# klory/vqa-attention-networks

Hardware: AMD Instinct MI355X
Metric: QA-pairs/sec fwd+bwd, MFB-baseline batch 512 (higher is better)
Workload: dtype f32

## Files before the change

include/vqa_fusion.h:

```cpp
#ifndef VQA_FUSION_H
#define VQA_FUSION_H

#include <stddef.h>
#include <stdint.h>

#ifdef __cplusplus
extern "C" {
#endif

#define VQF_OK 0
#define VQF_E_BADARG (-1)
#define VQF_E_ALIGN (-2)
#define VQF_E_UNSUPPORTED (-3)
#define VQF_E_WORKSPACE (-4)
#define VQF_E_TIMEOUT (-5)

#define VQF_POOL_K 5

#define VQF_GEMM_RELU 1
#define VQF_GEMM_ACCUM 2
#define VQF_GEMM_OUT_BF16 4

int vqf_abi_version(void);
const char* vqf_build_info(void);

#define VQF_OPT_GEMM_F32_PERSIST 0
#define VQF_OPT_GEMM_BF16_PERSIST 1
#define VQF_OPT_GEMM_F32_LOOP 2
#define VQF_OPT_GEMM_BF16_LOOP 3
#define VQF_OPT_GEMM_F32_BIG 4
#define VQF_OPT_GEMM_BF16_BIG 5
#define VQF_OPT_GEMM_F32_WAVE 6
#define VQF_OPT_FUSE_COAL 7
#define VQF_OPT_FUSE_LS 8
#define VQF_OPT_FUSE_LS_BWD 9
#define VQF_OPT_GEMM_CU_LIMIT 10
#define VQF_OPT_GEMM_F32_EDGE 11
#define VQF_OPT_GEMM_F32_ROUNDS 12
#define VQF_OPT_GEMM_SPLITK_FUSED 13
#define VQF_OPT_GEMM_F32_STREAMK 14
#define VQF_OPT_GEMM_SPLITK_ORDER 15
#define VQF_OPT_GEMM_F32_SAMPLE 16
#define VQF_OPT_GEMM_F32_N80 17
#define VQF_OPT_COUNT 18
int vqf_set_option(int option, int value, int* previous);
int vqf_get_option(int option, int* value);
const char* vqf_option_env_name(int option);

#define VQF_STAT_GEMM_F32_TILE128 0
#define VQF_STAT_GEMM_F32_BIG 1
#define VQF_STAT_GEMM_F32_WAVE 2
#define VQF_STAT_GEMM_BF16_TILE128 3
#define VQF_STAT_GEMM_BF16_BIG 4
#define VQF_STAT_GEMM_F32_SAMPLE 5
#define VQF_STAT_GEMM_F32_N80 6
#define VQF_STAT_COUNT 7
int vqf_stat_get(int stat, long long* value);

size_t vqf_gemm_f32_ws_bytes(int ta, int tb, int M, int N, int K);
int vqf_gemm_f32(int ta, int tb, int M, int N, int K,
                 const float* A, int lda, const float* B, int ldb,
                 float* C, int ldc, const float* bias, int flags,
                 void* ws, size_t ws_bytes, void* stream);

int vqf_gemm_f32_rowscale(int ta, int tb, int M, int N, int K, const float* A, int lda, const float* B, int ldb,
                          float* C, int ldc, const float* bias, int flags, const float* rowscale, int rows_per_scale,
                          void* stream);

int vqf_gemm_f32_big_rows(int ta, int tb, int M, int N, int K);
int vqf_gemm_f32_sample_supported(int NS, int L, int N, int K);
int vqf_gemm_f32_sample(int tb, int NS, int L, int N, int K, const float* A, int lda, const float* B, int ldb, float* C, int ldc,
                        const float* bias, int flags, void* stream);

int vqf_gemm_f32_batched(int ta, int tb, int batch, int M, int N, int K,
                         const float* A, int lda, long long strideA,
                         const float* B, int ldb, long long strideB,
                         float* C, int ldc, long long strideC, int flags, void* stream);

size_t vqf_gemm_bf16_ws_bytes(int ta, int tb, int M, int N, int K);
int vqf_gemm_bf16(int ta, int tb, int M, int N, int K,
                  const void* A, int lda, const void* B, int ldb,
                  float* C, int ldc, const float* bias, int flags,
                  void* ws, size_t ws_bytes, void* stream);
int vqf_gemm_bf16_rowscale(int ta, int tb, int M, int N, int K, const void* A, int lda, const void* B, int ldb,
                           float* C, int ldc, const float* bias, int flags, const float* rowscale, int rows_per_scale,
                           void* stream);

int vqf_cast_f32_bf16(const float* x, int R, int C, int ldx, void* y, int ldy, void* stream);

size_t vqf_colsum_ws_bytes(int M, int N);
int vqf_colsum_f32(const float* dY, int M, int N, int ldy, float* db,
                   void* ws, size_t ws_bytes, void* stream);

int vqf_group_reduce_f32(const float* in, int G, int J, int W, float* out, void* stream);

int vqf_relu_bwd_f32(const float* dX, const float* Y, int M, int C, float* dXpre,
                     float* dbias, void* ws, size_t ws_bytes, void* stream);

int vqf_relu_bwd_rank1_f32(const float* dX, const float* Y, const float* wts, const float* dpooled, int L, float scale, int M,
                           int C, float* dXpre, float* dbias, void* ws, size_t ws_bytes, void* stream);
int vqf_multi_add_f32(const float* const* a, const float* const* b, float* const* out, const long long* n, int count, void* stream);
int vqf_multi_copy_f32(const float* const* src, float* const* dst, const long long* n, int count, void* stream);


int vqf_att_logits_fwd(const float* hid, const float* w2, const float* b2,
                       int M, int Hh, int G, float* logits, void* stream);

int vqf_att_logits_fwd_lin(const float* hid, const float* w2, const float* b2, const float* b1, int M, int Hh, int G,
                           float* logits, float* lin, void* stream);

size_t vqf_att_logits_bwd_ws_bytes(int M, int Hh);
int vqf_att_logits_bwd(const float* dlogits, const float* hid, const float* w2,
                       int M, int Hh, int G, int relu_mask, float* dhid_pre, float* dw2,
                       float* db2, float* dbias1, void* ws, size_t ws_bytes, void* stream);
int vqf_att_logits_bwd_rowscale(const float* dlogits, const float* hid, const float* w2, const float* rowscale,
                                int rows_per_scale, int M, int Hh, int G, int relu_mask, float* dhid_pre, float* dw2,
                                float* db2, float* dbias1, void* ws, size_t ws_bytes, void* stream);
int vqf_att_logits_bwd_rowscale_obf16(const float* dlogits, const float* hid, const float* w2, const float* rowscale,
                                      int rows_per_scale, int M, int Hh, int G, void* dhid_pre_bf16, float* dw2, float* db2,
                                      float* dbias1, void* ws, size_t ws_bytes, void* stream);

int vqf_glimpse_pool_fwd(const float* feat, const float* logits, int N, int S, int C, int G,
                         int unit_softmax, float* wts, float* pooled, void* stream);

int vqf_glimpse_pool_bwd(const float* dpooled, const float* dwts_extra, const float* feat,
                         const float* wts, int N, int S, int C, int G, int unit_softmax,
                         float* dlogits, float* dfeat, void* stream);

int vqf_glimpse_pool_fwd_bf16(const void* feat, const float* logits, int N, int S, int C, int G,
                              int unit_softmax, float* wts, float* pooled, void* stream);
int vqf_glimpse_pool_bwd_bf16(const float* dpooled, const float* dwts_extra, const void* feat,
                              const float* wts, int N, int S, int C, int G, int unit_softmax,
                              float* dlogits, void* stream);

int vqf_mfb_fuse_fwd(const float* P, const float* pbias, const float* q, const float* cascade,
                     const uint8_t* keep, uint64_t seed, float p_drop,
                     int N, int L, int O, float* R, float* rowssq, float* zdrop,
                     void* stream);

int vqf_l2_group_norm(const float* rowssq, int N, int L, float* norm, float* inv, void* stream);

int vqf_scale_rows(const float* R, const float* inv, int M, int L, int W, float* Y, void* stream);

int vqf_rowdot(const float* Y, const float* dY, int M, int W, float* rowdot, void* stream);

int vqf_l2_norm_bwd_coef(const float* rowdot, const float* norm, const float* inv,
                         int N, int L, float* coefA, float* coefB, void* stream);
int vqf_l2_norm_bwd_coef_lin(const float* dlogits, const float* lin, int G, const float* norm, const float* inv, int N,
                             int L, float* coefA, float* coefB, float* unit, void* stream);

size_t vqf_mfb_fuse_bwd_ws_bytes(int N, int L, int O);
int vqf_mfb_fuse_bwd(const float* dY, const float* dzdrop, const float* Y, const float* inv,
                     const float* coefA, const float* coefB,
                     const float* P, const float* pbias, const float* q, const float* cascade,
                     const uint8_t* keep, uint64_t seed, float p_drop,
                     int N, int L, int O,
                     float* dP, float* dq, float* dcascade, float* dbiasP,
                     void* ws, size_t ws_bytes, void* stream);
int vqf_mfb_fuse_bwd_bf16dp(const float* dY, const float* Y, const float* inv, const float* coefA,
                            const float* coefB, const float* P, const float* pbias, const float* q,
                            const uint8_t* keep, uint64_t seed, float p_drop, int N, int L, int O,
                            void* dP_bf16, float* dq, float* dbiasP, void* ws, size_t ws_bytes, void* stream);
int vqf_mfb_fuse_fwd_pbf16(const void* P_bf16, const float* pbias, const float* q, const uint8_t* keep, uint64_t seed,
                           float p_drop, int N, int L, int O, float* R, float* rowssq, void* stream);
int vqf_mfb_fuse_fwd_pbf16_rb(const void* P_bf16, const float* pbias, const float* q, const uint8_t* keep, uint64_t seed,
                              float p_drop, int N, int L, int O, float* R, void* R_bf16, int ldrb, float* rowssq, void* stream);
int vqf_mfb_fuse_bwd_pbf16(const float* dY, const float* Y, const float* inv, const float* coefA,
                           const float* coefB, const void* P_bf16, const float* pbias, const float* q,
                           const uint8_t* keep, uint64_t seed, float p_drop, int N, int L, int O, void* dP_bf16,
                           float* dq, float* dbiasP, void* ws, size_t ws_bytes, void* stream);

int vqf_mfb_fuse_grouped_supported(int N, int U, int L, int O);
int vqf_mfb_fuse_fwd_grouped(const float* P, const float* pbias, const float* q, const int* idx, const uint8_t* keep, uint64_t seed,
                             float p_drop, int N, int U, int L, int O, float* R, float* rowssq, void* stream);
size_t vqf_mfb_fuse_bwd_grouped_ws_bytes(int N, int U, int L, int O);
int vqf_mfb_fuse_bwd_grouped(const float* dY, const float* Y, const float* inv, const float* coefA, const float* coefB,
                             const float* P, const float* pbias, const float* q, const int* idx, const int* order,
                             const int* grp_off, const uint8_t* keep, uint64_t seed, float p_drop, int N, int U, int L, int O,
                             float* dP, float* dq, float* dbiasP, void* ws, size_t ws_bytes, void* stream);

int vqf_mfb_fuse_fwd_len(const float* P, const float* pbias, const float* q, const int* lens, const uint8_t* keep, uint64_t seed,
                         float p_drop, int N, int L, int O, float* R, float* rowssq, void* stream);
int vqf_mfb_fuse_bwd_len(const float* dY, const float* Y, const float* inv, const float* coefA, const float* coefB, const float* P,
                         const float* pbias, const float* q, const int* lens, const uint8_t* keep, uint64_t seed, float p_drop,
                         int N, int L, int O, float* dP, float* dq, float* dbiasP, void* ws, size_t ws_bytes, void* stream);
int vqf_mfb_fuse_fwd_grouped_len(const float* P, const float* pbias, const float* q, const int* idx, const int* lens_q,
                                 const int* lens_u, const uint8_t* keep, uint64_t seed, float p_drop, int N, int U, int L, int O,
                                 float* R, float* rowssq, void* stream);
int vqf_mfb_fuse_bwd_grouped_len(const float* dY, const float* Y, const float* inv, const float* coefA, const float* coefB,
                                 const float* P, const float* pbias, const float* q, const int* idx, const int* order,
                                 const int* grp_off, const int* lens_q, const int* lens_u, const uint8_t* keep, uint64_t seed,
                                 float p_drop, int N, int U, int L, int O, float* dP, float* dq, float* dbiasP, void* ws,
                                 size_t ws_bytes, void* stream);
int vqf_glimpse_pool_fwd_grouped_len(const float* feat, const float* logits, const int* idx, const int* lens, int N, int U, int S, int C,
                                     int G, float* wts, float* pooled, void* stream);
int vqf_glimpse_pool_bwd_grouped_len(const float* dpooled, const float* dwts_extra, const float* feat, const float* wts, const int* idx,
                                     const int* order, const int* grp_off, const int* lens, int N, int U, int S, int C, int G,
                                     float* dlogits, float* dfeat, void* stream);


int vqf_dropout_f32(const float* x, const uint8_t* keep, uint64_t seed, float p_drop,
                    long long n, float* y, void* stream);
int vqf_dropout_bt(const float* x, long long sb_in, long long st_in, const uint8_t* keep, uint64_t seed, float p_drop, int B,
                   int T, int H, float* y, long long sb_out, long long st_out, void* stream);
int vqf_gate_tanh_sigmoid_fwd(const float* a, const float* b, long long n, float* y, void* stream);
int vqf_gate_tanh_sigmoid_bwd(const float* dy, const float* a, const float* b, long long n, float* da, float* db, void* stream);
int vqf_tanh_dropout_fwd(const float* a, const float* b, const uint8_t* keep, uint64_t seed,
                         float p_drop, long long n, float* y, void* stream);
int vqf_tanh_dropout_bwd(const float* dy, const float* y, const uint8_t* keep, uint64_t seed,
                         float p_drop, long long n, float* dx, void* stream);
int vqf_tanh_dropout_fwd2d(const float* a, int lda, const float* b, int ldb, const uint8_t* keep, uint64_t seed, float p_drop,
                           int R, int W, float* y, int ldy, void* stream);
int vqf_tanh_dropout_bwd2d(const float* dy, int lddy, const float* y, int ldy, const uint8_t* keep, uint64_t seed, float p_drop,
                           int R, int W, float* dx, int lddx, void* stream);
int vqf_hie_stream_supported(int N, int L, int E, int T);
int vqf_hie_chunks(int N, int L);
// ... 172 lines not shown
```

vqa-attention-networks_amd/csrc/common.h:

```cpp
#pragma once
#include <hip/hip_runtime.h>
#include <stdint.h>
#include "../../include/vqa_fusion.h"

typedef float f32x4 __attribute__((ext_vector_type(4)));
typedef float f32x16 __attribute__((ext_vector_type(16)));
typedef unsigned int u32x4 __attribute__((ext_vector_type(4)));

enum VqfKernelId {
  KID_GEMM_A0B0 = 0,
  KID_GEMM_A0B1,
  KID_GEMM_A1B0,
  KID_GEMM_A1B1,
  KID_SPLITK_REDUCE,
  KID_COLSUM,
  KID_GROUP_REDUCE,
  KID_RELU_BWD,
  KID_ATT_LOGITS_FWD,
  KID_ATT_LOGITS_BWD,
  KID_GLIMPSE_FWD,
  KID_GLIMPSE_BWD,
  KID_MFB_FUSE_FWD,
  KID_L2_GROUP_NORM,
  KID_SCALE_ROWS,
  KID_ROWDOT,
  KID_L2_BWD_COEF,
  KID_MFB_FUSE_BWD,
  KID_DROPOUT,
  KID_TANH_DROP_FWD,
  KID_TANH_DROP_BWD,
  KID_SOFTMAX_FWD,
  KID_SOFTMAX_BWD,
  KID_GEMM_BF16,
  KID_CAST_BF16,
  KID_LSTM_FWD,
  KID_LSTM_BWD,
  KID_CE_LOSS,
  KID_KLDIV_LOSS,
  KID_ADAM,
  KID_FEAT_TRANSPOSE,
  KID_LSTM_CELL_FWD,
  KID_LSTM_CELL_BWD,
  KID_EMBED_FWD,
  KID_EMBED_BWD,
  KID_HBM_COPY,
  KID_HBM_READ,
  KID_MULTI_ADD,
  KID_MULTI_COPY,
  KID_HIE_FWD,
  KID_HIE_HEAD,
  KID_HIE_ADD,
  KID_HIE_LEFT,
  KID_HIE_SLABSUM,
  KID_HIE_AFF,
  KID_PHRASE_FWD,
  KID_PHRASE_BWD,
  KID_HIE_AFF_LEVELS,
  KID_GUIDED_FWD,
  KID_GUIDED_BWD,
  KID_CE_LOSS_PRED,
  KID_ANSWER_MATCH,
  KID_TOPK_ROWS,
  KID_GLIMPSE_DFEAT_GROUPED,
  KID_ROW_BLOCK_GATHER,
  KID_ROW_BLOCK_GROUP_SUM,
  KID_MFB_FUSE_BWD_IMAGE,
  KID_ZERO_COLS,
  KID_COUNT
};

extern int g_vqf_prof_on;
extern int g_vqf_opt[VQF_OPT_COUNT];
static inline int vqf_opt(int id, int dflt) { const int v = g_vqf_opt[id]; return v < 0 ? dflt : v; }
extern long long g_vqf_stat[VQF_STAT_COUNT];
static inline void vqf_stat_bump(int id) { __atomic_fetch_add(&g_vqf_stat[id], 1LL, __ATOMIC_RELAXED); }
bool vqf_prof_begin(int id, hipStream_t s);
void vqf_prof_end(int id, hipStream_t s);
void vqf_prof_dims(int d0, int d1, int d2);

#define VQF_LAUNCH(id, kern, grid, block, shmem, stream, ...)                      \
  do {                                                                             \
    (void)hipGetLastError();     \
    const bool vqf_bracket_ = g_vqf_prof_on && vqf_prof_begin((id), (stream));     \
    hipLaunchKernelGGL(kern, grid, block, shmem, stream, __VA_ARGS__);             \
    if (vqf_bracket_) vqf_prof_end((id), (stream));                                \
  } while (0)

#define VQF_REDUCE_SPLITS 32
int vqf_colreduce_2stage(const float* in, int J, int W, float* out, float* scratch, hipStream_t s);

int vqf_splitk_reduce(const float* slab, int splits, int M, int N, float* C, int ldc,
                      const float* bias, int flags, hipStream_t s);
void vqf_splitk_counters_clear(int* words, int tiles, hipStream_t s);
int* vqf_splitk_counters(int tiles);

int vqf_gemm_bf16_big_try(int ta, int tb, int M, int N, int K, const void* A, int lda, const void* B, int ldb, float* C,
                          int ldc, const float* bias, int flags, const float* rowscale, int rps, void* ws, size_t ws_bytes,
                          hipStream_t s, int* rc);
size_t vqf_gemm_bf16_big_ws_bytes(int ta, int tb, int M, int N, int K);
int vqf_gemm_f32_big_try(int ta, int tb, int M, int N, int K, const float* A, int lda, const float* B, int ldb, float* C,
                         int ldc, const float* bias, int flags, const float* rowscale, int rps, void* ws, size_t ws_bytes,
                         hipStream_t s, int* rc, int* rows_done);
int vqf_gemm_f32_big_rows_impl(int ta, int tb, int M, int N, int K, int flags, size_t ws_bytes);
size_t vqf_gemm_f32_big_ws_bytes(int ta, int tb, int M, int N, int K);
int vqf_gemm_f32_n80_try(int M, int N, int K, const float* A, int lda, const float* B, int ldb, float* C, int ldc,
                         const float* bias, int flags, hipStream_t s, int* rc);
int vqf_lstm_step16_try(const float* h_prev, const float* w_hh, float* gates, const float* c_prev, int B, int H, float* c_out,
                        float* h_out, hipStream_t s, int* rc);
int vqf_gemm_f32_wave_try(int ta, int tb, int M, int N, int K, const float* A, int lda, const float* B, int ldb, float* C,
                          int ldc, const float* bias, int flags, hipStream_t s, int* rc);

static inline int vqf_last_error() {
  hipError_t e = hipGetLastError();
  return e == hipSuccess ? VQF_OK : (int)e;
}

static inline bool aligned16(const void* p) { return (((uintptr_t)p) & 15) == 0; }

struct VqfDynLdsFlags { int bytes[64]; };
static inline int vqf_set_dyn_lds(const void* fn, int bytes, VqfDynLdsFlags& f) {
  int dev = 0;
  (void)hipGetDevice(&dev);
  const bool tracked = dev >= 0 && dev < 64;
  if (tracked && f.bytes[dev] >= bytes) return VQF_OK;
  hipError_t e = hipFuncSetAttribute(fn, hipFuncAttributeMaxDynamicSharedMemorySize, bytes);
  if (e != hipSuccess) return (int)e;
  if (tracked && f.bytes[dev] < bytes) f.bytes[dev] = bytes;
  return VQF_OK;
}

static inline int vqf_cu_count() {
  static int cached[64] = {};
  int dev = 0;
  (void)hipGetDevice(&dev);
  const bool tracked = dev >= 0 && dev < 64;
  if (tracked && cached[dev] > 0) return cached[dev];
  int n = 0;
  if (hipDeviceGetAttribute(&n, hipDeviceAttributeMultiprocessorCount, dev) != hipSuccess) n = 0;
  if (tracked) cached[dev] = n;
  return n;
}

__device__ __forceinline__ float vqf_tanh_fast(float x) {
  const float e = __expf(2.0f * x);
  const float r = __builtin_amdgcn_rcpf(e + 1.0f);
  return e > 16777216.0f ? 1.0f : (e - 1.0f) * r;
}

#ifndef VQF_STREAM_NT
#define VQF_STREAM_NT 1
#endif
template <typename T> __device__ __forceinline__ T vqf_ld_stream(const T* p) {
  return VQF_STREAM_NT ? __builtin_nontemporal_load(p) : *p;
}
template <typename T> __device__ __forceinline__ void vqf_st_stream(T* p, T v) {
  if (VQF_STREAM_NT) __builtin_nontemporal_store(v, p); else *p = v;
}

__device__ __forceinline__ bool aligned16_dev(const void* p) { return (((uintptr_t)p) & 15) == 0; }
__device__ __forceinline__ float wave_sum(float v) {
#pragma unroll
  for (int o = 32; o > 0; o >>= 1) v += __shfl_xor(v, o, 64);
  return v;
}
__device__ __forceinline__ float wave_max(float v) {
#pragma unroll
  for (int o = 32; o > 0; o >>= 1) v = fmaxf(v, __shfl_xor(v, o, 64));
  return v;
}

__device__ __forceinline__ unsigned long long vqf_argmax_key(float v, int idx) {
  const unsigned int b = __float_as_uint(v);
  const unsigned int k = (v != v) ? 0xFFFFFFFEu : (v == 0.f ? 0x80000000u : ((b & 0x80000000u) ? ~b : (b | 0x80000000u)));
  return ((unsigned long long)k << 32) | (unsigned int)~(unsigned int)idx;
}
__device__ __forceinline__ int vqf_argmax_index(unsigned long long key) { return (int)~(unsigned int)key; }
__device__ __forceinline__ unsigned long long wave_max_u64(unsigned long long v) {
#pragma unroll
  for (int o = 32; o > 0; o >>= 1) {
    const unsigned long long t = __shfl_xor(v, o, 64);
    v = t > v ? t : v;
  }
  return v;
}
__device__ __forceinline__ unsigned long long vqf_block256_max_u64(unsigned long long v, unsigned long long* sh) {
  v = wave_max_u64(v);
  __syncthreads();
  if ((threadIdx.x & 63) == 0) sh[threadIdx.x >> 6] = v;
  __syncthreads();
  const unsigned long long a = sh[0] > sh[1] ? sh[0] : sh[1], b = sh[2] > sh[3] ? sh[2] : sh[3];
  return a > b ? a : b;
}

struct VqfSplitkTile { int* cnt; const float* slab; float* C; const float* bias; int M, N, ldc, flags; long long pstride; int sld; };
template <int TILE_M, int TILE_N, int NT, bool WT = false>
__device__ __forceinline__ bool vqf_splitk_combine(const VqfSplitkTile& g, int tile, int splits, int m0, int n0, int tid,
                                                   float* scratch) {
  asm volatile("s_waitcnt vmcnt(0)" ::: "memory");
  __syncthreads();
  if (tid == 0) {
    if (!WT) {
      __builtin_amdgcn_fence(__ATOMIC_RELEASE, "agent");
      asm volatile("s_waitcnt vmcnt(0)" ::: "memory");
    }
    const int ticket = __hip_atomic_fetch_add(g.cnt + tile, 1, __ATOMIC_RELAXED, __HIP_MEMORY_SCOPE_AGENT);
    *reinterpret_cast<volatile int*>(scratch) = ticket;
  }
  __syncthreads();
  const int ticket = *reinterpret_cast<volatile int*>(scratch);
  __syncthreads();
  if (ticket != splits - 1) return false;
  if (tid == 0) {
    __builtin_amdgcn_fence(__ATOMIC_ACQUIRE, "agent");
    asm volatile("s_waitcnt vmcnt(0)" ::: "memory");
    __hip_atomic_store(g.cnt + tile, 0, __ATOMIC_RELAXED, __HIP_MEMORY_SCOPE_AGENT);
  }
  __syncthreads();
  constexpr int CT = TILE_N / 4, RSTEP = NT / CT;
  static_assert(NT % CT == 0, "TILE_N / 4 must divide the workgroup size");
  const bool local = g.pstride != 0;
  const long long total = local ? g.pstride : (long long)g.M * g.N;
  const int sld = local ? g.sld : g.N;
  const int srow0 = local ? m0 : 0, scol0 = local ? n0 : 0;
  const bool relu = g.flags & VQF_GEMM_RELU, accum = g.flags & VQF_GEMM_ACCUM;
  const int c4 = tid % CT, r0 = tid / CT;
  const int col = n0 + 4 * c4;
  if ((g.N & 3) == 0 && (sld & 3) == 0 && (g.ldc & 3) == 0 && aligned16_dev(g.C) && aligned16_dev(g.slab) &&
      (!g.bias || aligned16_dev(g.bias))) {
    if (col >= g.N) return true;
    const f32x4 bv = g.bias ? *reinterpret_cast<const f32x4*>(g.bias + col) : f32x4{0.f, 0.f, 0.f, 0.f};
    for (int k = 0; k < TILE_M / RSTEP; k += 2) {
      const int rowA = m0 + r0 + RSTEP * k, rowB = rowA + RSTEP;
      if (rowA >= g.M) break;
      const bool hasB = rowB < g.M && k + 1 < TILE_M / RSTEP;
      const float* pA = g.slab + (long long)(rowA - srow0) * sld + (col - scol0);
      const float* pB = g.slab + (long long)((hasB ? rowB : rowA) - srow0) * sld + (col - scol0);
      f32x4 vA = {0.f, 0.f, 0.f, 0.f}, vB = vA;
      int z = 0;
      for (; z + 3 < splits; z += 4) {
        f32x4 a[4], b[4];
#pragma unroll
        for (int q = 0; q < 4; ++q) {
          a[q] = *reinterpret_cast<const f32x4*>(pA + (z + q) * total);
          b[q] = *reinterpret_cast<const f32x4*>(pB + (z + q) * total);
        }
#pragma unroll
        for (int q = 0; q < 4; ++q) { vA += a[q]; vB += b[q]; }
      }
      for (; z < splits; ++z) {
        vA += *reinterpret_cast<const f32x4*>(pA + z * total);
        vB += *reinterpret_cast<const f32x4*>(pB + z * total);
      }
      vA += bv; vB += bv;
      float* cA = g.C + (long long)rowA * g.ldc + col;
      float* cB = g.C + (long long)rowB * g.ldc + col;
      if (accum) {
        vA += *reinterpret_cast<const f32x4*>(cA);
        if (hasB) vB += *reinterpret_cast<const f32x4*>(cB);
      }
      if (relu) {
#pragma unroll
        for (int j = 0; j < 4; ++j) { vA[j] = fmaxf(vA[j], 0.f); vB[j] = fmaxf(vB[j], 0.f); }
      }
// ... 47 lines not shown
```

vqa-attention-networks_amd/csrc/gemm_f32.hip:

```cpp
#include "common.h"
#include <atomic>

namespace {

#ifndef VQF_SPLITK_WT
#define VQF_SPLITK_WT 0
#endif
#ifndef VQF_GEMM_BK
#define VQF_GEMM_BK 16
#endif
#ifndef VQF_GEMM_WAVES_PER_SIMD
#define VQF_GEMM_WAVES_PER_SIMD 4
#endif
#ifndef VQF_GEMM_GLDS
#define VQF_GEMM_GLDS 0
#endif
constexpr int BM = 128, BN = 128, BK = VQF_GEMM_BK, NTHREADS = 256;
constexpr bool GLDS = (VQF_GEMM_GLDS != 0) && (BK == 16);
constexpr int LD_RK = GLDS ? BK : BK + 4;
__device__ __forceinline__ int rk_swz(int row) { return GLDS ? ((row >> 2) & 3) : 0; }
constexpr int OP_FLOATS = BM * LD_RK;
constexpr int STAGE_FLOATS = 2 * OP_FLOATS;
constexpr int SMEM_BYTES = 2 * STAGE_FLOATS * 4;
constexpr int K4 = BK / 4;
constexpr int NLD = BM * BK / 4 / NTHREADS;
static_assert(BK % 8 == 0 && NLD >= 1, "BK must be a multiple of 8");

struct GemmArgs {
  const float* A;
  const float* B;
  float* C;
  const float* bias;
  float* slab;
  int M, N, K, lda, ldb, ldc;
  int flags;
  int kchunk;
  int tiles_m, tiles_n;
  int vecA, vecB;
  long long sA, sB, sC;
  const float* rowscale;
  int rps;
  int row0;
  int* cnt;
};

#ifndef VQF_GEMM_RK_REMAP
#define VQF_GEMM_RK_REMAP 0
#endif
__device__ __forceinline__ int rk_row(int f) {
  if (VQF_GEMM_RK_REMAP && K4 == 4) return ((f >> 5) << 3) + (((f >> 2) & 1) << 2) + ((f >> 3) & 3);
  return f / K4;
}
__device__ __forceinline__ int rk_k(int f) { return (f % K4) << 2; }

template <bool T>
__device__ __forceinline__ void load_tile(const float* __restrict__ p, int ld, int r0, int R,
                                          int k0, int kend, bool vec, int tid, f32x4 (&v)[NLD]) {
#pragma unroll
  for (int i = 0; i < NLD; ++i) {
    const int f = tid + NTHREADS * i;
    int r, k;
    if (!T) { r = r0 + rk_row(f); k = k0 + rk_k(f); }
    else    { k = k0 + (f >> 5); r = r0 + ((f & 31) << 2); }
    f32x4 x = {0.f, 0.f, 0.f, 0.f};
    if (!T) {
      if (r < R) {
        const float* q = p + (long long)r * ld + k;
        if (vec && k + 3 < kend) x = *reinterpret_cast<const f32x4*>(q);
        else {
#pragma unroll
          for (int j = 0; j < 4; ++j) if (k + j < kend) x[j] = q[j];
        }
      }
    } else {
      if (k < kend) {
        const float* q = p + (long long)k * ld + r;
        if (vec && r + 3 < R) x = *reinterpret_cast<const f32x4*>(q);
        else {
#pragma unroll
          for (int j = 0; j < 4; ++j) if (r + j < R) x[j] = q[j];
        }
      }
    }
    v[i] = x;
  }
}

typedef const float __attribute__((address_space(1))) gfloat;
typedef const f32x4 __attribute__((address_space(1))) gf32x4;

template <bool T>
__device__ __forceinline__ void init_ptrs(const float* __restrict__ p0, int ld, int r0, int R, int k0,
                                          int tid, gfloat* (&q)[NLD]) {
  gfloat* p = (gfloat*)p0;
#pragma unroll
  for (int i = 0; i < NLD; ++i) {
    const int f = tid + NTHREADS * i;
    if (!T) {
      const int r = min(r0 + rk_row(f), R - 1);
      q[i] = p + (long long)r * ld + (k0 + rk_k(f));
    } else {
      const int r = min(r0 + ((f & 31) << 2), R - 4);
      q[i] = p + (long long)(k0 + (f >> 5)) * ld + r;
    }
  }
}
template <bool T>
__device__ __forceinline__ void load_fast(gfloat* (&q)[NLD], int ld, f32x4 (&v)[NLD]) {
#pragma unroll
  for (int i = 0; i < NLD; ++i) {
    v[i] = *(gf32x4*)q[i];
    q[i] += T ? (long long)BK * ld : BK;
  }
}

constexpr int NGL = (BM * BK) / (4 * 64 * 4);
template <bool T>
__device__ __forceinline__ void init_glds_ptrs(const float* __restrict__ p0, int ld, int r0, int R, int k0,
                                               int wave, int lane, gfloat* (&q)[NGL]) {
  gfloat* p = (gfloat*)p0;
#pragma unroll
  for (int i = 0; i < NGL; ++i) {
    const int blk = wave * NGL + i;
    if (!T) {
      const int row = blk * 16 + (lane >> 2);
      const int c = (lane & 3) ^ rk_swz(row);
      q[i] = p + (long long)min(r0 + row, R - 1) * ld + (k0 + 4 * c);
    } else {
      const int k = blk * 2 + (lane >> 5);
      q[i] = p + (long long)(k0 + k) * ld + min(r0 + ((lane & 31) << 2), R - 4);
    }
  }
}
template <bool T>
__device__ __forceinline__ void glds_tile(gfloat* (&q)[NGL], int ld, float* s, int wave) {
  typedef __attribute__((address_space(3))) float lds_float;
#pragma unroll
  for (int i = 0; i < NGL; ++i) {
    lds_float* dst = (lds_float*)(s + (wave * NGL + i) * 256);
    __builtin_amdgcn_global_load_lds(q[i], dst, 16, 0, 0);
    q[i] += T ? (long long)BK * ld : BK;
  }
}

template <bool T>
__device__ __forceinline__ void store_tile(float* s, int tid, const f32x4 (&v)[NLD]) {
#pragma unroll
  for (int i = 0; i < NLD; ++i) {
    const int f = tid + NTHREADS * i;
    if (!T) *reinterpret_cast<f32x4*>(s + rk_row(f) * LD_RK + (((rk_k(f) >> 2) ^ rk_swz(rk_row(f))) << 2)) = v[i];
    else    *reinterpret_cast<f32x4*>(s + (f >> 5) * BM + ((f & 31) << 2)) = v[i];
  }
}
// ... 16 lines not shown
  const int nfull = (kend - kbeg) / BK;
  bool v10 = true, v01 = true;
  if (EDGE) {
    v10 = (m0 + wr * 64 + 32) < g.M;
    v01 = (n0 + wc * 64 + 32) < g.N;
  }
  f32x4 ra[NLD], rb[NLD];
  auto mma_tile = [&](const float* sA, const float* sB) {
#pragma unroll
    for (int g8 = 0; g8 < BK / 8; ++g8) {
      if (!EDGE) {
        f32x4 af[2], bf[2];
#pragma unroll
        for (int i = 0; i < 2; ++i) af[i] = read_frag<TA>(sA, wr * 64 + i * 32 + l31, g8, h);
#pragma unroll
        for (int j = 0; j < 2; ++j) bf[j] = read_frag<TB>(sB, wc * 64 + j * 32 + l31, g8, h);
#pragma unroll
        for (int kk = 0; kk < 4; ++kk)
#pragma unroll
          for (int i = 0; i < 2; ++i)
#pragma unroll
            for (int j = 0; j < 2; ++j)
              acc[i][j] = __builtin_amdgcn_mfma_f32_32x32x2f32(af[i][kk], bf[j][kk], acc[i][j], 0, 0, 0);
      } else {
        const f32x4 a0 = read_frag<TA>(sA, wr * 64 + l31, g8, h);
        const f32x4 b0 = read_frag<TB>(sB, wc * 64 + l31, g8, h);
#pragma unroll
        for (int kk = 0; kk < 4; ++kk)
          acc[0][0] = __builtin_amdgcn_mfma_f32_32x32x2f32(a0[kk], b0[kk], acc[0][0], 0, 0, 0);
        if (v10) {
          const f32x4 a1 = read_frag<TA>(sA, wr * 64 + 32 + l31, g8, h);
#pragma unroll
          for (int kk = 0; kk < 4; ++kk)
            acc[1][0] = __builtin_amdgcn_mfma_f32_32x32x2f32(a1[kk], b0[kk], acc[1][0], 0, 0, 0);
        }
        if (v01) {
          const f32x4 b1 = read_frag<TB>(sB, wc * 64 + 32 + l31, g8, h);
#pragma unroll
          for (int kk = 0; kk < 4; ++kk)
            acc[0][1] = __builtin_amdgcn_mfma_f32_32x32x2f32(a0[kk], b1[kk], acc[0][1], 0, 0, 0);
        }
      }
    }
  };

  if (FAST && GLDS) {
    const int lane = tid & 63, wave = 2 * wr + wc;
    gfloat* ga[NGL];
    gfloat* gb[NGL];
    init_glds_ptrs<TA>(gA, g.lda, m0, g.M, kbeg, wave, lane, ga);
    init_glds_ptrs<TB>(gB, g.ldb, n0, g.N, kbeg, wave, lane, gb);
    if (nfull > 0) {
      glds_tile<TA>(ga, g.lda, smem, wave);
      glds_tile<TB>(gb, g.ldb, smem + OP_FLOATS, wave);
    } else {
      load_tile<TA>(gA, g.lda, m0, g.M, kbeg, kend, g.vecA, tid, ra);
      load_tile<TB>(gB, g.ldb, n0, g.N, kbeg, kend, g.vecB, tid, rb);
      store_tile<TA>(smem, tid, ra);
      store_tile<TB>(smem + OP_FLOATS, tid, rb);
    }
    __syncthreads();
    for (int t = 0; t < ntiles; ++t) {
      float* sA = smem + (t & 1) * STAGE_FLOATS;
      float* sB = sA + OP_FLOATS;
      float* dA = smem + ((t + 1) & 1) * STAGE_FLOATS;
      const bool more = (t + 1) < ntiles;
      const bool dma = (t + 1) < nfull;
      if (!dma && more) {
        const int k0 = kbeg + (t + 1) * BK;
        load_tile<TA>(gA, g.lda, m0, g.M, k0, kend, g.vecA, tid, ra);
        load_tile<TB>(gB, g.ldb, n0, g.N, k0, kend, g.vecB, tid, rb);
      }
      if (!EDGE) {
        f32x4 af[BK / 8][2], bf[BK / 8][2];
#pragma unroll
        for (int g8 = 0; g8 < BK / 8; ++g8) {
#pragma unroll
          for (int i = 0; i < 2; ++i) af[g8][i] = read_frag<TA>(sA, wr * 64 + i * 32 + l31, g8, h);
#pragma unroll
          for (int j = 0; j < 2; ++j) bf[g8][j] = read_frag<TB>(sB, wc * 64 + j * 32 + l31, g8, h);
        }
        asm volatile("s_waitcnt lgkmcnt(0)" ::: "memory");
        if (dma) {
          glds_tile<TA>(ga, g.lda, dA, wave);
          glds_tile<TB>(gb, g.ldb, dA + OP_FLOATS, wave);
        }
#pragma unroll
        for (int g8 = 0; g8 < BK / 8; ++g8)
#pragma unroll
          for (int kk = 0; kk < 4; ++kk)
#pragma unroll
            for (int i = 0; i < 2; ++i)
#pragma unroll
              for (int j = 0; j < 2; ++j)
                acc[i][j] = __builtin_amdgcn_mfma_f32_32x32x2f32(af[g8][i][kk], bf[g8][j][kk], acc[i][j], 0, 0, 0);
      } else {
        if (dma) {
          glds_tile<TA>(ga, g.lda, dA, wave);
          glds_tile<TB>(gb, g.ldb, dA + OP_FLOATS, wave);
        }
        mma_tile(sA, sB);
      }
      if (more && !dma) {
        store_tile<TA>(dA, tid, ra);
        store_tile<TB>(dA + OP_FLOATS, tid, rb);
      }
      __syncthreads();
    }
    return;
  }

  gfloat* pa[NLD];
  gfloat* pb[NLD];
  if (FAST) {
    init_ptrs<TA>(gA, g.lda, m0, g.M, kbeg, tid, pa);
    init_ptrs<TB>(gB, g.ldb, n0, g.N, kbeg, tid, pb);
  }
  if (FAST && nfull > 0) {
    load_fast<TA>(pa, g.lda, ra);
    load_fast<TB>(pb, g.ldb, rb);
  } else {
    load_tile<TA>(gA, g.lda, m0, g.M, kbeg, kend, g.vecA, tid, ra);
    load_tile<TB>(gB, g.ldb, n0, g.N, kbeg, kend, g.vecB, tid, rb);
  }
  store_tile<TA>(smem, tid, ra);
  store_tile<TB>(smem + OP_FLOATS, tid, rb);
  __syncthreads();

  for (int t = 0; t < ntiles; ++t) {
    const float* sA = smem + (t & 1) * STAGE_FLOATS;
    const float* sB = sA + OP_FLOATS;
    const bool more = (t + 1) < ntiles;
    if (more) {
      if (FAST && (t + 1) < nfull) {
        load_fast<TA>(pa, g.lda, ra);
        load_fast<TB>(pb, g.ldb, rb);
      } else {
        const int k0 = kbeg + (t + 1) * BK;
        load_tile<TA>(gA, g.lda, m0, g.M, k0, kend, g.vecA, tid, ra);
        load_tile<TB>(gB, g.ldb, n0, g.N, k0, kend, g.vecB, tid, rb);
      }
    }
    mma_tile(sA, sB);
    if (more) {
      float* d = smem + ((t + 1) & 1) * STAGE_FLOATS;
      store_tile<TA>(d, tid, ra);
      store_tile<TB>(d + OP_FLOATS, tid, rb);
    }
    __syncthreads();
  }
}

template <bool TA, bool TB, bool FAST>
__global__ void __launch_bounds__(NTHREADS, VQF_GEMM_WAVES_PER_SIMD) gemm_f32_kernel(GemmArgs g) {
  extern __shared__ __attribute__((aligned(16))) float smem[];
  const int tid = threadIdx.x, lane = tid & 63;
  const int wave = __builtin_amdgcn_readfirstlane(tid >> 6);
  const int wr = wave >> 1, wc = wave & 1;
  const int l31 = lane & 31, h = lane >> 5;

  const int nwg = g.tiles_m * g.tiles_n;
  const int bid = blockIdx.x;
  const int q8 = nwg >> 3, r8 = nwg & 7, xcd = bid & 7;
  const int wg = (xcd < r8 ? xcd * (q8 + 1) : r8 * (q8 + 1) + (xcd - r8) * q8) + (bid >> 3);
  constexpr int GROUP_M = 8;
  const int per_group = GROUP_M * g.tiles_n;
  const int gid = wg / per_group;
  const int first_m = gid * GROUP_M;
  const int gsz = min(g.tiles_m - first_m, GROUP_M);
  const int in_g = wg - gid * per_group;
  const int tm = first_m + in_g % gsz, tn = in_g / gsz;
  const int m0 = tm * BM, n0 = tn * BN;
  const int kbeg = blockIdx.y * g.kchunk;
  const int kend = min(g.K, kbeg + g.kchunk);

  f32x16 acc[2][2];
#pragma unroll
  for (int i = 0; i < 2; ++i)
#pragma unroll
    for (int j = 0; j < 2; ++j)
#pragma unroll
      for (int r = 0; r < 16; ++r) acc[i][j][r] = 0.f;

  const float* gA = g.A + (long long)blockIdx.z * g.sA;
  const float* gB = g.B + (long long)blockIdx.z * g.sB;
  const bool all_valid = (m0 + wr * 64 + 32) < g.M && (n0 + wc * 64 + 32) < g.N;
  if (all_valid)
    gemm_mainloop<TA, TB, FAST, false>(g, smem, gA, gB, m0, n0, kbeg, kend, tid, wr, wc, l31, h, acc);
  else
    gemm_mainloop<TA, TB, FAST, true>(g, smem, gA, gB, m0, n0, kbeg, kend, tid, wr, wc, l31, h, acc);

  const bool to_slab = g.slab != nullptr;
  float* out = to_slab ? g.slab + (long long)blockIdx.y * g.M * g.N
                       : g.C + (long long)blockIdx.z * g.sC;
  const int ldo = to_slab ? g.N : g.ldc;
#pragma unroll
  for (int j = 0; j < 2; ++j) {
    const int col = n0 + wc * 64 + j * 32 + l31;
    if (col >= g.N) continue;
    const float bv = (!to_slab && g.bias) ? g.bias[col] : 0.f;
#pragma unroll
    for (int i = 0; i < 2; ++i) {
#pragma unroll
      for (int r = 0; r < 16; ++r) {
        const int row = m0 + wr * 64 + i * 32 + (r & 3) + 8 * (r >> 2) + 4 * h;
        if (row < g.M) {
          float* pc = out + (long long)row * ldo + col;
          float v = (g.rowscale ? acc[i][j][r] * g.rowscale[(g.row0 + row) / g.rps] : acc[i][j][r]) + bv;
          if (!to_slab) {
            if (g.flags & VQF_GEMM_ACCUM) v += *pc;
            if (g.flags & VQF_GEMM_RELU) v = fmaxf(v, 0.f);
          }
#if VQF_SPLITK_WT
          if (to_slab && g.cnt) __hip_atomic_store(pc, v, __ATOMIC_RELAXED, __HIP_MEMORY_SCOPE_AGENT); else
#endif
          *pc = v;
        }
      }
    }
  }
  if (to_slab && g.cnt) {
    const VqfSplitkTile st = {g.cnt, g.slab, g.C, g.bias, g.M, g.N, g.ldc, g.flags};
    vqf_splitk_combine<BM, BN, NTHREADS, VQF_SPLITK_WT != 0>(st, bid, (int)gridDim.y, m0, n0, tid, smem);
  }
}

__global__ void splitk_reduce_kernel(const float* __restrict__ slab, int splits, int M, int N,
                                     float* __restrict__ C, int ldc, const float* __restrict__ bias,
                                     int flags) {
  const long long total = (long long)M * N;
  const long long stride = (long long)gridDim.x * blockDim.x;
  for (long long i = (long long)blockIdx.x * blockDim.x + threadIdx.x; i < total; i += stride) {
    const int row = (int)(i / N), col = (int)(i - (long long)row * N);
    float v = 0.f;
    for (int z = 0; z < splits; ++z) v += slab[(long long)z * total + i];
    if (bias) v += bias[col];
    float* pc = C + (long long)row * ldc + col;
    if (flags & VQF_GEMM_ACCUM) v += *pc;
    if (flags & VQF_GEMM_RELU) v = fmaxf(v, 0.f);
    *pc = v;
  }
}

template <bool TA, bool TB, bool FAST>
int launch_gemm_impl(const GemmArgs& g, dim3 grid, hipStream_t s, int kid) {
  static VqfDynLdsFlags attr = {};
  if (int e = vqf_set_dyn_lds(reinterpret_cast<const void*>(&gemm_f32_kernel<TA, TB, FAST>), SMEM_BYTES, attr)) return e;
  VQF_LAUNCH(kid, (gemm_f32_kernel<TA, TB, FAST>), grid, dim3(NTHREADS), SMEM_BYTES, s, g);
  return vqf_last_error();
}

template <bool TA, bool TB>
int launch_gemm(const GemmArgs& g, dim3 grid, hipStream_t s, int kid) {
  const bool okA = g.vecA && (!TA || (g.M % 4 == 0 && g.M >= 4));
  const bool okB = g.vecB && (!TB || (g.N % 4 == 0 && g.N >= 4));
  if (okA && okB) return launch_gemm_impl<TA, TB, true>(g, grid, s, kid);
  return launch_gemm_impl<TA, TB, false>(g, grid, s, kid);
}

}

constexpr int VQF_SPLITK_RING = 1 << 16;
__device__ int vqf_splitk_ring[VQF_SPLITK_RING];
int* vqf_splitk_counters(int tiles) {
  static int* base[64] = {};
  static std::atomic<unsigned> next{0};
  if (tiles <= 0 || tiles > VQF_SPLITK_RING / 4) return nullptr;
  int dev = 0;
  if (hipGetDevice(&dev) != hipSuccess || dev < 0 || dev >= 64) return nullptr;
  if (!base[dev]) {
    void* q = nullptr;
    if (hipGetSymbolAddress(&q, HIP_SYMBOL(vqf_splitk_ring)) != hipSuccess) return nullptr;
    base[dev] = (int*)q;
  }
  unsigned cur = next.load(std::memory_order_relaxed), start;
  do {
    start = (cur % VQF_SPLITK_RING) + (unsigned)tiles <= (unsigned)VQF_SPLITK_RING ? cur % VQF_SPLITK_RING : 0u;
  } while (!next.compare_exchange_weak(cur, start + (unsigned)tiles, std::memory_order_relaxed));
  return base[dev] + start;
}

void vqf_splitk_counters_clear(int* words, int tiles, hipStream_t s) {
  if (words && tiles > 0) (void)hipMemsetAsync(words, 0, (size_t)tiles * sizeof(int), s);
}

int vqf_splitk_reduce(const float* slab, int splits, int M, int N, float* C, int ldc,
                      const float* bias, int flags, hipStream_t s) {
  const long long total = (long long)M * N;
  int blocks = (int)((total + 255) / 256);
  if (blocks > 4096) blocks = 4096;
  VQF_LAUNCH(KID_SPLITK_REDUCE, splitk_reduce_kernel, dim3(blocks), dim3(256), 0, s, slab, splits, M,
             N, C, ldc, bias, flags);
  return vqf_last_error();
}

extern "C" size_t vqf_gemm_f32_ws_bytes(int ta, int tb, int M, int N, int K) {
  return vqf_gemm_f32_big_ws_bytes(ta, tb, M, N, K);
}

static int gemm_tile128(int ta, int tb, int M, int N, int K, const float* A, int lda, const float* B, int ldb, float* C,
                        int ldc, const float* bias, int flags, const float* rowscale, int rps, int row0, void* ws,
                        size_t ws_bytes, hipStream_t s);

extern "C" int vqf_gemm_f32_big_rows(int ta, int tb, int M, int N, int K) {
  if (M <= 0 || N <= 0 || K <= 0) return 0;
  return vqf_gemm_f32_big_rows_impl(ta, tb, M, N, K, 0, (size_t)1 << 40);
}

extern "C" int vqf_gemm_f32(int ta, int tb, int M, int N, int K, const float* A, int lda,
                            const float* B, int ldb, float* C, int ldc, const float* bias,
                            int flags, void* ws, size_t ws_bytes, void* stream) {
  if (!A || !B || !C || M <= 0 || N <= 0 || K <= 0 || lda <= 0 || ldb <= 0 || ldc < N)
    return VQF_E_BADARG;
  hipStream_t s = (hipStream_t)stream;
  if (aligned16(A) && aligned16(B) && (lda % 4 == 0) && (ldb % 4 == 0)) {
    int rc = VQF_OK, done = 0;
    if (vqf_gemm_f32_big_try(ta, tb, M, N, K, A, lda, B, ldb, C, ldc, bias, flags, nullptr, 1, ws, ws_bytes, s, &rc, &done)) {
      if (rc != VQF_OK || done >= M) return rc;
      A += (size_t)done * lda; C += (size_t)done * ldc; M -= done;
      ws = nullptr; ws_bytes = 0;
    }
    else if (vqf_gemm_f32_wave_try(ta, tb, M, N, K, A, lda, B, ldb, C, ldc, bias, flags, s, &rc)) return rc;
    else if (!ta && !tb && vqf_gemm_f32_n80_try(M, N, K, A, lda, B, ldb, C, ldc, bias, flags, s, &rc)) return rc;
  }
  return gemm_tile128(ta, tb, M, N, K, A, lda, B, ldb, C, ldc, bias, flags, nullptr, 1, 0, ws, ws_bytes, s);
}

extern "C" int vqf_gemm_f32_rowscale(int ta, int tb, int M, int N, int K, const float* A, int lda, const float* B,
                                     int ldb, float* C, int ldc, const float* bias, int flags, const float* rowscale,
                                     int rows_per_scale, void* stream) {
  if (!A || !B || !C || !rowscale || rows_per_scale <= 0 || M <= 0 || N <= 0 || K <= 0 || lda <= 0 || ldb <= 0 || ldc < N)
    return VQF_E_BADARG;
  if (flags & VQF_GEMM_ACCUM) return VQF_E_UNSUPPORTED;
  hipStream_t s = (hipStream_t)stream;
  int row0 = 0;
  if (aligned16(A) && aligned16(B) && (lda % 4 == 0) && (ldb % 4 == 0)) {
    int rc = VQF_OK, done = 0;
    if (vqf_gemm_f32_big_try(ta, tb, M, N, K, A, lda, B, ldb, C, ldc, bias, flags, rowscale, rows_per_scale, nullptr, 0, s, &rc,
                             &done)) {
      if (rc != VQF_OK || done >= M) return rc;
      A += (size_t)done * lda; C += (size_t)done * ldc; M -= done; row0 = done;
    }
  }
  return gemm_tile128(ta, tb, M, N, K, A, lda, B, ldb, C, ldc, bias, flags, rowscale, rows_per_scale, row0, nullptr, 0, s);
}

static int gemm_tile128(int ta, int tb, int M, int N, int K, const float* A, int lda, const float* B, int ldb, float* C,
                        int ldc, const float* bias, int flags, const float* rowscale, int rps, int row0, void* ws,
                        size_t ws_bytes, hipStream_t s) {
  GemmArgs g;
  g.A = A; g.B = B; g.C = C; g.bias = bias; g.slab = nullptr;
  g.M = M; g.N = N; g.K = K; g.lda = lda; g.ldb = ldb; g.ldc = ldc; g.flags = flags;
  g.sA = g.sB = g.sC = 0;
  g.rowscale = rowscale; g.rps = rps; g.row0 = row0; g.cnt = nullptr;
  g.tiles_m = (M + BM - 1) / BM;
  g.tiles_n = (N + BN - 1) / BN;
  g.vecA = aligned16(A) && (lda % 4 == 0);
  g.vecB = aligned16(B) && (ldb % 4 == 0);

  const long long tiles = (long long)g.tiles_m * g.tiles_n;
  const int ktiles = (K + BK - 1) / BK;
  int splits = 1;
  const int slots = 512;
  if (ws && tiles < 1024 && ktiles >= 32 && !(tiles >= 512 && K <= 1024) && !(tiles >= 192 && tiles <= 256 && K <= 512)) {
    double best = 1e30;
    for (int sp = 1; sp <= 16; ++sp) {
      if (ktiles / sp < 16) break;
      if ((size_t)sp * M * N * sizeof(float) > ws_bytes) break;
      const double blocks = (double)tiles * sp;
      const double rounds = (double)((long long)((blocks + slots - 1) / slots));
      const double cost = rounds / sp * (1.0 + 0.01 * sp);
      if (cost < best - 1e-12) { best = cost; splits = sp; }
    }
  }
  int kt_per = (ktiles + splits - 1) / splits;
  g.kchunk = kt_per * BK;
  splits = (K + g.kchunk - 1) / g.kchunk;
  if (splits > 1) {
    g.slab = (float*)ws;
    if (vqf_opt(VQF_OPT_GEMM_SPLITK_FUSED, 0) == 1) g.cnt = vqf_splitk_counters((int)tiles);
  }

  dim3 grid((unsigned)tiles, (unsigned)splits);
  const int kid = KID_GEMM_A0B0 + 2 * (ta ? 1 : 0) + (tb ? 1 : 0);
  if (g_vqf_prof_on) vqf_prof_dims(M, N, K);
  vqf_stat_bump(VQF_STAT_GEMM_F32_TILE128);
  int rc;
  if (!ta && !tb) rc = launch_gemm<false, false>(g, grid, s, kid);
  else if (!ta && tb) rc = launch_gemm<false, true>(g, grid, s, kid);
  else if (ta && !tb) rc = launch_gemm<true, false>(g, grid, s, kid);
  else rc = launch_gemm<true, true>(g, grid, s, kid);
  if (rc != VQF_OK) {
    vqf_splitk_counters_clear(g.cnt, (int)tiles, s);
    return rc;
  }
  if (splits > 1 && !g.cnt) rc = vqf_splitk_reduce((const float*)ws, splits, M, N, C, ldc, bias, flags, s);
  return rc;
}

extern "C" int vqf_gemm_f32_batched(int ta, int tb, int batch, int M, int N, int K, const float* A,
                                    int lda, long long strideA, const float* B, int ldb,
                                    long long strideB, float* C, int ldc, long long strideC,
                                    int flags, void* stream) {
  if (!A || !B || !C || batch <= 0 || batch > 65535 || M <= 0 || N <= 0 || K <= 0 || lda <= 0 ||
      ldb <= 0 || ldc < N)
    return VQF_E_BADARG;
  GemmArgs g;
  g.A = A; g.B = B; g.C = C; g.bias = nullptr; g.slab = nullptr;
  g.M = M; g.N = N; g.K = K; g.lda = lda; g.ldb = ldb; g.ldc = ldc; g.flags = flags;
  g.sA = strideA; g.sB = strideB; g.sC = strideC;
  g.rowscale = nullptr; g.rps = 1; g.row0 = 0; g.cnt = nullptr;
  g.tiles_m = (M + BM - 1) / BM;
  g.tiles_n = (N + BN - 1) / BN;
  g.vecA = aligned16(A) && (lda % 4 == 0) && (strideA % 4 == 0);
  g.vecB = aligned16(B) && (ldb % 4 == 0) && (strideB % 4 == 0);
  g.kchunk = ((K + BK - 1) / BK) * BK;
  dim3 grid((unsigned)(g.tiles_m * g.tiles_n), 1, (unsigned)batch);
  hipStream_t s = (hipStream_t)stream;
  const int kid = KID_GEMM_A0B0 + 2 * (ta ? 1 : 0) + (tb ? 1 : 0);
  vqf_stat_bump(VQF_STAT_GEMM_F32_TILE128);
  if (!ta && !tb) return launch_gemm<false, false>(g, grid, s, kid);
  if (!ta && tb) return launch_gemm<false, true>(g, grid, s, kid);
  if (ta && !tb) return launch_gemm<true, false>(g, grid, s, kid);
  return launch_gemm<true, true>(g, grid, s, kid);
}
```

vqa-attention-networks_amd/csrc/gemm_f32_n80.hip:

```cpp
#include "common.h"

namespace {

typedef const float __attribute__((address_space(1))) gfloat;

constexpr int TM = 128, TN = 80, TK = 32, NT = 512, NSLOT = 4;
constexpr int A_BYTES = TM * TK * 4;
constexpr int b_bytes(int ntc) { return 16 * ntc * TK * 4; }
constexpr int slot_bytes(int ntc) { return A_BYTES + b_bytes(ntc); }

struct N80Args {
  const float* A; const float* B; float* C; const float* bias;
  int M, N, K, lda, ldb, ldc, flags, tiles_m, tiles;
  const float* c_prev; float* c_out; float* h_out; int H;
};

__device__ __forceinline__ float sigm_f(float x) { return 1.0f / (1.0f + expf(-x)); }

__device__ __forceinline__ int swz(int rho) {
  const int i = (rho >> 1) & 7;
  return i ^ (((i + 2) & 4) >> 1);
}

__device__ __forceinline__ void wait_own(int later, bool two) {
// ... 3 lines not shown
    else if (later == 1) asm volatile("s_waitcnt vmcnt(4)" ::: "memory");
    else                 asm volatile("s_waitcnt vmcnt(0)" ::: "memory");
  } else {
    if (later >= 3)      asm volatile("s_waitcnt vmcnt(9)" ::: "memory");
    else if (later == 2) asm volatile("s_waitcnt vmcnt(6)" ::: "memory");
    else if (later == 1) asm volatile("s_waitcnt vmcnt(3)" ::: "memory");
    else                 asm volatile("s_waitcnt vmcnt(0)" ::: "memory");
  }
}

template <int NTC, bool CELL>
__global__ void __launch_bounds__(NT, 1) gemm_f32_n80_kernel(const N80Args g) {
  constexpr int SLOT_BYTES = slot_bytes(NTC), TNC = 16 * NTC;
  extern __shared__ __attribute__((aligned(16))) char smem[];
  typedef __attribute__((address_space(3))) char lds_char;
  const int per = (gridDim.x + 7) >> 3;
  const int lin = (blockIdx.x & 7) * per + (blockIdx.x >> 3);
  if (lin >= g.tiles) return;
  const int tn = lin / g.tiles_m, tm = lin - tn * g.tiles_m;
  const int m0 = tm * TM, n0 = tn * TNC;
  const int tid = threadIdx.x, lane = tid & 63;
  const int wave = __builtin_amdgcn_readfirstlane(tid >> 6);
  const int c = lane & 15, kq = lane >> 4;
  const bool two = NTC == 5 && wave < 2;
  const int S = g.K / TK;

  float oldg[4][4], cpv[4];
  if (CELL) {
    const int u = (n0 >> 2) + c;
#pragma unroll
    for (int j = 0; j < 4; ++j) {
      const long long row = m0 + 16 * wave + 4 * kq + j;
#pragma unroll
      for (int t = 0; t < 4; ++t) oldg[t][j] = g.C[row * g.ldc + t * g.H + u];
      cpv[j] = g.c_prev ? g.c_prev[row * g.H + u] : 0.f;
    }
  }

  gfloat* qa[2];
  gfloat* qb[2];
#pragma unroll
  for (int i = 0; i < 2; ++i) {
    const int ra = 16 * wave + 8 * i + (lane >> 3);
    qa[i] = (gfloat*)(g.A + (long long)min(m0 + ra, g.M - 1) * g.lda + 4 * ((lane & 7) ^ swz(ra)));
    const int rho = 8 * (wave + 8 * i) + (lane >> 3);
    const int brow = CELL ? (min(rho, TNC - 1) >> 4) * g.H + (n0 >> 2) + (rho & 15)
                          : min(n0 + min(rho, TNC - 1), g.N - 1);
    qb[i] = (gfloat*)(g.B + (long long)brow * g.ldb + 4 * ((lane & 7) ^ swz(rho)));
  }
  auto issue_piece = [&](int s, int slot, int p) {
    lds_char* da = (lds_char*)(smem + slot * SLOT_BYTES + wave * 2048);
    lds_char* db = (lds_char*)(smem + slot * SLOT_BYTES + A_BYTES + wave * 1024);
    if (p == 0)      __builtin_amdgcn_global_load_lds(qa[0] + (long long)s * TK, da, 16, 0, 0);
    else if (p == 1) __builtin_amdgcn_global_load_lds(qa[1] + (long long)s * TK, da + 1024, 16, 0, 0);
    else if (p == 2) __builtin_amdgcn_global_load_lds(qb[0] + (long long)s * TK, db, 16, 0, 0);
    else if (two)    __builtin_amdgcn_global_load_lds(qb[1] + (long long)s * TK, db + 8 * 1024, 16, 0, 0);
  };
  auto issue = [&](int s, int slot) {
#pragma unroll
    for (int p = 0; p < 4; ++p) issue_piece(s, slot, p);
  };

  f32x4 acc[NTC];
#pragma unroll
  for (int t = 0; t < NTC; ++t) acc[t] = f32x4{0.f, 0.f, 0.f, 0.f};

  constexpr int NFR = 2 + 2 * NTC;
  struct Frag { f32x4 a[2], b[NTC][2]; };
  auto read_frag = [&](int slot, Frag& f, int i) {
    const char* sa = smem + slot * SLOT_BYTES;
    if (i < 2) {
      const int ra = 16 * wave + c;
      f.a[i] = *reinterpret_cast<const f32x4*>(sa + ra * 128 + (((2 * kq + i) ^ swz(ra)) << 4));
    } else {
      const int t = (i - 2) >> 1, u = (i - 2) & 1, rho = 16 * t + c;
      f.b[t][u] = *reinterpret_cast<const f32x4*>(sa + A_BYTES + rho * 128 + (((2 * kq + u) ^ swz(rho)) << 4));
    }
  };

  auto step = [&](int s, int q, const Frag& cur, Frag& nxt) {
    const bool more = s + 1 < S, copy = s + NSLOT < S;
#pragma unroll
    for (int grp = 0; grp < 8; ++grp) {
      const int u = grp >> 2, j = grp & 3;
#pragma unroll
      for (int t = 0; t < NTC; ++t) acc[t] = __builtin_amdgcn_mfma_f32_16x16x4f32(cur.a[u][j], cur.b[t][u][j], acc[t], 0, 0, 0);
#ifndef VQF_N80_NOCOPY
      if (grp < 4) { if (copy) issue_piece(s + NSLOT, q, grp); }
#endif
#ifndef VQF_N80_NOREAD
      if (more && 2 * grp < NFR) { read_frag((q + 1) % NSLOT, nxt, 2 * grp); read_frag((q + 1) % NSLOT, nxt, 2 * grp + 1); }
#endif
      __builtin_amdgcn_sched_barrier(0);
    }
  };
#pragma unroll
  for (int p = 0; p < NSLOT; ++p) issue(p, p);
  Frag fr[2];
  wait_own(NSLOT - 1, two);
  __builtin_amdgcn_s_barrier();
#pragma unroll
  for (int i = 0; i < NFR; ++i) read_frag(0, fr[0], i);
  for (int s0 = 0; s0 < S; s0 += NSLOT) {
#pragma unroll
    for (int q = 0; q < NSLOT; ++q) {
      const int s = s0 + q;
      if (s + 1 < S) wait_own(min(NSLOT - 2, S - 2 - s), two);
      __builtin_amdgcn_s_waitcnt(0xC07F);
#ifndef VQF_N80_NOBARRIER
      __builtin_amdgcn_s_barrier();
#endif
      step(s, q, fr[q & 1], fr[(q + 1) & 1]);
    }
  }

  if (CELL) {
    const int u = (n0 >> 2) + c;
#pragma unroll
    for (int j = 0; j < 4; ++j) {
      const long long row = m0 + 16 * wave + 4 * kq + j;
      const float ig = sigm_f(acc[0][j] + oldg[0][j]);
      const float fg = sigm_f(acc[1][j] + oldg[1][j]);
      const float gg = tanhf(acc[2 % NTC][j] + oldg[2][j]);
      const float og = sigm_f(acc[3 % NTC][j] + oldg[3][j]);
      float* pg = g.C + row * g.ldc + u;
      pg[0] = ig; pg[g.H] = fg; pg[2 * g.H] = gg; pg[3 * g.H] = og;
      const float cn = fg * cpv[j] + ig * gg;
      g.c_out[row * g.H + u] = cn;
      g.h_out[row * g.H + u] = og * tanhf(cn);
    }
    return;
  }
  const bool relu = g.flags & VQF_GEMM_RELU;
#pragma unroll
  for (int t = 0; t < NTC; ++t) {
    const int col = n0 + 16 * t + c;
    if (col < g.N) {
      const float bv = g.bias ? g.bias[col] : 0.f;
#pragma unroll
      for (int j = 0; j < 4; ++j) {
        const int row = m0 + 16 * wave + 4 * kq + j;
        if (row < g.M) {
          float v = acc[t][j] + bv;
          if (relu) v = fmaxf(v, 0.f);
          g.C[(long long)row * g.ldc + col] = v;
        }
      }
    }
  }
}

}

int vqf_gemm_f32_n80_try(int M, int N, int K, const float* A, int lda, const float* B, int ldb, float* C, int ldc,
                         const float* bias, int flags, hipStream_t s, int* rc) {
  if (vqf_opt(VQF_OPT_GEMM_F32_N80, 1) == 0) return 0;
  if ((flags & ~VQF_GEMM_RELU) || (K % 128) || K < 512 || !aligned16(A) || !aligned16(B) || (lda % 4) || (ldb % 4)) return 0;
  const int tiles_m = (M + TM - 1) / TM, tiles_n = (N + TN - 1) / TN;
  const long long tiles = (long long)tiles_m * tiles_n;
  const int cus = vqf_cu_count() > 0 ? vqf_cu_count() : 256;
  if (tiles > cus || tiles * 10 < (long long)cus * 8 || M > 1024) return 0;
  if (vqf_opt(VQF_OPT_GEMM_CU_LIMIT, 0) >= 8) return 0;
  N80Args g;
  g.A = A; g.B = B; g.C = C; g.bias = bias; g.M = M; g.N = N; g.K = K; g.lda = lda; g.ldb = ldb; g.ldc = ldc; g.flags = flags;
  g.tiles_m = tiles_m; g.tiles = (int)tiles;
  const int nwg = ((int)tiles + 7) & ~7;
  vqf_prof_dims(M, N, K);
  vqf_stat_bump(VQF_STAT_GEMM_F32_N80);
  static VqfDynLdsFlags attr = {};
  if (int e = vqf_set_dyn_lds(reinterpret_cast<const void*>(&gemm_f32_n80_kernel<5, false>), NSLOT * slot_bytes(5), attr)) { *rc = e; return 1; }
  VQF_LAUNCH(KID_GEMM_A0B0, (gemm_f32_n80_kernel<5, false>), dim3(nwg), dim3(NT), NSLOT * slot_bytes(5), s, g);
  *rc = vqf_last_error();
  return 1;
}

int vqf_lstm_step16_try(const float* h_prev, const float* w_hh, float* gates, const float* c_prev, int B, int H, float* c_out,
                        float* h_out, hipStream_t s, int* rc) {
  if (vqf_opt(VQF_OPT_GEMM_F32_N80, 1) == 0 || vqf_opt(VQF_OPT_GEMM_CU_LIMIT, 0) >= 8) return 0;
  if ((B % TM) || (H % 128) || H < 512) return 0;
  const int tiles_m = B / TM, tiles_n = H / 16;
  const long long tiles = (long long)tiles_m * tiles_n;
  const int cus = vqf_cu_count() > 0 ? vqf_cu_count() : 256;
  if (tiles > cus || tiles * 10 < (long long)cus * 8) return 0;
  N80Args g = {};
  g.A = h_prev; g.B = w_hh; g.C = gates; g.M = B; g.N = 4 * H; g.K = H; g.lda = H; g.ldb = H; g.ldc = 4 * H;
  g.tiles_m = tiles_m; g.tiles = (int)tiles;
  g.c_prev = c_prev; g.c_out = c_out; g.h_out = h_out; g.H = H;
  const int nwg = ((int)tiles + 7) & ~7;
  vqf_prof_dims(B, 4 * H, H);
  vqf_stat_bump(VQF_STAT_GEMM_F32_N80);
  static VqfDynLdsFlags attr = {};
  if (int e = vqf_set_dyn_lds(reinterpret_cast<const void*>(&gemm_f32_n80_kernel<4, true>), NSLOT * slot_bytes(4), attr)) { *rc = e; return 1; }
  VQF_LAUNCH(KID_LSTM_CELL_FWD, (gemm_f32_n80_kernel<4, true>), dim3(nwg), dim3(NT), NSLOT * slot_bytes(4), s, g);
  *rc = vqf_last_error();
  return 1;
}
```

vqa-attention-networks_amd/csrc/gemm_f32_wave.hip:

```cpp
#include "common.h"
#include <stdlib.h>

namespace {

typedef const float __attribute__((address_space(1))) gfloat;
typedef float f32x2 __attribute__((ext_vector_type(2)));

constexpr int WTM = 32, WTN = 64, TK = 16, NSLOT = 6, NT = 256;
constexpr int A_BYTES = WTM * TK * 4, B_BYTES = WTN * TK * 4, SLOT_BYTES = A_BYTES + B_BYTES;
constexpr int WAVE_LDS = NSLOT * SLOT_BYTES;
constexpr int SMEM_WAVE = 4 * WAVE_LDS;
constexpr int NGA = A_BYTES / 1024, NGB = B_BYTES / 1024, NGL = NGA + NGB;

struct WaveArgs {
  const float* A;
  const float* B;
  float* C;
  const float* bias;
  int M, N, K, lda, ldb, ldc, flags;
  int tiles_m, tiles_n, kpart;
  const float* c_prev;
  float* c_out;
  float* h_out;
  int H;
// ... 325 lines not shown
    if (s + 1 < S) half(s + 1, fb, fa);
  }
  const int cm = lane & 31, h = lane >> 5;
  const int col = n0 + 2 * cm;
  const float b0 = (g.bias && col < g.N) ? g.bias[col] : 0.f;
  const float b1 = (g.bias && col + 1 < g.N) ? g.bias[col + 1] : 0.f;
#pragma unroll
  for (int e = 0; e < 16; ++e)
    put2(g, m0 + (e & 3) + 8 * (e >> 2) + 4 * h, col, acc[0][e], acc[1][e], b0, b1, vec, cold[e][0], cold[e][1]);
}

template <bool TB, int NSL>
int launch_shb(const WaveArgs& g, int nwg, hipStream_t s) {
  static VqfDynLdsFlags attr = {};
  constexpr int SMEM_SHB = NSL * (4 * A_BYTES + B_BYTES);
  if (int e = vqf_set_dyn_lds(reinterpret_cast<const void*>(&gemm_f32_wave_shb_kernel<TB, NSL>), SMEM_SHB, attr)) return e;
  VQF_LAUNCH(KID_GEMM_A0B0 + (TB ? 1 : 0), (gemm_f32_wave_shb_kernel<TB, NSL>), dim3(nwg), dim3(NT), SMEM_SHB, s, g);
  return vqf_last_error();
}

__device__ __forceinline__ float sigm_f(float x) { return 1.0f / (1.0f + expf(-x)); }

__global__ void __launch_bounds__(NT, 1) gemm_f32_lstm_fwd_kernel(const WaveArgs g) {
  constexpr int NSL = 6;
  constexpr int SHB_A = NSL * A_BYTES;
  extern __shared__ __attribute__((aligned(16))) char smem[];
  typedef __attribute__((address_space(3))) char lds_char;
  const int tid = threadIdx.x, lane = tid & 63;
  const int wave = __builtin_amdgcn_readfirstlane(tid >> 6);
  const int nwg = gridDim.x, bid = blockIdx.x;
  const int q8 = nwg >> 3, r8 = nwg & 7, xcd = bid & 7;
  const int wg = (xcd < r8 ? xcd * (q8 + 1) : r8 * (q8 + 1) + (xcd - r8) * q8) + (bid >> 3);
  const int t = 4 * wg + wave;
  const int tm = t % g.tiles_m, tn = t / g.tiles_m;
  const int m0 = tm * WTM, u0 = tn * 16, H = g.H;
  const int S = g.kpart / TK;
  char* myA = smem + wave * SHB_A;
  char* shB = smem + 4 * SHB_A;

  f32x16 acc[2];
#pragma unroll
  for (int j = 0; j < 2; ++j)
#pragma unroll
    for (int e = 0; e < 16; ++e) acc[j][e] = 0.f;

  gfloat* q[NGS];
#pragma unroll
  for (int i = 0; i < NGA; ++i) {
    const int row = 16 * i + (lane >> 2);
    const int chunk = (lane & 3) ^ swz(row);
    q[i] = (gfloat*)(g.A + (long long)min(m0 + row, g.M - 1) * g.lda + chunk * 4);
  }
  {
    const int rho = 16 * wave + (lane >> 2);
    const int chunk = (lane & 3) ^ swz(rho);
    const int gate = 2 * (rho >> 5) + ((rho & 31) >> 4);
    q[NGA] = (gfloat*)(g.B + (long long)(gate * H + u0 + (rho & 15)) * g.ldb + chunk * 4);
  }
  auto copy = [&](int i, int sl) {
    lds_char* dst = (i < NGA) ? (lds_char*)(myA + sl * A_BYTES + i * 1024) : (lds_char*)(shB + sl * B_BYTES + wave * 1024);
    __builtin_amdgcn_global_load_lds(q[i], dst, 16, 0, 0);
    q[i] += TK;
  };
#pragma unroll
  for (int p = 0; p < NSL - 1; ++p)
    if (p < S) {
#pragma unroll
      for (int i = 0; i < NGS; ++i) copy(i, p);
    }
  const int cm = lane & 31, hh = lane >> 5;
  const int col0 = (cm >> 4) * H + u0 + (cm & 15);
  float old0[16], old1[16], cpv[16];
#pragma unroll
  for (int e = 0; e < 16; ++e) {
    const int row = m0 + (e & 3) + 8 * (e >> 2) + 4 * hh;
    const float* pc = g.C + (long long)row * g.ldc + col0;
    old0[e] = pc[0];
    old1[e] = pc[2 * H];
    cpv[e] = (g.c_prev && cm < 16) ? g.c_prev[(long long)row * H + u0 + cm] : 0.f;
  }
  FragS<false> fa[2], fb[2];
  int slot = 0;
  auto half = [&](int s, FragS<false> (&cur)[2], FragS<false> (&nxt)[2]) {
    const bool more = s + 1 < S, refill = s + NSL - 1 < S;
    const int nslot = (slot + 1 == NSL) ? 0 : slot + 1;
    const int rslot = (slot == 0) ? NSL - 1 : slot - 1;
#pragma unroll
    for (int n = 0; n < 16; ++n) {
      const int ks = n >> 3, e = (n >> 1) & 3, j = n & 1;
      acc[j] = __builtin_amdgcn_mfma_f32_32x32x2f32(cur[ks].a[e], cur[ks].b(j, e), acc[j], 0, 0, 0);
      if (n < NGS && refill) copy(n, rslot);
      if (n == 6 && more) {
        wait_copies3(min(NSL - 2, S - 2 - s));
        __builtin_amdgcn_s_barrier();
      }
      if (n == 7 && more) nxt[0].load(myA + nslot * A_BYTES, shB + nslot * B_BYTES, 0, lane);
      if (n == 9 && more) nxt[1].load(myA + nslot * A_BYTES, shB + nslot * B_BYTES, 1, lane);
      __builtin_amdgcn_sched_barrier(0);
    }
    __builtin_amdgcn_s_waitcnt(0xC07F);
    __builtin_amdgcn_sched_barrier(0);
    slot = nslot;
  };
  if (S > 0) {
    wait_copies3(min(NSL - 2, S - 1));
    __builtin_amdgcn_s_barrier();
    fa[0].load(myA, shB, 0, lane);
    fa[1].load(myA, shB, 1, lane);
    __builtin_amdgcn_sched_barrier(0);
    __builtin_amdgcn_s_waitcnt(0xC07F);
    __builtin_amdgcn_sched_barrier(0);
  }
  for (int s = 0; s < S; s += 2) {
    half(s, fa, fb);
    if (s + 1 < S) half(s + 1, fb, fa);
  }
  const bool lo = cm < 16;
#pragma unroll
  for (int e = 0; e < 16; ++e) {
    const int row = m0 + (e & 3) + 8 * (e >> 2) + 4 * hh;
    const float a0 = sigm_f(acc[0][e] + old0[e]);
    const float p1 = acc[1][e] + old1[e];
    const float a1 = lo ? tanhf(p1) : sigm_f(p1);
    float* pc = g.C + (long long)row * g.ldc + col0;
    pc[0] = a0;
    pc[2 * H] = a1;
    const float f_act = __shfl_xor(a0, 16, 64), o_act = __shfl_xor(a1, 16, 64);
    if (lo) {
      const float c = f_act * cpv[e] + a0 * a1;
      g.c_out[(long long)row * H + u0 + cm] = c;
      g.h_out[(long long)row * H + u0 + cm] = o_act * tanhf(c);
    }
  }
}

int launch_lstm_fwd(const WaveArgs& g, int nwg, hipStream_t s) {
  static VqfDynLdsFlags attr = {};
  constexpr int SMEM_SHB = 6 * (4 * A_BYTES + B_BYTES);
  if (int e = vqf_set_dyn_lds(reinterpret_cast<const void*>(&gemm_f32_lstm_fwd_kernel), SMEM_SHB, attr)) return e;
  VQF_LAUNCH(KID_LSTM_CELL_FWD, gemm_f32_lstm_fwd_kernel, dim3(nwg), dim3(NT), SMEM_SHB, s, g);
  return vqf_last_error();
}

template <bool TB, int WK>
int launch(const WaveArgs& g, int nwg, hipStream_t s) {
  static VqfDynLdsFlags attr = {};
  if (int e = vqf_set_dyn_lds(reinterpret_cast<const void*>(&gemm_f32_wave_kernel<TB, WK>), SMEM_WAVE, attr)) return e;
  VQF_LAUNCH(KID_GEMM_A0B0 + (TB ? 1 : 0), (gemm_f32_wave_kernel<TB, WK>), dim3(nwg), dim3(NT), SMEM_WAVE, s, g);
  return vqf_last_error();
}

}

int vqf_gemm_f32_wave_try(int ta, int tb, int M, int N, int K, const float* A, int lda, const float* B, int ldb, float* C,
                          int ldc, const float* bias, int flags, hipStream_t s, int* rc) {
  if (vqf_opt(VQF_OPT_GEMM_F32_WAVE, 1) == 0) return 0;
  if (ta || M > 1024 || (K % TK) || K < 256 || !aligned16(A) || !aligned16(B) || (lda % 4) || (ldb % 4)) return 0;
  if (tb && (N % 4)) return 0;
  if ((long long)((M + 127) / 128) * ((N + 127) / 128) >= 256) return 0;
  WaveArgs g;
  g.A = A; g.B = B; g.C = C; g.bias = bias;
  g.M = M; g.N = N; g.K = K; g.lda = lda; g.ldb = ldb; g.ldc = ldc; g.flags = flags;
  g.tiles_m = (M + WTM - 1) / WTM;
  g.tiles_n = (N + WTN - 1) / WTN;
  const int tiles = g.tiles_m * g.tiles_n;
  const int nwg1 = (tiles + 3) / 4, nwg4 = tiles;
  const bool ok4 = (K % (4 * TK) == 0) && K / 4 >= 256;
  int wk = 0;
  if (nwg1 <= 256 && nwg1 >= 192) wk = 1;
  else if (ok4 && nwg4 <= 256 && nwg4 >= 192) wk = 4;
  if (!wk) return 0;
  g.kpart = (wk == 1) ? K : K / 4;
  vqf_prof_dims(M, N, K);
  vqf_stat_bump(VQF_STAT_GEMM_F32_WAVE);
  const bool shb = wk == 1 && (g.tiles_m % 4 == 0) && tiles % 4 == 0 && vqf_opt(VQF_OPT_GEMM_F32_WAVE, 2) != 1;
  if (shb && vqf_opt(VQF_OPT_GEMM_F32_WAVE, 2) == 3)
    *rc = tb ? launch_shb<true, 12>(g, nwg1, s) : launch_shb<false, 12>(g, nwg1, s);
  else if (shb)     *rc = tb ? launch_shb<true, 6>(g, nwg1, s) : launch_shb<false, 6>(g, nwg1, s);
  else if (wk == 1) *rc = tb ? launch<true, 1>(g, nwg1, s) : launch<false, 1>(g, nwg1, s);
  else         *rc = tb ? launch<true, 4>(g, nwg4, s) : launch<false, 4>(g, nwg4, s);
  return 1;
}

extern "C" int vqf_lstm_step_supported(int B, int H) {
  return B > 0 && H >= 256 && (B % 128) == 0 && (H % 16) == 0 && vqf_opt(VQF_OPT_GEMM_F32_WAVE, 2) != 0;
}
extern "C" int vqf_lstm_step_fwd(const float* h_prev, const float* w_hh, float* gates, const float* c_prev, int B, int H,
                                 float* c_out, float* h_out, void* stream) {
  if (!h_prev || !w_hh || !gates || !c_out || !h_out || B <= 0 || H <= 0) return VQF_E_BADARG;
  if (!vqf_lstm_step_supported(B, H)) return VQF_E_UNSUPPORTED;
  if (!aligned16(h_prev) || !aligned16(w_hh) || !aligned16(gates) || !aligned16(c_out) || !aligned16(h_out) ||
      (c_prev && !aligned16(c_prev)))
    return VQF_E_ALIGN;
  {
    int rc = VQF_OK;
    if (vqf_lstm_step16_try(h_prev, w_hh, gates, c_prev, B, H, c_out, h_out, (hipStream_t)stream, &rc)) return rc;
  }
  WaveArgs g = {};
  g.A = h_prev; g.B = w_hh; g.C = gates; g.bias = nullptr;
  g.M = B; g.N = 4 * H; g.K = H; g.lda = H; g.ldb = H; g.ldc = 4 * H; g.flags = VQF_GEMM_ACCUM;
  g.tiles_m = B / WTM;
  g.tiles_n = H / 16;
  g.kpart = H;
  g.c_prev = c_prev; g.c_out = c_out; g.h_out = h_out; g.H = H;
  vqf_prof_dims(B, 4 * H, H);
  vqf_stat_bump(VQF_STAT_GEMM_F32_WAVE);
  return launch_lstm_fwd(g, g.tiles_m * g.tiles_n / 4, (hipStream_t)stream);
}
```

vqa-attention-networks_amd/csrc/prof.hip:

```cpp
#include "common.h"
#include <mutex>
#include <stdlib.h>
#include <vector>

int g_vqf_prof_on = 0;
int g_vqf_opt[VQF_OPT_COUNT];
long long g_vqf_stat[VQF_STAT_COUNT] = {};

namespace {
const char* const kOptEnv[VQF_OPT_COUNT] = {
    "VQF_GEMM_F32_PERSIST", "VQF_GEMM_BF16_PERSIST", "VQF_GEMM_F32_LOOP", "VQF_GEMM_BF16_LOOP", "VQF_GEMM_F32_BIG",
    "VQF_GEMM_BF16_BIG", "VQF_GEMM_F32_WAVE", "VQF_FUSE_COAL", "VQF_FUSE_LS", "VQF_FUSE_LS_BWD", "VQF_GEMM_CU_LIMIT",
    "VQF_GEMM_F32_EDGE", "VQF_GEMM_F32_ROUNDS", "VQF_GEMM_SPLITK_FUSED", "VQF_GEMM_F32_STREAMK", "VQF_GEMM_SPLITK_ORDER", "VQF_GEMM_F32_SAMPLE", "VQF_GEMM_F32_N80"};
const char* const kOptEnvOld[VQF_OPT_COUNT] = {
    nullptr, nullptr, "VQF_GEMM_F32_PP", "VQF_GEMM_BF16_PP", nullptr, nullptr, nullptr, nullptr, nullptr, nullptr, nullptr,
    nullptr, nullptr, nullptr, nullptr, nullptr, nullptr};
struct OptInit {
  OptInit() {
    for (int i = 0; i < VQF_OPT_COUNT; ++i) {
      const char* e = getenv(kOptEnv[i]);
      if (!e && kOptEnvOld[i]) e = getenv(kOptEnvOld[i]);
      g_vqf_opt[i] = (e && ((e[0] >= '0' && e[0] <= '9') || e[0] == '-')) ? atoi(e) : -1;
    }
  }
} g_opt_init;
}

namespace {
struct Pair { hipEvent_t a, b; int id; int d[3]; };
std::mutex g_mu;
std::vector<Pair> g_pairs;
std::vector<hipEvent_t> g_free;
thread_local hipEvent_t t_start = nullptr;
thread_local int t_dims[3] = {0, 0, 0};
long long g_min_mnk = 0;

const char* const kNames[KID_COUNT] = {
    "gemm_f32_a0b0(fwd)", "gemm_f32_a0b1(dgrad)", "gemm_f32_a1b0", "gemm_f32_a1b1(wgrad)",
    "splitk_reduce", "colsum", "group_reduce", "relu_bwd",
    "att_logits_fwd", "att_logits_bwd", "glimpse_pool_fwd", "glimpse_pool_bwd",
    "mfb_fuse_fwd", "l2_group_norm", "scale_rows", "rowdot", "l2_norm_bwd_coef", "mfb_fuse_bwd",
    "dropout", "tanh_dropout_fwd", "tanh_dropout_bwd", "softmax_rows_fwd", "softmax_rows_bwd",
    "gemm_bf16", "cast_f32_bf16",
    "lstm_seq_fwd(all steps)", "lstm_seq_bwd(all steps)",
    "ce_loss", "kldiv_loss", "adam_step", "feat_transpose",
    "lstm_cell_fwd", "lstm_cell_bwd", "embed_tanh_fwd", "embed_tanh_bwd", "hbm_copy", "hbm_read_sweep", "multi_add", "multi_copy", "hie_hv_fwd", "hie_head_bwd", "hie_rank_add", "hie_rank_left", "hie_slab_sum", "hie_affinity",
    "phrase_ngram_fwd", "phrase_ngram_bwd", "hie_affinity_levels", "guided_logits_fwd", "guided_logits_bwd",
    "ce_loss_pred", "answer_match_rows", "topk_rows", "glimpse_dfeat_grouped", "row_block_gather", "row_block_group_sum",
    "mfb_fuse_bwd_image", "zero_cols_len"};

hipEvent_t get_event() {
  std::lock_guard<std::mutex> lk(g_mu);
  if (!g_free.empty()) { hipEvent_t e = g_free.back(); g_free.pop_back(); return e; }
  hipEvent_t e = nullptr;
  (void)hipEventCreate(&e);
  return e;
}
}

bool vqf_prof_begin(int id, hipStream_t s) {
  if (g_min_mnk > 0) {
    const bool gemm = (id >= KID_GEMM_A0B0 && id <= KID_GEMM_A1B1) || id == KID_GEMM_BF16;
    if (!gemm || (long long)t_dims[0] * t_dims[1] * t_dims[2] < g_min_mnk) return false;
  }
  t_start = get_event();
  (void)hipEventRecord(t_start, s);
  return true;
}
void vqf_prof_end(int id, hipStream_t s) {
  hipEvent_t b = get_event();
  (void)hipEventRecord(b, s);
  std::lock_guard<std::mutex> lk(g_mu);
  g_pairs.push_back({t_start, b, id, {t_dims[0], t_dims[1], t_dims[2]}});
}
void vqf_prof_dims(int d0, int d1, int d2) { t_dims[0] = d0; t_dims[1] = d1; t_dims[2] = d2; }

extern "C" {
int vqf_abi_version(void) { return 7; }
int vqf_set_option(int option, int value, int* previous) {
  if (option < 0 || option >= VQF_OPT_COUNT) return VQF_E_BADARG;
  if (previous) *previous = g_vqf_opt[option];
  g_vqf_opt[option] = value < 0 ? -1 : value;
  return VQF_OK;
}
int vqf_stat_get(int stat, long long* value) {
  if (stat < 0 || stat >= VQF_STAT_COUNT || !value) return VQF_E_BADARG;
  *value = __atomic_load_n(&g_vqf_stat[stat], __ATOMIC_RELAXED);
  return VQF_OK;
}
int vqf_get_option(int option, int* value) {
  if (option < 0 || option >= VQF_OPT_COUNT || !value) return VQF_E_BADARG;
  *value = g_vqf_opt[option];
  return VQF_OK;
}
const char* vqf_option_env_name(int option) { return (option >= 0 && option < VQF_OPT_COUNT) ? kOptEnv[option] : ""; }
const char* vqf_build_info(void) {
  return "libvqa_fusion gfx950 fp32-mfma(v_mfma_f32_32x32x2_f32) tiles 128x128x16 + 256x256x16(lds-dma, staggered) + "
         "32x64-per-wave(small M) bf16-mfma(v_mfma_f32_16x16x32_bf16 / 32x32x16) tiles 128x128x32 + "
         "256x256x32(lds-dma, ping-pong) wave64 philox4x32-10";
}
void vqf_prof_enable(int on) { g_vqf_prof_on = on ? 1 : 0; }
void vqf_prof_filter(long long min_mnk) { g_min_mnk = min_mnk > 0 ? min_mnk : 0; }
void vqf_prof_reset(void) {
  std::lock_guard<std::mutex> lk(g_mu);
  for (auto& p : g_pairs) { g_free.push_back(p.a); g_free.push_back(p.b); }
  g_pairs.clear();
}
int vqf_prof_num_kernels(void) { return KID_COUNT; }
const char* vqf_prof_kernel_name(int id) { return (id >= 0 && id < KID_COUNT) ? kNames[id] : ""; }
int vqf_prof_get(int id, long long* launches, double* total_ms) {
  return vqf_prof_get_shape(id, -1, -1, -1, launches, total_ms);
}
int vqf_prof_get_shape(int id, int d0, int d1, int d2, long long* launches, double* total_ms) {
  if (id < 0 || id >= KID_COUNT || !launches || !total_ms) return VQF_E_BADARG;
  std::lock_guard<std::mutex> lk(g_mu);
  long long n = 0;
  double ms = 0.0;
  for (auto& p : g_pairs) {
    if (p.id != id) continue;
    if ((d0 >= 0 && p.d[0] != d0) || (d1 >= 0 && p.d[1] != d1) || (d2 >= 0 && p.d[2] != d2)) continue;
    hipError_t e = hipEventSynchronize(p.b);
    if (e != hipSuccess) return (int)e;
    float t = 0.f;
    e = hipEventElapsedTime(&t, p.a, p.b);
    if (e != hipSuccess) return (int)e;
    ms += t;
    ++n;
  }
  *launches = n;
  *total_ms = ms;
  return VQF_OK;
}
}
```

vqa-attention-networks_amd/host/functions.py:

```python
import torch

from . import ops


def _c(t):
    return t if t.is_contiguous() else t.contiguous()


def _w2d(w):
    return _c(w.reshape(w.shape[0], -1))


def _bf16_ok(*dims):
    return all(d % 8 == 0 for d in dims)


class EmbedTanhFn(torch.autograd.Function):

    @staticmethod
    def forward(ctx, ids, weight, tanh=True, time_major=False, lens=None):
        ids = ids.contiguous()
        out = ops.embed_tanh_fwd(_c(weight), ids, tanh, time_major, lens=lens)
        ctx.save_for_backward(ids, out if tanh else None)
        ctx.V, ctx.tm, ctx.lens = weight.shape[0], bool(time_major), lens
        return out

    @staticmethod
    def backward(ctx, dout):
        ids, out = ctx.saved_tensors
        return None, ops.embed_tanh_bwd(_c(dout), out, ids, ctx.V, ctx.tm, lens=ctx.lens), None, None, None


def _plain_embedding(embedding, ids):
    w = embedding.weight
    return (w.is_cuda and w.dtype == torch.float32 and ids.is_cuda and ids.dtype == torch.int64 and embedding.padding_idx is None
            and embedding.max_norm is None and not embedding.sparse and not embedding.scale_grad_by_freq and w.shape[1] <= 1024)


def embed_tanh(embedding, ids, time_major=False):
    if _plain_embedding(embedding, ids):
        return EmbedTanhFn.apply(ids, embedding.weight, True, bool(time_major) and ids.dim() == 2)
    y = torch.tanh(embedding(ids))
    return y.transpose(0, 1).contiguous() if time_major and ids.dim() == 2 else y


def embed(embedding, ids):
    if _plain_embedding(embedding, ids):
        return EmbedTanhFn.apply(ids, embedding.weight, False, False)
    return embedding(ids)


class NormLink:
    __slots__ = ("inv", "L", "lin", "xb")

    def __init__(self):
        self.inv, self.L, self.lin, self.xb = None, 0, None, None


class LinearFn(torch.autograd.Function):

    @staticmethod
    def forward(ctx, x, w, b, relu=False, bf16=False):
        x = _c(x)
        w2 = _w2d(w)
        bf16 = bool(bf16) and _bf16_ok(x.shape[0], x.shape[1], w2.shape[0])
        if bf16:
            xb, wb = ops.cast_bf16(x), ops.cast_bf16(w2)
            y = ops.gemm_bf16(xb, wb, bias=b, relu=relu)
            ctx.save_for_backward(xb, w, y if relu else None, wb)
        else:
            y = ops.gemm(x, w2, bias=b, relu=relu)
            ctx.save_for_backward(x, w, y if relu else None, None)
        ctx.has_bias = b is not None
        ctx.relu = relu
        ctx.bf16 = bf16
        return y

    @staticmethod
    def backward(ctx, dy):
        x, w, y, wb = ctx.saved_tensors
        w2 = _w2d(w)
        dy = _c(dy)
        db = None
        if ctx.relu:
            dy, db = ops.relu_bwd(dy, y, want_bias=ctx.has_bias)
        elif ctx.has_bias and ctx.needs_input_grad[2]:
            db = ops.colsum(dy)
        dx = dw = None
        if ctx.bf16:
            dyb = ops.cast_bf16(dy)
            if ctx.needs_input_grad[0]:
                dx = ops.gemm_bf16(dyb, wb, tb=True)
            if ctx.needs_input_grad[1]:
                dw = ops.gemm_bf16(dyb, x, ta=True, tb=True).view_as(w)
            return dx, dw, db, None, None
        if ctx.needs_input_grad[0]:
            dx = ops.gemm(dy, w2, tb=True)
        if ctx.needs_input_grad[1]:
            dw = ops.gemm(dy, x, ta=True, tb=True).view_as(w)
        return dx, dw, db, None, None


class Linear2Fn(torch.autograd.Function):

    @staticmethod
    def forward(ctx, x1, x2, w, b):
        x1, x2 = _c(x1), _c(x2)
        w2 = _w2d(w)
        K1 = x1.shape[1]
        y = ops.gemm(x1, w2[:, :K1], bias=b)
        ops.gemm(x2, w2[:, K1:], out=y, accumulate=True)
        ctx.save_for_backward(x1, x2, w)
        ctx.has_bias = b is not None
        return y

    @staticmethod
    def backward(ctx, dy):
        x1, x2, w = ctx.saved_tensors
        w2 = _w2d(w)
        dy = _c(dy)
        K1 = x1.shape[1]
        dx1 = ops.gemm(dy, w2[:, :K1], tb=True) if ctx.needs_input_grad[0] else None
        dx2 = ops.gemm(dy, w2[:, K1:], tb=True) if ctx.needs_input_grad[1] else None
        dw = None
        if ctx.needs_input_grad[2]:
            dw = torch.empty_like(w2)
            ops.gemm(dy, x1, ta=True, tb=True, out=dw[:, :K1])
            ops.gemm(dy, x2, ta=True, tb=True, out=dw[:, K1:])
            dw = dw.view_as(w)
        db = ops.colsum(dy) if (ctx.has_bias and ctx.needs_input_grad[3]) else None
        return dx1, dx2, dw, db


class JoinRowsFn(torch.autograd.Function):

    @staticmethod
    def forward(ctx, v, q, buf):
        n = v.shape[0]
        if v.data_ptr() != buf.data_ptr() or q.data_ptr() != buf[n:].data_ptr() or buf.shape[0] != n + q.shape[0]:
            raise ops._l.VqfError("JoinRowsFn: v and q must be the row blocks of buf")
        ctx.n = n
        return buf.view_as(buf)

    @staticmethod
    def backward(ctx, g):
        g = _c(g)
        return g[:ctx.n], g[ctx.n:], None


class AttHeadFn(torch.autograd.Function):

    @staticmethod
    def _pool_fwd(feat, logits, unit, grp, lens=None):
        if grp is None:
            return ops.glimpse_pool_fwd(feat, logits, unit, lens=lens)
        if unit:
            U, S, _ = feat.shape
            zeros = torch.zeros((U * S, logits.shape[1]), dtype=torch.float32, device=feat.device)
            _, per_image = ops.glimpse_pool_fwd(feat, zeros, True, lens=None if lens is None else lens[1])
            return None, ops.row_block_gather(per_image, grp[0])
        return ops.glimpse_pool_fwd_grouped(feat, logits, grp[0], lens=None if lens is None else lens[0])

    @staticmethod
    def _pool_bwd(dpooled, feat, wts, unit, need_dfeat, grp, NS, G, lens=None):
        if grp is None:
            return ops.glimpse_pool_bwd(dpooled, feat, wts, unit, need_dfeat, lens=lens)
        if need_dfeat:
            raise ops._l.VqfError("AttHeadFn: with shared images (grp) the feature tensor is data and gets no gradient")
        if unit:
            return torch.zeros((NS, G), dtype=torch.float32, device=dpooled.device), None
        return ops.glimpse_pool_bwd_grouped(dpooled, feat, wts, grp[0], grp[1], grp[2], False, lens=None if lens is None else lens[0])

    @staticmethod
    def forward(ctx, x, feat, w1, b1, wm, bm, w2, b2, unit_softmax, bf16=False, link=None, same_src=False, grp=None, lens=None):
        x = _c(x)
        feat = _c(feat)
        ctx.bf16 = bool(bf16)
        ctx.same_src = bool(same_src)
        ctx.grp = grp
        ctx.lens = lens
        if lens is not None and (ctx.bf16 or ctx.same_src or feat.dtype != torch.float32 or ctx.needs_input_grad[1]):
            raise ops._l.VqfError("AttHeadFn: region counts (lens) are fp32 only, for a feature tensor that is data")
        if grp is not None and (ctx.bf16 or ctx.same_src or feat.dtype != torch.float32):
            raise ops._l.VqfError("AttHeadFn: shared images (grp) are fp32 only and never the MLP's own source")
        if ctx.same_src and (x.numel() != feat.numel() or x.shape[-1] != feat.shape[-1] or x.dtype != feat.dtype):
            raise ops._l.VqfError("AttHeadFn: same_src needs x = feat.view(N*S, C)")
        ctx.link = link if (link is not None and link.inv is not None) else None
        if ctx.link is not None:
            if wm is not None or b1 is None:
                raise ops._l.VqfError("AttHeadFn: a NormLink needs the single-hidden-layer head with a bias")
            ctx.bf16 = ctx.bf16 and _bf16_ok(_w2d(w1).shape[0], _w2d(w1).shape[1])
            if ctx.bf16:
                w1b = ops.cast_bf16(_w2d(w1), 32)
                xb = link.xb if (link.xb is not None and link.xb.shape == (x.shape[0], w1b.shape[1])) else ops.cast_bf16(x, 32)
                link.xb = None
                hid1 = ops.gemm_bf16_rowscale(xb, w1b, link.inv, link.L, bias=b1, relu=True, K=xb.shape[1])
                x = xb
            else:
                hid1 = ops.gemm_rowscale(x, _w2d(w1), link.inv, link.L, bias=b1, relu=True)
            logits, lin = ops.att_logits_fwd_lin(hid1, _w2d(w2), b2, b1)
            wts, pooled = AttHeadFn._pool_fwd(feat, logits, unit_softmax, grp, lens)
            ctx.save_for_backward(x, feat, w1, w1b if ctx.bf16 else None, w2, hid1, None, wts, lin)
            ctx.unit = bool(unit_softmax)
            return pooled
        ctx.bf16 = ctx.bf16 and _bf16_ok(_w2d(w1).shape[0], _w2d(w1).shape[1])
        if ctx.bf16:
            xb, w1b = ops.cast_bf16(x, 32), ops.cast_bf16(_w2d(w1), 32)
            hid1 = ops.gemm_bf16(xb, w1b, K=xb.shape[1], bias=b1, relu=True)
            x = xb
        else:
            hid1 = ops.gemm(x, _w2d(w1), bias=b1, relu=True)
        hid2 = ops.gemm(hid1, _w2d(wm), bias=bm, relu=True) if wm is not None else None
        last = hid2 if hid2 is not None else hid1
        logits = ops.att_logits_fwd(last, _w2d(w2), b2)
        wts, pooled = AttHeadFn._pool_fwd(feat, logits, unit_softmax, grp, lens)
        ctx.save_for_backward(x, feat, w1, wm, w2, hid1, hid2, wts, w1b if ctx.bf16 else None)
        ctx.unit = bool(unit_softmax)
        return pooled

    @staticmethod
    def backward(ctx, dpooled):
        x, feat, w1, wm, w2, hid1, hid2, wts, lin = ctx.saved_tensors
        dpooled = _c(dpooled)
        need_dfeat = ctx.needs_input_grad[1]
        dlogits, dfeat = AttHeadFn._pool_bwd(dpooled, feat, wts, ctx.unit, need_dfeat, ctx.grp, hid1.shape[0], _w2d(w2).shape[0],
                                             ctx.lens)
        if ctx.link is not None:
            link = ctx.link
            w1b = wm
            obf = ctx.bf16 and hid1.shape[1] % 8 == 0 and w2.shape[0] == 2
            d1s, dw2, db2, db1 = ops.att_logits_bwd(dlogits, hid1, _w2d(w2), relu_mask=True, rowscale=link.inv,
                                                    rows_per_scale=link.L, out_bf16=obf)
            link.lin = (dlogits, lin)
            if ctx.bf16:
                cin = _w2d(w1).shape[1]
                d1b = d1s if obf else ops.cast_bf16(d1s)
                dw1 = ops.gemm_bf16(d1b, x, ta=True, tb=True)[:, :cin].contiguous().view_as(w1)
                dx = ops.gemm_bf16(d1b, w1b, tb=True, N=cin) if ctx.needs_input_grad[0] else None
                return dx, dfeat, dw1, db1, None, None, dw2.view_as(w2), db2, None, None, None, None, None, None
            dw1 = ops.gemm(d1s, x, ta=True, tb=True).view_as(w1)
            dx = ops.gemm(d1s, _w2d(w1), tb=True) if ctx.needs_input_grad[0] else None
            return dx, dfeat, dw1, db1, None, None, dw2.view_as(w2), db2, None, None, None, None, None, None
        last = hid2 if hid2 is not None else hid1
        dlast_pre, dw2, db2, dblast = ops.att_logits_bwd(dlogits, last, _w2d(w2), relu_mask=True)
        dwm = dbm = None
        if hid2 is not None:
            dwm = ops.gemm(dlast_pre, hid1, ta=True, tb=True).view_as(wm)
            dbm = dblast
            dhid1 = ops.gemm(dlast_pre, _w2d(wm), tb=True)
            d1_pre, db1 = ops.relu_bwd(dhid1, hid1, want_bias=True)
        else:
            d1_pre, db1 = dlast_pre, dblast
        if ctx.bf16:
            cin = _w2d(w1).shape[1]
            d1b = ops.cast_bf16(d1_pre)
            dw1 = ops.gemm_bf16(d1b, x, ta=True, tb=True)[:, :cin].contiguous().view_as(w1)
            dx = None
            if ctx.needs_input_grad[0]:
                dx = ops.gemm_bf16(d1b, lin, tb=True, N=cin)
        else:
            dw1 = ops.gemm(d1_pre, x, ta=True, tb=True).view_as(w1)
            if ctx.same_src and dfeat is not None:
                ops.gemm(d1_pre, _w2d(w1), tb=True, out=dfeat.view(x.shape), accumulate=True)
                dx = None
            else:
                dx = ops.gemm(d1_pre, _w2d(w1), tb=True) if ctx.needs_input_grad[0] else None
        return dx, dfeat, dw1, db1, dwm, dbm, dw2.view_as(w2), db2, None, None, None, None, None, None


def _arm_link(link, inv, L, xb=None):
    if link is not None:
        link.inv, link.L, link.lin, link.xb = inv, L, None, (xb[0] if xb else None)
    return link

# ... 137 lines not shown
    return P0, img2


class ImgProjLateFn(torch.autograd.Function):

    @staticmethod
    def forward(ctx, P0, img2, wi, cu_limit=0):
        ctx.save_for_backward(img2, wi)
        ctx.cu_limit = cu_limit
        return P0.view_as(P0)

    @staticmethod
    def backward(ctx, dP):
        img2, wi = ctx.saved_tensors
        dP = _c(dP)
        with (ops.options(gemm_cu_limit=ctx.cu_limit) if ctx.cu_limit else ops.options()):
            if img2.dtype == torch.bfloat16:
                dPb = dP if dP.dtype == torch.bfloat16 else ops.cast_bf16(dP)
                dwi = ops.gemm_bf16(dPb, img2, ta=True, tb=True).view_as(wi)
            else:
                dwi = ops.gemm(dP, img2, ta=True, tb=True).view_as(wi)
        return None, None, dwi, None


class MfbFuseFn(torch.autograd.Function):

    @staticmethod
    def forward(ctx, P0, bi, q, keep, seed, p_drop, N, L, link=None, grp=None, lens=None):
        P0, q = _c(P0), _c(q)
        O = P0.shape[1] // ops.POOL_K
        ctx.grp = grp
        ctx.lens = lens
        if lens is not None and P0.dtype != torch.float32:
            raise ops._l.VqfError("MfbFuseFn: region counts (lens) are fp32 only, got a %s projection" % P0.dtype)
        if grp is not None:
            if P0.dtype != torch.float32:
                raise ops._l.VqfError("MfbFuseFn: shared images (grp) are fp32 only, got a %s projection" % P0.dtype)
            U = P0.shape[0] // L
            Y, norm, inv = ops.mfb_fuse_fwd_grouped(P0, q, grp[0], N, U, L, O, keep=keep, seed=seed, p_drop=p_drop, pbias=bi,
                                                    normalise=link is None, lens=lens)
            ctx.link = _arm_link(link, inv, L, None)
            ctx.save_for_backward(P0, bi, q, Y, norm, inv, keep)
            ctx.seed, ctx.p_drop, ctx.dims = seed, p_drop, (N, L, O)
            return Y
        rb = [] if (link is not None and P0.dtype == torch.bfloat16) else None
        Y, norm, inv, _ = ops.mfb_fuse_fwd(P0, q, N, L, O, keep=keep, seed=seed, p_drop=p_drop, pbias=bi,
                                           normalise=link is None, r_bf16=rb, lens=lens)
        ctx.link = _arm_link(link, inv, L, rb)
        ctx.save_for_backward(P0, bi, q, Y, norm, inv, keep)
        ctx.seed, ctx.p_drop, ctx.dims = seed, p_drop, (N, L, O)
        return Y

    @staticmethod
    def backward(ctx, dY):
        P0, bi, q, Y, norm, inv, keep = ctx.saved_tensors
        N, L, O = ctx.dims
        if ctx.grp is not None:
            dP, dq, dbi = ops.mfb_fuse_bwd_grouped(_c(dY), Y, norm, inv, P0, q, ctx.grp[0], ctx.grp[1], ctx.grp[2], N,
                                                   P0.shape[0] // L, L, O, keep=keep, seed=ctx.seed, p_drop=ctx.p_drop,
                                                   want_dbias=True, pbias=bi, lin=_take_lin(ctx.link), lens=ctx.lens)
            return dP, dbi, dq, None, None, None, None, None, None, None, None
        dP, dq, _, dbi = ops.mfb_fuse_bwd(_c(dY), Y, norm, inv, P0, q, N, L, O, keep=keep, seed=ctx.seed,
                                          p_drop=ctx.p_drop, want_dbias=True, pbias=bi, lin=_take_lin(ctx.link),
                                          dp_bf16=P0.dtype == torch.bfloat16, lens=ctx.lens)
        return dP, dbi, dq, None, None, None, None, None, None, None, None


class _Fork:
    _streams = {}

    def __init__(self, device):
        self.cur = torch.cuda.current_stream(device)
        self.side = _Fork._streams.get(device)
        if self.side is None:
            self.side = _Fork._streams[device] = torch.cuda.Stream(device=device)
        self.side.wait_stream(self.cur)
        self._ctx = torch.cuda.stream(self.side)

    def __enter__(self):
        self._ctx.__enter__()
        return self

    def __exit__(self, *exc):
        return self._ctx.__exit__(*exc)

    def join(self, *tensors):
        self.cur.wait_stream(self.side)
        for t in tensors:
            if t is not None:
                t.record_stream(self.cur)


class FinalMfbFn(torch.autograd.Function):

    TWO_STREAMS = False

    @staticmethod
    def forward(ctx, qa, va, wq, bq, wv, bv, keep, seed, p_drop, cascade=None, want_zdrop=False, bf16=False):
        qa, va = _c(qa), _c(va)
        N = qa.shape[0]
        O = wq.shape[0] // ops.POOL_K
        wq2, wv2 = _w2d(wq), _w2d(wv)
        bf16 = bool(bf16) and _bf16_ok(N, qa.shape[1], va.shape[1], wq2.shape[0])
        if bf16:
            qa_s, va_s, wqb, wvb = ops.cast_bf16(qa), ops.cast_bf16(va), ops.cast_bf16(wq2), ops.cast_bf16(wv2)
            qq = ops.gemm_bf16(qa_s, wqb, bias=bq)
            vv = ops.gemm_bf16(va_s, wvb, bias=bv)
        elif FinalMfbFn.TWO_STREAMS:
            qa_s, va_s, wqb, wvb = qa, va, None, None
            with _Fork(qa.device) as f:
                vv = ops.gemm(va, wv2, bias=bv)
            qq = ops.gemm(qa, wq2, bias=bq)
            f.join(vv)
        else:
            qa_s, va_s, wqb, wvb = qa, va, None, None
            qq = ops.gemm(qa, wq2, bias=bq)
            vv = ops.gemm(va, wv2, bias=bv)
        if cascade is not None:
            cascade = _c(cascade)
        y, norm, inv, zdrop = ops.mfb_fuse_fwd(vv, qq, N, 1, O, keep=keep, seed=seed, p_drop=p_drop,
                                               cascade=cascade, want_zdrop=want_zdrop)
        ctx.save_for_backward(qa_s, va_s, wq, wv, qq, vv, y, norm, inv, keep, cascade, wqb, wvb)
        ctx.seed, ctx.p_drop, ctx.dims, ctx.bf16 = seed, p_drop, (N, O), bf16
        if want_zdrop:
            return y, zdrop
        return y

    @staticmethod
    def backward(ctx, dy, dz=None):
        qa, va, wq, wv, qq, vv, y, norm, inv, keep, cascade, wqb, wvb = ctx.saved_tensors
        N, O = ctx.dims
        dvv, dqq, dcasc, _ = ops.mfb_fuse_bwd(_c(dy), y, norm, inv, vv, qq, N, 1, O, keep=keep,
                                              seed=ctx.seed, p_drop=ctx.p_drop, cascade=cascade,
                                              dzdrop=None if dz is None else _c(dz))
        if ctx.bf16:
            dqb, dvb = ops.cast_bf16(dqq), ops.cast_bf16(dvv)
            dqa = ops.gemm_bf16(dqb, wqb, tb=True) if ctx.needs_input_grad[0] else None
            dva = ops.gemm_bf16(dvb, wvb, tb=True) if ctx.needs_input_grad[1] else None
            dwq = ops.gemm_bf16(dqb, qa, ta=True, tb=True).view_as(wq)
            dwv = ops.gemm_bf16(dvb, va, ta=True, tb=True).view_as(wv)
        elif FinalMfbFn.TWO_STREAMS:
            wq2, wv2 = _w2d(wq), _w2d(wv)
            with _Fork(dqq.device) as f:
                dva = ops.gemm(dvv, wv2, tb=True) if ctx.needs_input_grad[1] else None
                dwv = ops.gemm(dvv, va, ta=True, tb=True).view_as(wv)
                dbv = ops.colsum(dvv)
            dqa = ops.gemm(dqq, wq2, tb=True) if ctx.needs_input_grad[0] else None
            dwq = ops.gemm(dqq, qa, ta=True, tb=True).view_as(wq)
            dbq = ops.colsum(dqq)
            f.join(dva, dwv, dbv)
            return dqa, dva, dwq, dbq, dwv, dbv, None, None, None, dcasc, None, None
        else:
            wq2, wv2 = _w2d(wq), _w2d(wv)
            dqa = ops.gemm(dqq, wq2, tb=True) if ctx.needs_input_grad[0] else None
            dva = ops.gemm(dvv, wv2, tb=True) if ctx.needs_input_grad[1] else None
            dwq = ops.gemm(dqq, qa, ta=True, tb=True).view_as(wq)
            dwv = ops.gemm(dvv, va, ta=True, tb=True).view_as(wv)
        dbq = ops.colsum(dqq)
        dbv = ops.colsum(dvv)
        return dqa, dva, dwq, dbq, dwv, dbv, None, None, None, dcasc, None, None


class DropoutFn(torch.autograd.Function):

    @staticmethod
    def forward(ctx, x, keep, seed, p_drop):
        x = _c(x)
        ctx.keep, ctx.seed, ctx.p = keep, seed, p_drop
        return ops.dropout(x, keep=keep, seed=seed, p_drop=p_drop)

    @staticmethod
    def backward(ctx, dy):
        return ops.dropout(_c(dy), keep=ctx.keep, seed=ctx.seed, p_drop=ctx.p), None, None, None


class DropoutBTFn(torch.autograd.Function):

    @staticmethod
    def forward(ctx, x, keep, seed, p_drop, lens=None):
        ctx.keep, ctx.seed, ctx.p, ctx.lens = keep, seed, p_drop, lens
        ctx.in_strides = (x.stride(0), x.stride(1))
        return ops.dropout_bt(x, torch.empty(x.shape, dtype=torch.float32, device=x.device), keep, seed, p_drop, lens=lens)

    @staticmethod
    def backward(ctx, dy):
        B, T, H = dy.shape
        if dy.stride(2) != 1 or dy.stride(0) % 4 or dy.stride(1) % 4 or dy.data_ptr() % 16:
            dy = dy.contiguous()
        sb, st = ctx.in_strides
        if st > sb and sb == H and st == B * H:
            dx = torch.empty((T, B, H), dtype=torch.float32, device=dy.device).transpose(0, 1)
        else:
            dx = torch.empty((B, T, H), dtype=torch.float32, device=dy.device)
        ops.dropout_bt(dy, dx, ctx.keep, ctx.seed, ctx.p, lens=ctx.lens)
        return dx, None, None, None, None


def lstm_out_dropout(module, x, seeds, tag="l"):
    p = float(module.p) if module.training else 0.0
    keep = seeds.keep.get(tag)
    if x.dim() == 3 and x.is_cuda and x.dtype == torch.float32 and x.stride(2) == 1 and x.shape[2] % 4 == 0 \
            and all(s % 4 == 0 for s in x.stride()[:2]) and x.data_ptr() % 16 == 0:
        if p <= 0.0 and keep is None and x.is_contiguous():
            return x
        seed, pp = seeds.next(module.training, p)
        return DropoutBTFn.apply(x, keep, seed, p if keep is not None else pp)
    return module(x).contiguous()


class TanhDropFn(torch.autograd.Function):

    @staticmethod
    def forward(ctx, a, b, keep, seed, p_drop):
        a = _c(a)
        b = None if b is None else _c(b)
        y = ops.tanh_dropout_fwd(a, b, keep=keep, seed=seed, p_drop=p_drop)
        ctx.save_for_backward(y)
        ctx.keep, ctx.seed, ctx.p, ctx.has_b = keep, seed, p_drop, b is not None
        return y

    @staticmethod
    def backward(ctx, dy):
        (y,) = ctx.saved_tensors
        dx = ops.tanh_dropout_bwd(_c(dy), y, keep=ctx.keep, seed=ctx.seed, p_drop=ctx.p)
        return dx, (dx if ctx.has_b else None), None, None, None


class GateFn(torch.autograd.Function):

    @staticmethod
    def forward(ctx, a, b):
        a, b = _c(a), _c(b)
        ctx.save_for_backward(a, b)
        return ops.gate_tanh_sigmoid_fwd(a, b)

    @staticmethod
    def backward(ctx, dy):
        a, b = ctx.saved_tensors
        return ops.gate_tanh_sigmoid_bwd(_c(dy), a, b)


class BmmFn(torch.autograd.Function):

    @staticmethod
    def forward(ctx, a, b, ta, tb):
        a, b = _c(a), _c(b)
        ctx.save_for_backward(a, b)
        ctx.ta, ctx.tb = ta, tb
        return ops.bgemm(a, b, ta=ta, tb=tb)

    @staticmethod
    def backward(ctx, dc):
        a, b = ctx.saved_tensors
        dc = _c(dc)
        ta, tb = ctx.ta, ctx.tb
        da = db = None
        if ctx.needs_input_grad[0]:
            if not ta:
                da = ops.bgemm(dc, b, ta=False, tb=not tb)
            else:
                da = ops.bgemm(b, dc, ta=not tb, tb=False)
        if ctx.needs_input_grad[1]:
            if not tb:
                db = ops.bgemm(dc, a, ta=True, tb=not ta)
            else:
                db = ops.bgemm(a, dc, ta=not ta, tb=True)
        return da, db, None, None


class AttPoolFn(torch.autograd.Function):

    @staticmethod
    def forward(ctx, x, feat, w, b, pooled_out=None):
        x, feat = _c(x), _c(feat)
        w2 = _w2d(w)
        logits = ops.att_logits_fwd(x, w2, b)
        wts, pooled = ops.glimpse_pool_fwd(feat, logits, False, pooled_out=pooled_out)
        ctx.save_for_backward(x, feat, w, wts)
        return (pooled.view_as(pooled) if pooled_out is not None else pooled), wts

    @staticmethod
    def backward(ctx, dpooled, dwts):
        x, feat, w, wts = ctx.saved_tensors
        dlogits, dfeat = ops.glimpse_pool_bwd(_c(dpooled), feat, wts, False, ctx.needs_input_grad[1],
                                              dwts=None if dwts is None else _c(dwts))
        dx, dw, db, _ = ops.att_logits_bwd(dlogits, x, _w2d(w), relu_mask=False)
        return (dx if ctx.needs_input_grad[0] else None), dfeat, dw.view_as(w), db, None


def _hie_hv_ti(Vh, C, Qh, drop, N, L, T, Hv, ti, stream, rlens=None):
    E = Vh.shape[1]
    if stream:
        rk = {} if rlens is None else {"rlens": rlens}
        S = ops.hie_chunks(N, L)
        if S == 1:
            ops.hie_hv_fwd(Vh, C, Qh, drop, N, L, T, Hv, ti, **rk)
        else:
            part = torch.empty((S, N * T, E), dtype=torch.float32, device=Vh.device)
            ops.hie_hv_fwd(Vh, C, Qh, drop, N, L, T, Hv, part, **rk)
            ops.hie_slab_sum(part, ti)
    else:
        tq = ops.bgemm(C, Qh.view(N, T, E), ta=True, tb=True).view(N * L, E)
        ops.tanh_dropout_fwd2d(Vh, tq, *drop, out=Hv)
        ops.bgemm(C, Vh.view(N, L, E), ta=False, tb=True, out=ti.view(N, T, E))


def _hie_dc(dti, Vh, Qh, dtq, C, drop, N, L, T, aff, out=None, lens=None, rlens=None):
    if aff:
        rk = {} if rlens is None else {"rlens": rlens}
        return ops.hie_affinity(dti, Vh, N, L, T, x2=Qh, y2=dtq, epi=2, yprev=C, drop=drop, out=out, lens=lens, **rk)
# ... 135 lines not shown
    @staticmethod
    def forward(ctx, x):
        y = ops.softmax_rows_fwd(_c(x))
        ctx.save_for_backward(y)
        return y

    @staticmethod
    def backward(ctx, dy):
        (y,) = ctx.saved_tensors
        return ops.softmax_rows_bwd(_c(dy), y)


class LogSoftmaxRowsFn(torch.autograd.Function):

    @staticmethod
    def forward(ctx, x):
        y = ops.log_softmax_rows_fwd(_c(x))
        ctx.save_for_backward(y)
        return y

    @staticmethod
    def backward(ctx, dy):
        (y,) = ctx.saved_tensors
        return ops.log_softmax_rows_bwd(_c(dy), y)


def _bias_sum(b_ih, b_hh):
    if b_ih is None:
        return None
    if b_ih.is_cuda and b_ih.dtype == torch.float32 and b_ih.is_contiguous() and b_hh.is_contiguous():
        out = torch.empty_like(b_ih)
        ops.multi_add([(b_ih.detach(), b_hh.detach(), out)])
        return out
    return b_ih + b_hh


def _copy_of(t):
    if t is None:
        return None
    if t.is_cuda and t.dtype == torch.float32 and t.is_contiguous():
        out = torch.empty_like(t)
        ops.multi_copy([(t, out)])
        return out
    return t.clone()


def _lstm_in_proj(x2, w_ih, bias, bf16_proj):
    if not bf16_proj:
        return ops.gemm(x2, _c(w_ih), bias=bias), None, None
    xb, wb = ops.cast_bf16(x2), ops.cast_bf16(_c(w_ih))
    return ops.gemm_bf16(xb, wb, bias=bias), xb, wb


def _lstm_in_proj_bwd(dgb, xb, wb, I, need_dx):
    dx = ops.gemm_bf16(dgb, wb, tb=True)[:, :I].contiguous() if need_dx else None
    dw = ops.gemm_bf16(dgb, xb, ta=True, tb=True)[:, :I].contiguous()
    return dx, dw


class LstmSeqFn(torch.autograd.Function):

    @staticmethod
    def forward(ctx, x, w_ih, w_hh, b_ih, b_hh, bf16=False):
        x = _c(x)
        S, B, I = x.shape
        H = w_hh.shape[1]
        bias = _bias_sum(b_ih, b_hh)
        ctx.bf16 = bool(bf16)
        ctx.bf16_proj = bf16 == "all" and H % 8 == 0
        xw, xb, wb = _lstm_in_proj(x.view(S * B, I), w_ih, bias, ctx.bf16_proj)
        xw = xw.view(S, B, 4 * H)
        hs, cs, gates = ops.lstm_seq_fwd(xw, _c(w_hh), bf16=ctx.bf16)
        ctx.save_for_backward(x, w_ih, w_hh, hs, cs, gates, xb, wb)
        ctx.has_bias = b_ih is not None
        return hs

    @staticmethod
    def backward(ctx, dhs):
        x, w_ih, w_hh, hs, cs, gates, xb, wb = ctx.saved_tensors
        S, B, I = x.shape
        H = w_hh.shape[1]
        dg = ops.lstm_seq_bwd(_c(dhs), gates, cs, _c(w_hh), bf16=ctx.bf16)
        dg2 = dg.view(S * B, 4 * H)
        dgb = ops.cast_bf16(dg2) if ctx.bf16 and H % 8 == 0 else None
        if ctx.bf16_proj:
            dx, dw_ih = _lstm_in_proj_bwd(dgb, xb, wb, I, ctx.needs_input_grad[0])
            dx = dx.view(S, B, I) if dx is not None else None
        else:
            dx = ops.gemm(dg2, _c(w_ih), tb=True).view(S, B, I) if ctx.needs_input_grad[0] else None
            dw_ih = ops.gemm(dg2, x.view(S * B, I), ta=True, tb=True)
        if S > 1:
            if dgb is not None:
                dw_hh = ops.gemm_bf16(dgb[B:], ops.cast_bf16(hs[:-1].reshape((S - 1) * B, H)), ta=True, tb=True)
            else:
                dw_hh = ops.gemm(dg[1:].reshape((S - 1) * B, 4 * H), hs[:-1].reshape((S - 1) * B, H), ta=True, tb=True)
        else:
            dw_hh = torch.zeros_like(w_hh)
        db = ops.colsum(dg2) if ctx.has_bias else None
        return dx, dw_ih, dw_hh, db, _copy_of(db), None


class LstmBatchFn(torch.autograd.Function):

    FUSED_STEP = True

    @staticmethod
    def forward(ctx, x, w_ih, w_hh, b_ih, b_hh, bf16=False):
        x = _c(x)
        T, B, I = x.shape
        H = w_hh.shape[1]
        bias = _bias_sum(b_ih, b_hh)
        ctx.bf16 = bool(bf16) and H % 8 == 0
        ctx.bf16_proj = ctx.bf16 and bf16 == "all"
        whh = ops.cast_bf16(_c(w_hh)) if ctx.bf16 else _c(w_hh)
        gates, xb, wb = _lstm_in_proj(x.view(T * B, I), w_ih, bias, ctx.bf16_proj)
        gates = gates.view(T, B, 4 * H)
        hs = torch.empty((T, B, H), dtype=torch.float32, device=x.device)
        cs = torch.empty_like(hs)
        fused = LstmBatchFn.FUSED_STEP and not ctx.bf16 and ops.lstm_step_supported(B, H)
        for t in range(T):
            if t > 0 and fused:
                ops.lstm_step_fwd(hs[t - 1], whh, gates[t], cs[t - 1], cs[t], hs[t])
                continue
            if t > 0:
                if ctx.bf16:
                    ops.gemm_bf16(ops.cast_bf16(hs[t - 1]), whh, out=gates[t], accumulate=True)
                else:
                    ops.gemm(hs[t - 1], whh, out=gates[t], accumulate=True)
            ops.lstm_cell_fwd(gates[t], cs[t - 1] if t else None, cs[t], hs[t])
        ctx.save_for_backward(x, w_ih, w_hh, hs, cs, gates, xb, wb)
        ctx.has_bias = b_ih is not None
        return hs

    @staticmethod
    def backward(ctx, dhs):
        x, w_ih, w_hh, hs, cs, gates, xb, wb = ctx.saved_tensors
        T, B, I = x.shape
        H = w_hh.shape[1]
        dhs = _c(dhs)
        whh = ops.cast_bf16(_c(w_hh)) if ctx.bf16 else _c(w_hh)
        dG = torch.empty_like(gates)
        dc = torch.empty((B, H), dtype=torch.float32, device=x.device)
        dh = None
        for t in range(T - 1, -1, -1):
            ops.lstm_cell_bwd(dhs[t], dh, gates[t], cs[t], cs[t - 1] if t else None, t == T - 1, dc, dG[t])
            if t > 0:
                dh = ops.gemm_bf16(ops.cast_bf16(dG[t]), whh, tb=True) if ctx.bf16 else ops.gemm(dG[t], whh, tb=True)
        dG2 = dG.view(T * B, 4 * H)
        if ctx.bf16_proj:
            dGb = ops.cast_bf16(dG2)
            dx, dw_ih = _lstm_in_proj_bwd(dGb, xb, wb, I, ctx.needs_input_grad[0])
            dx = dx.view(T, B, I) if dx is not None else None
        else:
            dx = ops.gemm(dG2, _c(w_ih), tb=True).view(T, B, I) if ctx.needs_input_grad[0] else None
            dw_ih = ops.gemm(dG2, x.view(T * B, I), ta=True, tb=True)
        if T > 1 and ctx.bf16_proj and B % 8 == 0:
            dw_hh = ops.gemm_bf16(dGb[B:], ops.cast_bf16(hs[:-1].reshape((T - 1) * B, H)), ta=True, tb=True)
        elif T > 1:
            dw_hh = ops.gemm(dG[1:].reshape((T - 1) * B, 4 * H), hs[:-1].reshape((T - 1) * B, H), ta=True, tb=True)
        else:
            dw_hh = torch.zeros_like(w_hh)
        db = ops.colsum(dG2) if ctx.has_bias else None
        return dx, dw_ih, dw_hh, db, _copy_of(db), None


class UnitPoolFn(torch.autograd.Function):

    @staticmethod
    def forward(ctx, feat, G, lens=None):
        feat = _c(feat)
        N, S, C = feat.shape
        logits = torch.zeros((N * S, G), dtype=torch.float32, device=feat.device)
        wts, pooled = ops.glimpse_pool_fwd(feat, logits, True, lens=lens)
        ctx.save_for_backward(feat, wts)
        ctx.lens = lens
        return pooled

    @staticmethod
    def backward(ctx, dpooled):
        feat, wts = ctx.saved_tensors
        if not ctx.needs_input_grad[0]:
            return None, None, None
        _, dfeat = ops.glimpse_pool_bwd(_c(dpooled), feat, wts, True, True, lens=ctx.lens)
        return dfeat, None, None


class DeadParamsFn(torch.autograd.Function):

    @staticmethod
    def forward(ctx, out, *params):
        ctx.meta = [(p.shape, p.dtype, p.device) for p in params]
        return out.view_as(out)

    @staticmethod
    def backward(ctx, g):
        return (g,) + tuple(torch.zeros(sh, dtype=dt, device=dv) for sh, dt, dv in ctx.meta)
```

vqa-attention-networks_amd/host/lib.py:

```python
import ctypes
import os
import subprocess
import threading

_HERE = os.path.dirname(os.path.abspath(__file__))
PKG_DIR = os.path.dirname(_HERE)
CSRC_DIR = os.path.join(PKG_DIR, "csrc")
LIB_PATH = os.path.join(PKG_DIR, "libvqa_fusion.so")
if os.environ.get("VQF_LIB"):
    LIB_PATH = os.path.abspath(os.environ["VQF_LIB"])
HEADER_PATH = os.path.join(os.path.dirname(PKG_DIR), "include", "vqa_fusion.h")

ABI_VERSION = 7

_lock = threading.Lock()
_lib = None

c_f = ctypes.c_void_p
c_i = ctypes.c_int
c_sz = ctypes.c_size_t
c_u64 = ctypes.c_uint64
c_p = ctypes.c_void_p

SIGNATURES = {
    "vqf_abi_version": (c_i, []),
    "vqf_build_info": (ctypes.c_char_p, []),
    "vqf_set_option": (c_i, [c_i, c_i, ctypes.POINTER(c_i)]),
    "vqf_get_option": (c_i, [c_i, ctypes.POINTER(c_i)]),
    "vqf_option_env_name": (ctypes.c_char_p, [c_i]),
    "vqf_stat_get": (c_i, [c_i, ctypes.POINTER(ctypes.c_longlong)]),
    "vqf_gemm_f32_ws_bytes": (c_sz, [c_i, c_i, c_i, c_i, c_i]),
    "vqf_gemm_f32": (c_i, [c_i, c_i, c_i, c_i, c_i, c_f, c_i, c_f, c_i, c_f, c_i, c_f, c_i, c_p, c_sz, c_p]),
    "vqf_gemm_f32_big_rows": (c_i, [c_i, c_i, c_i, c_i, c_i]),
    "vqf_gemm_f32_sample_supported": (c_i, [c_i, c_i, c_i, c_i]),
    "vqf_gemm_f32_sample": (c_i, [c_i, c_i, c_i, c_i, c_i, c_f, c_i, c_f, c_i, c_f, c_i, c_f, c_i, c_p]),
    "vqf_gemm_f32_rowscale": (c_i, [c_i, c_i, c_i, c_i, c_i, c_f, c_i, c_f, c_i, c_f, c_i, c_f, c_i, c_f, c_i, c_p]),
    "vqf_gemm_f32_batched": (c_i, [c_i, c_i, c_i, c_i, c_i, c_i, c_f, c_i, ctypes.c_longlong,
                                   c_f, c_i, ctypes.c_longlong, c_f, c_i, ctypes.c_longlong, c_i, c_p]),
    "vqf_gemm_bf16_ws_bytes": (c_sz, [c_i, c_i, c_i, c_i, c_i]),
    "vqf_gemm_bf16": (c_i, [c_i, c_i, c_i, c_i, c_i, c_p, c_i, c_p, c_i, c_f, c_i, c_f, c_i, c_p, c_sz, c_p]),
    "vqf_gemm_bf16_rowscale": (c_i, [c_i, c_i, c_i, c_i, c_i, c_p, c_i, c_p, c_i, c_f, c_i, c_f, c_i, c_f, c_i, c_p]),
    "vqf_cast_f32_bf16": (c_i, [c_f, c_i, c_i, c_i, c_p, c_i, c_p]),
    "vqf_colsum_ws_bytes": (c_sz, [c_i, c_i]),
    "vqf_colsum_f32": (c_i, [c_f, c_i, c_i, c_i, c_f, c_p, c_sz, c_p]),
    "vqf_group_reduce_f32": (c_i, [c_f, c_i, c_i, c_i, c_f, c_p]),
    "vqf_relu_bwd_f32": (c_i, [c_f, c_f, c_i, c_i, c_f, c_f, c_p, c_sz, c_p]),
    "vqf_att_logits_fwd": (c_i, [c_f, c_f, c_f, c_i, c_i, c_i, c_f, c_p]),
    "vqf_att_logits_fwd_lin": (c_i, [c_f, c_f, c_f, c_f, c_i, c_i, c_i, c_f, c_f, c_p]),
    "vqf_att_logits_bwd_ws_bytes": (c_sz, [c_i, c_i]),
    "vqf_att_logits_bwd_rowscale": (c_i, [c_f, c_f, c_f, c_f, c_i, c_i, c_i, c_i, c_i, c_f, c_f, c_f, c_f, c_p, c_sz, c_p]),
    "vqf_att_logits_bwd_rowscale_obf16": (c_i, [c_f, c_f, c_f, c_f, c_i, c_i, c_i, c_i, c_p, c_f, c_f, c_f, c_p, c_sz, c_p]),
    "vqf_att_logits_bwd": (c_i, [c_f, c_f, c_f, c_i, c_i, c_i, c_i, c_f, c_f, c_f, c_f, c_p, c_sz, c_p]),
    "vqf_glimpse_pool_fwd": (c_i, [c_f, c_f, c_i, c_i, c_i, c_i, c_i, c_f, c_f, c_p]),
    "vqf_glimpse_pool_bwd": (c_i, [c_f, c_f, c_f, c_f, c_i, c_i, c_i, c_i, c_i, c_f, c_f, c_p]),
    "vqf_glimpse_pool_fwd_bf16": (c_i, [c_p, c_f, c_i, c_i, c_i, c_i, c_i, c_f, c_f, c_p]),
    "vqf_glimpse_pool_bwd_bf16": (c_i, [c_f, c_f, c_p, c_f, c_i, c_i, c_i, c_i, c_i, c_f, c_p]),
    "vqf_dropout_f32": (c_i, [c_f, c_p, c_u64, ctypes.c_float, ctypes.c_longlong, c_f, c_p]),
    "vqf_dropout_bt": (c_i, [c_f, ctypes.c_longlong, ctypes.c_longlong, c_p, c_u64, ctypes.c_float, c_i, c_i, c_i, c_f,
                             ctypes.c_longlong, ctypes.c_longlong, c_p]),
    "vqf_gate_tanh_sigmoid_fwd": (c_i, [c_f, c_f, ctypes.c_longlong, c_f, c_p]),
    "vqf_gate_tanh_sigmoid_bwd": (c_i, [c_f, c_f, c_f, ctypes.c_longlong, c_f, c_f, c_p]),
    "vqf_tanh_dropout_fwd": (c_i, [c_f, c_f, c_p, c_u64, ctypes.c_float, ctypes.c_longlong, c_f, c_p]),
    "vqf_tanh_dropout_bwd": (c_i, [c_f, c_f, c_p, c_u64, ctypes.c_float, ctypes.c_longlong, c_f, c_p]),
    "vqf_tanh_dropout_fwd2d": (c_i, [c_f, c_i, c_f, c_i, c_p, c_u64, ctypes.c_float, c_i, c_i, c_f, c_i, c_p]),
    "vqf_tanh_dropout_bwd2d": (c_i, [c_f, c_i, c_f, c_i, c_p, c_u64, ctypes.c_float, c_i, c_i, c_f, c_i, c_p]),
    "vqf_relu_bwd_rank1_f32": (c_i, [c_f, c_f, c_f, c_f, c_i, ctypes.c_float, c_i, c_i, c_f, c_f, c_p, c_sz, c_p]),
    "vqf_multi_add_f32": (c_i, [c_p, c_p, c_p, c_p, c_i, c_p]),
    "vqf_multi_copy_f32": (c_i, [c_p, c_p, c_p, c_i, c_p]),
    "vqf_hie_stream_supported": (c_i, [c_i, c_i, c_i, c_i]),
    "vqf_hie_chunks": (c_i, [c_i, c_i]),
    "vqf_hie_hv_fwd": (c_i, [c_f, c_i, c_f, c_f, c_i, c_p, c_u64, ctypes.c_float, c_i, c_i, c_i, c_i, c_f, c_i, c_f, c_i, c_p]),
    "vqf_hie_head_bwd": (c_i, [c_f, c_i, c_f, c_f, c_f, c_p, c_u64, ctypes.c_float, c_i, c_i, c_i, c_i, c_f, c_i, c_f, c_i, c_f, c_i,
                               c_f, c_i, c_p]),
    "vqf_hie_rank_add": (c_i, [c_f, c_i, c_f, c_f, c_i, c_i, c_i, c_i, c_i, c_f, c_i, c_f, c_i, c_p]),
    "vqf_hie_rank_left": (c_i, [c_f, c_f, c_i, c_f, c_i, c_i, c_i, c_i, c_i, c_f, c_i, c_f, c_i, c_f, c_i, c_p]),
    "vqf_hie_slab_sum": (c_i, [c_f, c_i, c_i, c_i, c_f, c_i, c_f, c_i, c_p]),
    "vqf_hie_affinity_supported": (c_i, [c_i, c_i, c_i, c_i, c_i]),
    "vqf_hie_affinity": (c_i, [c_f, c_i, c_f, c_i, c_f, c_i, c_f, c_i, c_i, c_f, c_p, c_u64, ctypes.c_float, c_i, c_i, c_i, c_i, c_f, c_p]),
    "vqf_phrase_ngram_supported": (c_i, [c_i, c_i]),
    "vqf_phrase_ngram_fwd": (c_i, [c_f, c_i, c_f, c_i, c_i, c_i, c_f, c_i, c_p, c_p]),
    "vqf_phrase_ngram_bwd": (c_i, [c_f, c_i, c_f, c_i, c_p, c_i, c_i, c_i, c_f, c_i, c_p]),
    "vqf_hie_affinity_levels_supported": (c_i, [c_i, c_i, c_i, c_i, c_i, c_i]),
    "vqf_hie_affinity_levels": (c_i, [c_f, c_i, c_i, c_f, c_i, c_i, c_f, c_i, c_i, c_f, c_i, c_i, c_i, c_i, c_f, c_i, c_i, c_i, c_i,
                                      c_f, c_p]),
    "vqf_embed_tanh_fwd_len": (c_i, [c_f, c_p, c_p, c_i, c_i, c_i, c_i, c_f, c_p]),
    "vqf_embed_tanh_bwd_len": (c_i, [c_f, c_f, c_p, c_p, c_i, c_i, c_i, c_i, c_f, c_p]),
    "vqf_phrase_ngram_fwd_len": (c_i, [c_f, c_i, c_f, c_p, c_i, c_i, c_i, c_f, c_i, c_p, c_p]),
    "vqf_phrase_ngram_bwd_len": (c_i, [c_f, c_i, c_f, c_i, c_p, c_p, c_i, c_i, c_i, c_f, c_i, c_p]),
    "vqf_dropout_bt_len": (c_i, [c_f, ctypes.c_longlong, ctypes.c_longlong, c_p, c_u64, ctypes.c_float, c_p, c_i, c_i, c_i, c_f,
                                 ctypes.c_longlong, ctypes.c_longlong, c_p]),
    "vqf_glimpse_pool_fwd_len": (c_i, [c_f, c_f, c_p, c_i, c_i, c_i, c_i, c_i, c_f, c_f, c_p]),
    "vqf_glimpse_pool_bwd_len": (c_i, [c_f, c_f, c_f, c_f, c_p, c_i, c_i, c_i, c_i, c_i, c_f, c_f, c_p]),
    "vqf_hie_affinity_len": (c_i, [c_f, c_i, c_f, c_i, c_f, c_i, c_f, c_i, c_i, c_f, c_p, c_u64, ctypes.c_float, c_p, c_i, c_i, c_i,
                                   c_i, c_f, c_p]),
    "vqf_hie_affinity_levels_len": (c_i, [c_f, c_i, c_i, c_f, c_i, c_i, c_f, c_i, c_i, c_f, c_i, c_i, c_i, c_i, c_f, c_p, c_i, c_i,
                                          c_i, c_i, c_f, c_p]),
    "vqf_tanh_bwd_rows_len": (c_i, [c_f, c_f, c_p, c_i, c_i, c_i, c_f, c_p]),
    "vqf_hie_affinity_regions": (c_i, [c_f, c_i, c_f, c_i, c_f, c_i, c_f, c_i, c_i, c_f, c_p, c_u64, ctypes.c_float, c_p, c_p, c_i,
                                       c_i, c_i, c_i, c_f, c_p]),
    "vqf_hie_affinity_levels_regions": (c_i, [c_f, c_i, c_i, c_f, c_i, c_i, c_f, c_i, c_i, c_f, c_i, c_i, c_i, c_i, c_f, c_p, c_p,
                                              c_i, c_i, c_i, c_i, c_f, c_p]),
    "vqf_hie_hv_fwd_regions": (c_i, [c_f, c_i, c_f, c_f, c_i, c_p, c_u64, ctypes.c_float, c_p, c_i, c_i, c_i, c_i, c_f, c_i, c_f, c_i,
                                     c_f, c_i, c_p]),
    "vqf_hie_rank_add_regions": (c_i, [c_f, c_i, c_f, c_f, c_i, c_p, c_i, c_i, c_i, c_i, c_f, c_i, c_f, c_i, c_p]),
    "vqf_hie_rank_left_regions": (c_i, [c_f, c_f, c_i, c_f, c_i, c_p, c_i, c_i, c_i, c_i, c_f, c_i, c_f, c_i, c_f, c_i, c_f, c_i,
                                        c_p]),
    "vqf_zero_cols_len": (c_i, [c_f, c_p, ctypes.c_longlong, c_i, c_i, c_i, c_p]),
    "vqf_guided_logits_supported": (c_i, [c_i, c_i, c_i, c_i]),
    "vqf_guided_logits_fwd": (c_i, [c_f, c_i, c_f, c_f, c_i, c_i, c_i, c_i, c_f, c_p]),
    "vqf_guided_logits_bwd_ws_bytes": (c_sz, [c_i, c_i, c_i, c_i]),
    "vqf_guided_logits_bwd": (c_i, [c_f, c_f, c_i, c_f, c_f, c_i, c_i, c_i, c_i, c_f, c_i, c_f, c_f, c_p, c_sz, c_p]),
    "vqf_guided_logits_grouped_supported": (c_i, [c_i, c_i, c_i, c_i, c_i]),
    "vqf_guided_logits_fwd_grouped": (c_i, [c_f, c_i, c_f, c_f, c_p, c_i, c_i, c_i, c_i, c_i, c_f, c_p]),
    "vqf_guided_logits_bwd_grouped_ws_bytes": (c_sz, [c_i, c_i, c_i, c_i, c_i]),
    "vqf_guided_logits_bwd_grouped": (c_i, [c_f, c_f, c_i, c_f, c_f, c_p, c_p, c_i, c_i, c_i, c_i, c_i, c_f, c_i, c_f, c_f, c_p, c_sz,
                                            c_p]),
    "vqf_glimpse_pool_grouped_supported": (c_i, [c_i, c_i, c_i, c_i, c_i]),
    "vqf_glimpse_pool_fwd_grouped": (c_i, [c_f, c_f, c_p, c_i, c_i, c_i, c_i, c_i, c_f, c_f, c_p]),
    "vqf_glimpse_pool_bwd_grouped": (c_i, [c_f, c_f, c_f, c_f, c_p, c_p, c_p, c_i, c_i, c_i, c_i, c_i, c_f, c_f, c_p]),
    "vqf_row_block_supported": (c_i, [c_i, c_i, ctypes.c_longlong]),
    "vqf_row_block_gather": (c_i, [c_f, c_p, c_i, c_i, ctypes.c_longlong, c_f, c_p]),
    "vqf_row_block_group_sum": (c_i, [c_f, c_p, c_p, c_i, c_i, ctypes.c_longlong, c_f, c_p]),
    "vqf_softmax_rows_fwd": (c_i, [c_f, c_i, c_i, c_f, c_p]),
    "vqf_softmax_rows_bwd": (c_i, [c_f, c_f, c_i, c_i, c_f, c_p]),
    "vqf_log_softmax_rows_fwd": (c_i, [c_f, c_i, c_i, c_f, c_p]),
    "vqf_log_softmax_rows_bwd": (c_i, [c_f, c_f, c_i, c_i, c_f, c_p]),
    "vqf_mfb_fuse_fwd": (c_i, [c_f, c_f, c_f, c_f, c_p, c_u64, ctypes.c_float, c_i, c_i, c_i, c_f, c_f, c_f, c_p]),
    "vqf_l2_group_norm": (c_i, [c_f, c_i, c_i, c_f, c_f, c_p]),
    "vqf_scale_rows": (c_i, [c_f, c_f, c_i, c_i, c_i, c_f, c_p]),
    "vqf_rowdot": (c_i, [c_f, c_f, c_i, c_i, c_f, c_p]),
    "vqf_l2_norm_bwd_coef": (c_i, [c_f, c_f, c_f, c_i, c_i, c_f, c_f, c_p]),
    "vqf_l2_norm_bwd_coef_lin": (c_i, [c_f, c_f, c_i, c_f, c_f, c_i, c_i, c_f, c_f, c_f, c_p]),
    "vqf_mfb_fuse_bwd_ws_bytes": (c_sz, [c_i, c_i, c_i]),
    "vqf_mfb_fuse_bwd": (c_i, [c_f, c_f, c_f, c_f, c_f, c_f, c_f, c_f, c_f, c_f, c_p, c_u64, ctypes.c_float,
                               c_i, c_i, c_i, c_f, c_f, c_f, c_f, c_p, c_sz, c_p]),
    "vqf_mfb_fuse_fwd_pbf16": (c_i, [c_p, c_f, c_f, c_p, c_u64, ctypes.c_float, c_i, c_i, c_i, c_f, c_f, c_p]),
    "vqf_mfb_fuse_fwd_pbf16_rb": (c_i, [c_p, c_f, c_f, c_p, c_u64, ctypes.c_float, c_i, c_i, c_i, c_f, c_p, c_i, c_f, c_p]),
    "vqf_mfb_fuse_bwd_pbf16": (c_i, [c_f, c_f, c_f, c_f, c_f, c_p, c_f, c_f, c_p, c_u64, ctypes.c_float,
                                     c_i, c_i, c_i, c_p, c_f, c_f, c_p, c_sz, c_p]),
    "vqf_mfb_fuse_bwd_bf16dp": (c_i, [c_f, c_f, c_f, c_f, c_f, c_f, c_f, c_f, c_p, c_u64, ctypes.c_float,
                                      c_i, c_i, c_i, c_p, c_f, c_f, c_p, c_sz, c_p]),
    "vqf_mfb_fuse_grouped_supported": (c_i, [c_i, c_i, c_i, c_i]),
    "vqf_mfb_fuse_fwd_grouped": (c_i, [c_f, c_f, c_f, c_p, c_p, c_u64, ctypes.c_float, c_i, c_i, c_i, c_i, c_f, c_f, c_p]),
    "vqf_mfb_fuse_bwd_grouped_ws_bytes": (c_sz, [c_i, c_i, c_i, c_i]),
    "vqf_mfb_fuse_bwd_grouped": (c_i, [c_f, c_f, c_f, c_f, c_f, c_f, c_f, c_f, c_p, c_p, c_p, c_p, c_u64, ctypes.c_float,
                                       c_i, c_i, c_i, c_i, c_f, c_f, c_f, c_p, c_sz, c_p]),
    "vqf_mfb_fuse_fwd_len": (c_i, [c_f, c_f, c_f, c_p, c_p, c_u64, ctypes.c_float, c_i, c_i, c_i, c_f, c_f, c_p]),
    "vqf_mfb_fuse_bwd_len": (c_i, [c_f, c_f, c_f, c_f, c_f, c_f, c_f, c_f, c_p, c_p, c_u64, ctypes.c_float,
                                   c_i, c_i, c_i, c_f, c_f, c_f, c_p, c_sz, c_p]),
    "vqf_mfb_fuse_fwd_grouped_len": (c_i, [c_f, c_f, c_f, c_p, c_p, c_p, c_p, c_u64, ctypes.c_float, c_i, c_i, c_i, c_i, c_f, c_f,
                                           c_p]),
    "vqf_mfb_fuse_bwd_grouped_len": (c_i, [c_f, c_f, c_f, c_f, c_f, c_f, c_f, c_f, c_p, c_p, c_p, c_p, c_p, c_p, c_u64, ctypes.c_float,
                                           c_i, c_i, c_i, c_i, c_f, c_f, c_f, c_p, c_sz, c_p]),
    "vqf_glimpse_pool_fwd_grouped_len": (c_i, [c_f, c_f, c_p, c_p, c_i, c_i, c_i, c_i, c_i, c_f, c_f, c_p]),
    "vqf_glimpse_pool_bwd_grouped_len": (c_i, [c_f, c_f, c_f, c_f, c_p, c_p, c_p, c_p, c_i, c_i, c_i, c_i, c_i, c_f, c_f, c_p]),
    "vqf_lstm_seq_supported": (c_i, [c_i, c_i]),
    "vqf_lstm_seq_ws_bytes": (c_sz, [c_i, c_i]),
    "vqf_lstm_seq_fwd": (c_i, [c_f, c_f, c_i, c_i, c_i, c_f, c_f, c_f, c_i, c_p, c_sz, c_p]),
    "vqf_lstm_seq_bwd": (c_i, [c_f, c_f, c_f, c_f, c_i, c_i, c_i, c_f, c_f, c_i, c_p, c_sz, c_p]),
    "vqf_lstm_cell_fwd": (c_i, [c_f, c_f, c_i, c_i, c_f, c_f, c_p]),
    "vqf_lstm_step_supported": (c_i, [c_i, c_i]),
    "vqf_lstm_step_fwd": (c_i, [c_f, c_f, c_f, c_f, c_i, c_i, c_f, c_f, c_p]),
    "vqf_lstm_cell_bwd": (c_i, [c_f, c_f, c_f, c_f, c_f, c_i, c_i, c_i, c_f, c_f, c_p]),
    "vqf_embed_tanh_fwd": (c_i, [c_f, c_p, c_i, c_i, c_i, c_f, c_p]),
    "vqf_embed_tanh_bwd": (c_i, [c_f, c_f, c_p, c_i, c_i, c_i, c_f, c_p]),
    "vqf_embed_fwd": (c_i, [c_f, c_p, c_i, c_i, c_i, c_f, c_p]),
    "vqf_embed_bwd": (c_i, [c_f, c_p, c_i, c_i, c_i, c_f, c_p]),
    "vqf_embed_dropout_fwd": (c_i, [c_f, c_p, c_i, c_i, c_i, c_p, c_u64, ctypes.c_float, c_f, c_p]),
    "vqf_embed_dropout_bwd": (c_i, [c_f, c_p, c_i, c_i, c_i, c_p, c_u64, ctypes.c_float, c_f, c_p]),
    "vqf_embed_tanh_fwd_tm": (c_i, [c_f, c_p, c_i, c_i, c_i, c_i, c_f, c_p]),
    "vqf_embed_tanh_bwd_tm": (c_i, [c_f, c_f, c_p, c_i, c_i, c_i, c_i, c_f, c_p]),
    "vqf_feat_transpose": (c_i, [c_f, c_i, c_i, c_i, c_i, c_p, c_p]),
    "vqf_loss_ws_bytes": (c_sz, [c_i, c_i]),
    "vqf_ce_loss": (c_i, [c_f, c_p, c_i, c_i, c_f, c_f, c_p, c_sz, c_p]),
    "vqf_kldiv_loss": (c_i, [c_f, c_f, c_i, c_i, c_f, c_f, c_p, c_sz, c_p]),
    "vqf_ce_loss_pred": (c_i, [c_f, c_p, c_i, c_i, c_f, c_f, c_p, c_p, c_p, c_f, c_i, c_p, c_sz, c_p]),
    "vqf_answer_match_rows": (c_i, [c_f, c_f, c_i, c_i, c_p, c_p, c_f, c_p, c_p, c_f, c_p, c_f, c_i, c_p, c_sz, c_p]),
    "vqf_topk_rows_supported": (c_i, [c_i, c_i]),
    "vqf_topk_rows": (c_i, [c_f, c_i, c_i, c_i, c_i, c_i, c_p, c_f, c_p]),
    "vqf_adam_step": (c_i, [c_p, c_i, ctypes.c_double, ctypes.c_double, ctypes.c_double, ctypes.c_double,
                            ctypes.c_double, ctypes.c_longlong, c_p]),
    "vqf_hbm_copy": (c_i, [c_p, c_p, ctypes.c_longlong, c_i, c_p]),
    "vqf_hbm_read_sweep_blocks": (c_i, [ctypes.c_longlong]),
    "vqf_hbm_read_sweep": (c_i, [c_p, ctypes.c_longlong, c_i, c_f, c_p]),
    "vqf_prof_enable": (None, [c_i]),
# ... 72 lines not shown
```

vqa-attention-networks_amd/host/ops.py:

```python
import ctypes
import math
import torch

from . import lib as _l

GEMM_RELU = 1
GEMM_ACCUM = 2
POOL_K = 5


def _lib():
    return _l.load()


def _stream():
    return ctypes.c_void_p(torch.cuda.current_stream().cuda_stream)


def _ptr(t):
    return ctypes.c_void_p(t.data_ptr()) if t is not None else ctypes.c_void_p(0)


def _chk(*ts):
    for t in ts:
        if t is None:
            continue
        if not t.is_cuda:
            raise _l.VqfError("vqa fusion ops need GPU tensors (HIP extension is the only path; "
                              "no CPU fallback)")
        if t.dtype != torch.float32:
            raise _l.VqfError("fp32 tensor expected, got %s" % t.dtype)
        if not t.is_contiguous():
            raise _l.VqfError("contiguous tensor expected")


class _Workspace:

    def __init__(self):
        self.bufs = {}

    def get(self, device, nbytes):
        nbytes = max(int(nbytes), 256)
        key = (device, torch.cuda.current_stream(device).cuda_stream)
        b = self.bufs.get(key)
        if b is None or b.numel() < nbytes:
            b = torch.empty(int(nbytes * 1.25) + 1024, dtype=torch.uint8, device=device)
            self.bufs[key] = b
        return b


_ws = _Workspace()
SPLITK_WS_BYTES = 192 << 20


def workspace(device, nbytes):
    return _ws.get(device, nbytes)


OPTIONS = {"gemm_f32_persist": 0, "gemm_bf16_persist": 1, "gemm_f32_loop": 2, "gemm_bf16_loop": 3, "gemm_f32_big": 4,
           "gemm_bf16_big": 5, "gemm_f32_wave": 6, "fuse_coal": 7, "fuse_ls": 8, "fuse_ls_bwd": 9, "gemm_cu_limit": 10,
           "gemm_f32_edge": 11, "gemm_f32_rounds": 12, "gemm_splitk_fused": 13, "gemm_f32_streamk": 14,
           "gemm_splitk_order": 15, "gemm_f32_sample": 16, "gemm_f32_n80": 17}


def set_option(name, value):
    prev = ctypes.c_int(0)
    _l.check(_lib().vqf_set_option(OPTIONS[name], -1 if value is None else int(value), ctypes.byref(prev)),
             "vqf_set_option(%s)" % name)
    return prev.value


def get_option(name):
    v = ctypes.c_int(0)
    _l.check(_lib().vqf_get_option(OPTIONS[name], ctypes.byref(v)), "vqf_get_option(%s)" % name)
    return v.value


STATS = {"gemm_f32_tile128": 0, "gemm_f32_big": 1, "gemm_f32_wave": 2, "gemm_bf16_tile128": 3, "gemm_bf16_big": 4,
         "gemm_f32_sample": 5, "gemm_f32_n80": 6}


def stat(name):
    v = ctypes.c_longlong(0)
    _l.check(_lib().vqf_stat_get(STATS[name], ctypes.byref(v)), "vqf_stat_get(%s)" % name)
    return v.value


class options:

    def __init__(self, **kw):
        self.kw, self.prev = kw, {}

    def __enter__(self):
        for k, v in self.kw.items():
            self.prev[k] = set_option(k, v)
        return self

    def __exit__(self, *exc):
        for k, v in self.prev.items():
            set_option(k, v)
        return False


def gemm(a, b, ta=False, tb=False, bias=None, relu=False, out=None, accumulate=False,
         M=None, N=None, K=None, splitk=True):
    _chk(bias)
    for t in (a, b, out):
        if t is None:
            continue
        if not t.is_cuda or t.dtype != torch.float32 or t.dim() != 2 or t.stride(1) != 1:
            raise _l.VqfError("gemm: 2-D fp32 GPU tensors with contiguous rows expected")
    if M is None:
        M = a.shape[1] if ta else a.shape[0]
    if K is None:
        K = a.shape[0] if ta else a.shape[1]
        kb = b.shape[0] if tb else b.shape[1]
        if kb != K:
            raise _l.VqfError("gemm: inner dimensions differ (%d vs %d)" % (K, kb))
    if N is None:
        N = b.shape[1] if tb else b.shape[0]
    if out is None:
        if accumulate:
            raise _l.VqfError("gemm: accumulate needs out")
        out = torch.empty((M, N), dtype=torch.float32, device=a.device)
    flags = (GEMM_RELU if relu else 0) | (GEMM_ACCUM if accumulate else 0)
    ws = None
    if splitk:
        ws = workspace(a.device, max(SPLITK_WS_BYTES, int(_lib().vqf_gemm_f32_ws_bytes(int(ta), int(tb), M, N, K))))
    rc = _lib().vqf_gemm_f32(int(ta), int(tb), M, N, K, _ptr(a), a.stride(0), _ptr(b), b.stride(0),
                             _ptr(out), out.stride(0), _ptr(bias), flags,
                             _ptr(ws), ws.numel() if ws is not None else 0, _stream())
    _l.check(rc, "vqf_gemm_f32")
    return out


def gemm_rows(a, b, L, tb=False, bias=None, relu=False, out=None):
    M, K = a.shape
    N = b.shape[1] if tb else b.shape[0]
    ok = (L > 0 and M % L == 0 and a.is_cuda and a.dtype == torch.float32 and b.dtype == torch.float32 and a.dim() == 2 and b.dim() == 2
          and a.stride(1) == 1 and b.stride(1) == 1 and (b.shape[0] if tb else b.shape[1]) == K
          and _lib().vqf_gemm_f32_sample_supported(M // L, L, N, K)
          and a.data_ptr() % 16 == 0 and b.data_ptr() % 16 == 0 and a.stride(0) % 4 == 0 and b.stride(0) % 4 == 0)
    if out is not None:
        ok = ok and out.dtype == torch.float32 and out.dim() == 2 and out.stride(1) == 1 and out.stride(0) % 2 == 0 and out.data_ptr() % 8 == 0
    if not ok:
        return gemm(a, b, tb=tb, bias=bias, relu=relu, out=out)
    _chk(bias)
    if out is None:
        out = torch.empty((M, N), dtype=torch.float32, device=a.device)
    _l.check(_lib().vqf_gemm_f32_sample(int(bool(tb)), M // L, int(L), N, K, _ptr(a), a.stride(0), _ptr(b), b.stride(0), _ptr(out),
                                        out.stride(0), _ptr(bias), GEMM_RELU if relu else 0, _stream()), "vqf_gemm_f32_sample")
    return out


def gemm_rows_supported(NS, L, N, K):
    return bool(_lib().vqf_gemm_f32_sample_supported(int(NS), int(L), int(N), int(K)))


def gemm_big_rows(ta, tb, M, N, K):
    return int(_lib().vqf_gemm_f32_big_rows(int(bool(ta)), int(bool(tb)), int(M), int(N), int(K)))


def gemm_rowscale(a, b, rowscale, rows_per_scale, bias=None, relu=False):
    _chk(a, b, rowscale, bias)
    M, K = a.shape
    N = b.shape[0]
    if b.shape[1] != K or rowscale.numel() * rows_per_scale < M:
        raise _l.VqfError("gemm_rowscale: shape mismatch")
    out = torch.empty((M, N), dtype=torch.float32, device=a.device)
    _l.check(_lib().vqf_gemm_f32_rowscale(0, 0, M, N, K, _ptr(a), a.stride(0), _ptr(b), b.stride(0), _ptr(out), N,
                                          _ptr(bias), GEMM_RELU if relu else 0, _ptr(rowscale), int(rows_per_scale),
                                          _stream()), "vqf_gemm_f32_rowscale")
    return out


def _chk_bf16(*ts):
    for t in ts:
        if not t.is_cuda or t.dtype != torch.bfloat16 or t.stride(-1) != 1:
            raise _l.VqfError("bf16 GPU tensor with contiguous rows expected")


def cast_bf16(x, pad_to=8):
    _chk(x)
    R, C = x.shape
    Cp = (C + pad_to - 1) // pad_to * pad_to
    y = torch.empty((R, Cp), dtype=torch.bfloat16, device=x.device)
    _l.check(_lib().vqf_cast_f32_bf16(_ptr(x), R, C, x.stride(0), _ptr(y), Cp, _stream()), "vqf_cast_f32_bf16")
    return y


GEMM_OUT_BF16 = 4


def gemm_bf16(a, b, ta=False, tb=False, bias=None, relu=False, M=None, N=None, K=None, out=None,
              accumulate=False, out_bf16=False):
    _chk_bf16(a, b)
    _chk(bias)
    if out is not None:
        want = torch.bfloat16 if out_bf16 else torch.float32
        if not out.is_cuda or out.dtype != want or out.dim() != 2 or out.stride(1) != 1:
            raise _l.VqfError("gemm_bf16: out must be a 2-D %s GPU tensor with contiguous rows" % want)
    if M is None:
        M = a.shape[1] if ta else a.shape[0]
    if K is None:
        K = a.shape[0] if ta else a.shape[1]
    if N is None:
        N = b.shape[1] if tb else b.shape[0]
    if out is None:
        out = torch.empty((M, N), dtype=torch.bfloat16 if out_bf16 else torch.float32, device=a.device)
    flags = (GEMM_RELU if relu else 0) | (GEMM_ACCUM if accumulate else 0) | (GEMM_OUT_BF16 if out_bf16 else 0)
    ws = workspace(a.device, max(SPLITK_WS_BYTES, int(_lib().vqf_gemm_bf16_ws_bytes(int(ta), int(tb), M, N, K))))
    rc = _lib().vqf_gemm_bf16(int(ta), int(tb), M, N, K, _ptr(a), a.stride(0), _ptr(b), b.stride(0),
                              _ptr(out), out.stride(0), _ptr(bias), flags, _ptr(ws), ws.numel(), _stream())
    if out_bf16 and rc == -3:
        return None
    _l.check(rc, "vqf_gemm_bf16")
    return out


def gemm_bf16_rowscale(a, b, rowscale, rows_per_scale, bias=None, relu=False, K=None):
    _chk_bf16(a, b)
    _chk(rowscale, bias)
    M, N = a.shape[0], b.shape[0]
    if K is None:
        K = a.shape[1]
    if b.shape[1] < K or a.shape[1] < K or rowscale.numel() * rows_per_scale < M:
        raise _l.VqfError("gemm_bf16_rowscale: shape mismatch")
    out = torch.empty((M, N), dtype=torch.float32, device=a.device)
    _l.check(_lib().vqf_gemm_bf16_rowscale(0, 0, M, N, K, _ptr(a), a.stride(0), _ptr(b), b.stride(0), _ptr(out), N, _ptr(bias),
                                           GEMM_RELU if relu else 0, _ptr(rowscale), int(rows_per_scale), _stream()),
             "vqf_gemm_bf16_rowscale")
    return out


def _chk3(*ts):
    for t in ts:
        if t is None:
            continue
        if not t.is_cuda or t.dtype != torch.float32 or t.dim() != 3 or t.stride(2) != 1:
            raise _l.VqfError("bgemm: 3-D fp32 GPU tensors with a contiguous innermost dimension expected")


def bgemm(a, b, ta=False, tb=False, out=None, accumulate=False):
    _chk3(a, b, out)
    Bn = a.shape[0]
    M = a.shape[2] if ta else a.shape[1]
    K = a.shape[1] if ta else a.shape[2]
    N = b.shape[2] if tb else b.shape[1]
    kb = b.shape[1] if tb else b.shape[2]
    if kb != K or b.shape[0] != Bn:
        raise _l.VqfError("bgemm: shape mismatch")
    if out is None:
        out = torch.empty((Bn, M, N), dtype=torch.float32, device=a.device)
    rc = _lib().vqf_gemm_f32_batched(int(ta), int(tb), Bn, M, N, K, _ptr(a), a.stride(1), a.stride(0),
                                     _ptr(b), b.stride(1), b.stride(0), _ptr(out), out.stride(1),
                                     out.stride(0), GEMM_ACCUM if accumulate else 0, _stream())
    _l.check(rc, "vqf_gemm_f32_batched")
    return out


def colsum(x):
    _chk(x)
    M, N = x.shape
    out = torch.empty(N, dtype=torch.float32, device=x.device)
    need = _lib().vqf_colsum_ws_bytes(M, N)
    ws = workspace(x.device, need)
    _l.check(_lib().vqf_colsum_f32(_ptr(x), M, N, x.stride(0), _ptr(out), _ptr(ws), ws.numel(), _stream()),
             "vqf_colsum_f32")
    return out


def relu_bwd(dx, y, want_bias=True):
    _chk(dx, y)
    M, C = y.shape
    dpre = torch.empty_like(y)
    db = torch.empty(C, dtype=torch.float32, device=y.device) if want_bias else None
    ws = workspace(y.device, _lib().vqf_colsum_ws_bytes(M, C))
    _l.check(_lib().vqf_relu_bwd_f32(_ptr(dx), _ptr(y), M, C, _ptr(dpre), _ptr(db), _ptr(ws), ws.numel(),
                                     _stream()), "vqf_relu_bwd_f32")
    return dpre, db


def att_logits_fwd(hid, w2, b2):
    _chk(hid, w2, b2)
    M, Hh = hid.shape
    G = w2.shape[0]
# ... 1221 lines not shown
```

Before: 12850.

## Group independent backward fp32 GEMMs into a single multi-problem kernel launch

Adds a grouped fp32 GEMM entry point that packs up to four independent GEMM problems (such as dx and dW in linear, bilinear, MFB and LSTM backward) into one launch. Each problem gets its own split-K plan and workspace slab, followed by one grouped split-K reduce. The goal is to fill the GPU when each individual GEMM has too few tiles and to cut launch overhead. Problems suited to the specialised big, wave or n80 paths are still routed to solo calls. The costs are a larger combined workspace and a kernel that dispatches at runtime across eight transpose/loader template variants.

```diff
diff --git a/include/vqa_fusion.h b/include/vqa_fusion.h
--- a/include/vqa_fusion.h
+++ b/include/vqa_fusion.h
@@ -42,7 +42,8 @@
 #define VQF_OPT_GEMM_SPLITK_ORDER 15
 #define VQF_OPT_GEMM_F32_SAMPLE 16
 #define VQF_OPT_GEMM_F32_N80 17
-#define VQF_OPT_COUNT 18
+#define VQF_OPT_GEMM_F32_GROUP 18
+#define VQF_OPT_COUNT 19
 int vqf_set_option(int option, int value, int* previous);
 int vqf_get_option(int option, int* value);
 const char* vqf_option_env_name(int option);
@@ -54,7 +55,8 @@
 #define VQF_STAT_GEMM_BF16_BIG 4
 #define VQF_STAT_GEMM_F32_SAMPLE 5
 #define VQF_STAT_GEMM_F32_N80 6
-#define VQF_STAT_COUNT 7
+#define VQF_STAT_GEMM_F32_GROUP 7
+#define VQF_STAT_COUNT 8
 int vqf_stat_get(int stat, long long* value);
 
 size_t vqf_gemm_f32_ws_bytes(int ta, int tb, int M, int N, int K);
@@ -62,6 +64,17 @@
                  const float* A, int lda, const float* B, int ldb,
                  float* C, int ldc, const float* bias, int flags,
                  void* ws, size_t ws_bytes, void* stream);
+
+typedef struct VqfGemmDesc {
+  int ta, tb, M, N, K;
+  const float* A; int lda;
+  const float* B; int ldb;
+  float* C; int ldc;
+  const float* bias;
+  int flags;
+} VqfGemmDesc;
+size_t vqf_gemm_f32_group_ws_bytes(int count, const VqfGemmDesc* descs);
+int vqf_gemm_f32_group(int count, const VqfGemmDesc* descs, void* ws, size_t ws_bytes, void* stream);
 
 int vqf_gemm_f32_rowscale(int ta, int tb, int M, int N, int K, const float* A, int lda, const float* B, int ldb,
                           float* C, int ldc, const float* bias, int flags, const float* rowscale, int rows_per_scale,
diff --git a/vqa-attention-networks_amd/csrc/common.h b/vqa-attention-networks_amd/csrc/common.h
--- a/vqa-attention-networks_amd/csrc/common.h
+++ b/vqa-attention-networks_amd/csrc/common.h
@@ -66,6 +66,7 @@
   KID_ROW_BLOCK_GROUP_SUM,
   KID_MFB_FUSE_BWD_IMAGE,
   KID_ZERO_COLS,
+  KID_GEMM_GROUP,
   KID_COUNT
 };
 
@@ -105,10 +106,13 @@
 size_t vqf_gemm_f32_big_ws_bytes(int ta, int tb, int M, int N, int K);
 int vqf_gemm_f32_n80_try(int M, int N, int K, const float* A, int lda, const float* B, int ldb, float* C, int ldc,
                          const float* bias, int flags, hipStream_t s, int* rc);
+int vqf_gemm_f32_n80_applies(int M, int N, int K, const float* A, int lda, const float* B, int ldb, int flags);
 int vqf_lstm_step16_try(const float* h_prev, const float* w_hh, float* gates, const float* c_prev, int B, int H, float* c_out,
                         float* h_out, hipStream_t s, int* rc);
 int vqf_gemm_f32_wave_try(int ta, int tb, int M, int N, int K, const float* A, int lda, const float* B, int ldb, float* C,
                           int ldc, const float* bias, int flags, hipStream_t s, int* rc);
+
+int vqf_gemm_f32_wave_applies(int ta, int tb, int M, int N, int K, const float* A, int lda, const float* B, int ldb);
 
 static inline int vqf_last_error() {
   hipError_t e = hipGetLastError();
diff --git a/vqa-attention-networks_amd/csrc/gemm_f32.hip b/vqa-attention-networks_amd/csrc/gemm_f32.hip
--- a/vqa-attention-networks_amd/csrc/gemm_f32.hip
+++ b/vqa-attention-networks_amd/csrc/gemm_f32.hip
@@ -1,4 +1,5 @@
 #include "common.h"
+#include "gemm_group_plan.h"
 #include <atomic>
 
 namespace {
@@ -321,15 +322,13 @@
 }
 
 template <bool TA, bool TB, bool FAST>
-__global__ void __launch_bounds__(NTHREADS, VQF_GEMM_WAVES_PER_SIMD) gemm_f32_kernel(GemmArgs g) {
-  extern __shared__ __attribute__((aligned(16))) float smem[];
+__device__ __forceinline__ void gemm_tile_body(const GemmArgs& g, float* smem, int bid, int ks, int zb, int nsplits) {
   const int tid = threadIdx.x, lane = tid & 63;
   const int wave = __builtin_amdgcn_readfirstlane(tid >> 6);
   const int wr = wave >> 1, wc = wave & 1;
   const int l31 = lane & 31, h = lane >> 5;
 
   const int nwg = g.tiles_m * g.tiles_n;
-  const int bid = blockIdx.x;
   const int q8 = nwg >> 3, r8 = nwg & 7, xcd = bid & 7;
   const int wg = (xcd < r8 ? xcd * (q8 + 1) : r8 * (q8 + 1) + (xcd - r8) * q8) + (bid >> 3);
   constexpr int GROUP_M = 8;
@@ -340,7 +339,7 @@
   const int in_g = wg - gid * per_group;
   const int tm = first_m + in_g % gsz, tn = in_g / gsz;
   const int m0 = tm * BM, n0 = tn * BN;
-  const int kbeg = blockIdx.y * g.kchunk;
+  const int kbeg = ks * g.kchunk;
   const int kend = min(g.K, kbeg + g.kchunk);
 
   f32x16 acc[2][2];
@@ -351,8 +350,8 @@
 #pragma unroll
       for (int r = 0; r < 16; ++r) acc[i][j][r] = 0.f;
 
-  const float* gA = g.A + (long long)blockIdx.z * g.sA;
-  const float* gB = g.B + (long long)blockIdx.z * g.sB;
+  const float* gA = g.A + (long long)zb * g.sA;
+  const float* gB = g.B + (long long)zb * g.sB;
   const bool all_valid = (m0 + wr * 64 + 32) < g.M && (n0 + wc * 64 + 32) < g.N;
   if (all_valid)
     gemm_mainloop<TA, TB, FAST, false>(g, smem, gA, gB, m0, n0, kbeg, kend, tid, wr, wc, l31, h, acc);
@@ -360,8 +359,8 @@
     gemm_mainloop<TA, TB, FAST, true>(g, smem, gA, gB, m0, n0, kbeg, kend, tid, wr, wc, l31, h, acc);
 
   const bool to_slab = g.slab != nullptr;
-  float* out = to_slab ? g.slab + (long long)blockIdx.y * g.M * g.N
-                       : g.C + (long long)blockIdx.z * g.sC;
+  float* out = to_slab ? g.slab + (long long)ks * g.M * g.N
+                       : g.C + (long long)zb * g.sC;
   const int ldo = to_slab ? g.N : g.ldc;
 #pragma unroll
   for (int j = 0; j < 2; ++j) {
@@ -390,16 +389,49 @@
   }
   if (to_slab && g.cnt) {
     const VqfSplitkTile st = {g.cnt, g.slab, g.C, g.bias, g.M, g.N, g.ldc, g.flags};
-    vqf_splitk_combine<BM, BN, NTHREADS, VQF_SPLITK_WT != 0>(st, bid, (int)gridDim.y, m0, n0, tid, smem);
-  }
-}
-
-__global__ void splitk_reduce_kernel(const float* __restrict__ slab, int splits, int M, int N,
-                                     float* __restrict__ C, int ldc, const float* __restrict__ bias,
-                                     int flags) {
+    vqf_splitk_combine<BM, BN, NTHREADS, VQF_SPLITK_WT != 0>(st, bid, nsplits, m0, n0, tid, smem);
+  }
+}
+
+template <bool TA, bool TB, bool FAST>
+__global__ void __launch_bounds__(NTHREADS, VQF_GEMM_WAVES_PER_SIMD) gemm_f32_kernel(GemmArgs g) {
+  extern __shared__ __attribute__((aligned(16))) float smem[];
+  gemm_tile_body<TA, TB, FAST>(g, smem, (int)blockIdx.x, (int)blockIdx.y, (int)blockIdx.z, (int)gridDim.y);
+}
+
+struct GroupArgs {
+  GemmArgs g[VQF_GROUP_MAX];
+  int end[VQF_GROUP_MAX];
+  int form[VQF_GROUP_MAX];
+};
+
+__global__ void __launch_bounds__(NTHREADS, VQF_GEMM_WAVES_PER_SIMD) gemm_f32_group_kernel(GroupArgs ga) {
+  extern __shared__ __attribute__((aligned(16))) float smem[];
+  const int b = (int)blockIdx.x;
+  const int p = (b >= ga.end[0] ? 1 : 0) + (b >= ga.end[1] ? 1 : 0) + (b >= ga.end[2] ? 1 : 0);
+  const int first = p > 0 ? ga.end[p - 1] : 0;
+  const GemmArgs& g = ga.g[p];
+  const int nwg = g.tiles_m * g.tiles_n;
+  const int local = b - first;
+  const int ks = local / nwg, bid = local - ks * nwg;
+  const int nsplits = (g.K + g.kchunk - 1) / g.kchunk;
+  switch (ga.form[p]) {
+    case 0: gemm_tile_body<false, false, false>(g, smem, bid, ks, 0, nsplits); break;
+    case 1: gemm_tile_body<false, false, true>(g, smem, bid, ks, 0, nsplits); break;
+    case 2: gemm_tile_body<false, true, false>(g, smem, bid, ks, 0, nsplits); break;
+    case 3: gemm_tile_body<false, true, true>(g, smem, bid, ks, 0, nsplits); break;
+    case 4: gemm_tile_body<true, false, false>(g, smem, bid, ks, 0, nsplits); break;
+    case 5: gemm_tile_body<true, false, true>(g, smem, bid, ks, 0, nsplits); break;
+    case 6: gemm_tile_body<true, true, false>(g, smem, bid, ks, 0, nsplits); break;
+    default: gemm_tile_body<true, true, true>(g, smem, bid, ks, 0, nsplits); break;
+  }
+}
+
+__device__ __forceinline__ void splitk_reduce_body(const float* __restrict__ slab, int splits, int M, int N, float* __restrict__ C,
+                                                   int ldc, const float* __restrict__ bias, int flags, int blk, int nblk) {
   const long long total = (long long)M * N;
-  const long long stride = (long long)gridDim.x * blockDim.x;
-  for (long long i = (long long)blockIdx.x * blockDim.x + threadIdx.x; i < total; i += stride) {
+  const long long stride = (long long)nblk * blockDim.x;
+  for (long long i = (long long)blk * blockDim.x + threadIdx.x; i < total; i += stride) {
     const int row = (int)(i / N), col = (int)(i - (long long)row * N);
     float v = 0.f;
     for (int z = 0; z < splits; ++z) v += slab[(long long)z * total + i];
@@ -411,6 +443,26 @@
   }
 }
 
+__global__ void splitk_reduce_kernel(const float* __restrict__ slab, int splits, int M, int N,
+                                     float* __restrict__ C, int ldc, const float* __restrict__ bias,
+                                     int flags) {
+  splitk_reduce_body(slab, splits, M, N, C, ldc, bias, flags, (int)blockIdx.x, (int)gridDim.x);
+}
+
+struct GroupReduceArgs {
+  const float* slab[VQF_GROUP_MAX];
+  float* C[VQF_GROUP_MAX];
+  const float* bias[VQF_GROUP_MAX];
+  int splits[VQF_GROUP_MAX], M[VQF_GROUP_MAX], N[VQF_GROUP_MAX], ldc[VQF_GROUP_MAX], flags[VQF_GROUP_MAX];
+  int end[VQF_GROUP_MAX];
+};
+__global__ void splitk_reduce_group_kernel(GroupReduceArgs r) {
+  const int b = (int)blockIdx.x;
+  const int p = (b >= r.end[0] ? 1 : 0) + (b >= r.end[1] ? 1 : 0) + (b >= r.end[2] ? 1 : 0);
+  const int first = p > 0 ? r.end[p - 1] : 0;
+  splitk_reduce_body(r.slab[p], r.splits[p], r.M[p], r.N[p], r.C[p], r.ldc[p], r.bias[p], r.flags[p], b - first, r.end[p] - first);
+}
+
 template <bool TA, bool TB, bool FAST>
 int launch_gemm_impl(const GemmArgs& g, dim3 grid, hipStream_t s, int kid) {
   static VqfDynLdsFlags attr = {};
@@ -419,11 +471,15 @@
   return vqf_last_error();
 }
 
+bool fast_loaders_ok(const GemmArgs& g, bool ta, bool tb) {
+  const bool okA = g.vecA && (!ta || (g.M % 4 == 0 && g.M >= 4));
+  const bool okB = g.vecB && (!tb || (g.N % 4 == 0 && g.N >= 4));
+  return okA && okB;
+}
+
 template <bool TA, bool TB>
 int launch_gemm(const GemmArgs& g, dim3 grid, hipStream_t s, int kid) {
-  const bool okA = g.vecA && (!TA || (g.M % 4 == 0 && g.M >= 4));
-  const bool okB = g.vecB && (!TB || (g.N % 4 == 0 && g.N >= 4));
-  if (okA && okB) return launch_gemm_impl<TA, TB, true>(g, grid, s, kid);
+  if (fast_loaders_ok(g, TA, TB)) return launch_gemm_impl<TA, TB, true>(g, grid, s, kid);
   return launch_gemm_impl<TA, TB, false>(g, grid, s, kid);
 }
 
@@ -514,9 +570,8 @@
   return gemm_tile128(ta, tb, M, N, K, A, lda, B, ldb, C, ldc, bias, flags, rowscale, rows_per_scale, row0, nullptr, 0, s);
 }
 
-static int gemm_tile128(int ta, int tb, int M, int N, int K, const float* A, int lda, const float* B, int ldb, float* C,
-                        int ldc, const float* bias, int flags, const float* rowscale, int rps, int row0, void* ws,
-                        size_t ws_bytes, hipStream_t s) {
+static GemmArgs tile128_args(int M, int N, int K, const float* A, int lda, const float* B, int ldb, float* C, int ldc,
+                             const float* bias, int flags, const float* rowscale, int rps, int row0) {
   GemmArgs g;
   g.A = A; g.B = B; g.C = C; g.bias = bias; g.slab = nullptr;
   g.M = M; g.N = N; g.K = K; g.lda = lda; g.ldb = ldb; g.ldc = ldc; g.flags = flags;
@@ -526,25 +581,16 @@
   g.tiles_n = (N + BN - 1) / BN;
   g.vecA = aligned16(A) && (lda % 4 == 0);
   g.vecB = aligned16(B) && (ldb % 4 == 0);
-
+  g.kchunk = ((K + BK - 1) / BK) * BK;
+  return g;
+}
+
+static int gemm_tile128(int ta, int tb, int M, int N, int K, const float* A, int lda, const float* B, int ldb, float* C,
+                        int ldc, const float* bias, int flags, const float* rowscale, int rps, int row0, void* ws,
+                        size_t ws_bytes, hipStream_t s) {
+  GemmArgs g = tile128_args(M, N, K, A, lda, B, ldb, C, ldc, bias, flags, rowscale, rps, row0);
   const long long tiles = (long long)g.tiles_m * g.tiles_n;
-  const int ktiles = (K + BK - 1) / BK;
-  int splits = 1;
-  const int slots = 512;
-  if (ws && tiles < 1024 && ktiles >= 32 && !(tiles >= 512 && K <= 1024) && !(tiles >= 192 && tiles <= 256 && K <= 512)) {
-    double best = 1e30;
-    for (int sp = 1; sp <= 16; ++sp) {
-      if (ktiles / sp < 16) break;
-      if ((size_t)sp * M * N * sizeof(float) > ws_bytes) break;
-      const double blocks = (double)tiles * sp;
-      const double rounds = (double)((long long)((blocks + slots - 1) / slots));
-      const double cost = rounds / sp * (1.0 + 0.01 * sp);
-      if (cost < best - 1e-12) { best = cost; splits = sp; }
-    }
-  }
-  int kt_per = (ktiles + splits - 1) / splits;
-  g.kchunk = kt_per * BK;
-  splits = (K + g.kchunk - 1) / g.kchunk;
+  const int splits = vqf_tile128_split(M, N, K, BK, ws != nullptr, ws_bytes, &g.kchunk);
   if (splits > 1) {
     g.slab = (float*)ws;
     if (vqf_opt(VQF_OPT_GEMM_SPLITK_FUSED, 0) == 1) g.cnt = vqf_splitk_counters((int)tiles);
@@ -565,6 +611,81 @@
   }
   if (splits > 1 && !g.cnt) rc = vqf_splitk_reduce((const float*)ws, splits, M, N, C, ldc, bias, flags, s);
   return rc;
+}
+
+static int group_other_family(const VqfGemmDesc* d, const void* ws, size_t ws_bytes) {
+  if (!(aligned16(d->A) && aligned16(d->B) && (d->lda % 4 == 0) && (d->ldb % 4 == 0))) return 0;
+  const size_t ws_ok = (ws && aligned16(ws)) ? ws_bytes : 0;
+  if (vqf_gemm_f32_big_rows_impl(d->ta, d->tb, d->M, d->N, d->K, d->flags, ws_ok) > 0) return 1;
+  if (vqf_gemm_f32_wave_applies(d->ta, d->tb, d->M, d->N, d->K, d->A, d->lda, d->B, d->ldb)) return 1;
+  if (!d->ta && !d->tb && vqf_gemm_f32_n80_applies(d->M, d->N, d->K, d->A, d->lda, d->B, d->ldb, d->flags)) return 1;
+  return 0;
+}
+
+static int gemm_solo(const VqfGemmDesc& d, void* ws, size_t ws_bytes, void* stream) {
+  return vqf_gemm_f32(d.ta, d.tb, d.M, d.N, d.K, d.A, d.lda, d.B, d.ldb, d.C, d.ldc, d.bias, d.flags, ws, ws_bytes, stream);
+}
+
+extern "C" size_t vqf_gemm_f32_group_ws_bytes(int count, const VqfGemmDesc* descs) {
+  if (count < 1 || count > VQF_GROUP_MAX || !descs) return 0;
+  size_t sum = 0, solo = 0;
+  for (int i = 0; i < count; ++i) {
+    const VqfGemmDesc& d = descs[i];
+    if (!vqf_gemm_desc_ok(d)) return 0;
+    int kchunk = 0;
+    const int sp = vqf_tile128_split(d.M, d.N, d.K, BK, true, (size_t)1 << 40, &kchunk);
+    if (sp > 1) sum += (size_t)sp * d.M * d.N * sizeof(float) + VQF_GROUP_WS_ALIGN;
+    const size_t own = vqf_gemm_f32_ws_bytes(d.ta, d.tb, d.M, d.N, d.K);
+    if (own > solo) solo = own;
+  }
+  return sum > solo ? sum : solo;
+}
+
+extern "C" int vqf_gemm_f32_group(int count, const VqfGemmDesc* descs, void* ws, size_t ws_bytes, void* stream) {
+  VqfGroupPlan plan;
+  const bool grouping = vqf_opt(VQF_OPT_GEMM_F32_GROUP, 1) != 0;
+  if (int e = vqf_gemm_group_plan(count, descs, ws, ws_bytes, BK, grouping, group_other_family, &plan)) return e;
+  hipStream_t s = (hipStream_t)stream;
+  if (plan.n_grouped > 0) {
+    GroupArgs ga;
+    GroupReduceArgs ra;
+    int nr = 0;
+    for (int i = 0; i < VQF_GROUP_MAX; ++i) {
+      const VqfGroupMember& m = plan.m[i < plan.n_grouped ? i : plan.n_grouped - 1];
+      const VqfGemmDesc& d = descs[m.desc];
+      GemmArgs g = tile128_args(d.M, d.N, d.K, d.A, d.lda, d.B, d.ldb, d.C, d.ldc, d.bias, d.flags, nullptr, 1, 0);
+      g.kchunk = m.kchunk;
+      if (m.splits > 1) g.slab = (float*)((char*)ws + m.slab_off);
+      ga.g[i] = g;
+      ga.end[i] = i < plan.n_grouped ? m.block_end : plan.total_blocks;
+      ga.form[i] = 4 * (d.ta ? 1 : 0) + 2 * (d.tb ? 1 : 0) + (fast_loaders_ok(g, d.ta != 0, d.tb != 0) ? 1 : 0);
+      if (i < plan.n_grouped && m.splits > 1) {
+        ra.slab[nr] = g.slab; ra.C[nr] = d.C; ra.bias[nr] = d.bias;
+        ra.splits[nr] = m.splits; ra.M[nr] = d.M; ra.N[nr] = d.N; ra.ldc[nr] = d.ldc; ra.flags[nr] = d.flags;
+        ra.end[nr] = m.reduce_end;
+        ++nr;
+      }
+    }
+    for (int i = nr; i < VQF_GROUP_MAX; ++i) {
+      ra.slab[i] = nullptr; ra.C[i] = nullptr; ra.bias[i] = nullptr;
+      ra.splits[i] = 0; ra.M[i] = 0; ra.N[i] = 1; ra.ldc[i] = 0; ra.flags[i] = 0;
+      ra.end[i] = plan.reduce_total;
+    }
+    static VqfDynLdsFlags attr = {};
+    if (int e = vqf_set_dyn_lds(reinterpret_cast<const void*>(&gemm_f32_group_kernel), SMEM_BYTES, attr)) return e;
+    const VqfGemmDesc& d0 = descs[plan.m[0].desc];
+    if (g_vqf_prof_on) vqf_prof_dims(d0.M, d0.N, d0.K);
+    vqf_stat_bump(VQF_STAT_GEMM_F32_GROUP);
+    VQF_LAUNCH(KID_GEMM_GROUP, gemm_f32_group_kernel, dim3((unsigned)plan.total_blocks), dim3(NTHREADS), SMEM_BYTES, s, ga);
+    if (int e = vqf_last_error()) return e;
+    if (nr > 0) {
+      VQF_LAUNCH(KID_SPLITK_REDUCE, splitk_reduce_group_kernel, dim3((unsigned)plan.reduce_total), dim3(256), 0, s, ra);
+      if (int e = vqf_last_error()) return e;
+    }
+  }
+  for (int i = 0; i < plan.n_solo; ++i)
+    if (int e = gemm_solo(descs[plan.solo[i]], ws, ws_bytes, stream)) return e;
+  return VQF_OK;
 }
 
 extern "C" int vqf_gemm_f32_batched(int ta, int tb, int batch, int M, int N, int K, const float* A,
diff --git a/vqa-attention-networks_amd/csrc/gemm_f32_n80.hip b/vqa-attention-networks_amd/csrc/gemm_f32_n80.hip
--- a/vqa-attention-networks_amd/csrc/gemm_f32_n80.hip
+++ b/vqa-attention-networks_amd/csrc/gemm_f32_n80.hip
@@ -179,8 +179,7 @@
 
 }
 
-int vqf_gemm_f32_n80_try(int M, int N, int K, const float* A, int lda, const float* B, int ldb, float* C, int ldc,
-                         const float* bias, int flags, hipStream_t s, int* rc) {
+int vqf_gemm_f32_n80_applies(int M, int N, int K, const float* A, int lda, const float* B, int ldb, int flags) {
   if (vqf_opt(VQF_OPT_GEMM_F32_N80, 1) == 0) return 0;
   if ((flags & ~VQF_GEMM_RELU) || (K % 128) || K < 512 || !aligned16(A) || !aligned16(B) || (lda % 4) || (ldb % 4)) return 0;
   const int tiles_m = (M + TM - 1) / TM, tiles_n = (N + TN - 1) / TN;
@@ -188,6 +187,14 @@
   const int cus = vqf_cu_count() > 0 ? vqf_cu_count() : 256;
   if (tiles > cus || tiles * 10 < (long long)cus * 8 || M > 1024) return 0;
   if (vqf_opt(VQF_OPT_GEMM_CU_LIMIT, 0) >= 8) return 0;
+  return 1;
+}
+
+int vqf_gemm_f32_n80_try(int M, int N, int K, const float* A, int lda, const float* B, int ldb, float* C, int ldc,
+                         const float* bias, int flags, hipStream_t s, int* rc) {
+  if (!vqf_gemm_f32_n80_applies(M, N, K, A, lda, B, ldb, flags)) return 0;
+  const int tiles_m = (M + TM - 1) / TM, tiles_n = (N + TN - 1) / TN;
+  const long long tiles = (long long)tiles_m * tiles_n;
   N80Args g;
   g.A = A; g.B = B; g.C = C; g.bias = bias; g.M = M; g.N = N; g.K = K; g.lda = lda; g.ldb = ldb; g.ldc = ldc; g.flags = flags;
   g.tiles_m = tiles_m; g.tiles = (int)tiles;
diff --git a/vqa-attention-networks_amd/csrc/gemm_f32_wave.hip b/vqa-attention-networks_amd/csrc/gemm_f32_wave.hip
--- a/vqa-attention-networks_amd/csrc/gemm_f32_wave.hip
+++ b/vqa-attention-networks_amd/csrc/gemm_f32_wave.hip
@@ -501,12 +501,23 @@
 
 }
 
-int vqf_gemm_f32_wave_try(int ta, int tb, int M, int N, int K, const float* A, int lda, const float* B, int ldb, float* C,
-                          int ldc, const float* bias, int flags, hipStream_t s, int* rc) {
+int vqf_gemm_f32_wave_applies(int ta, int tb, int M, int N, int K, const float* A, int lda, const float* B, int ldb) {
   if (vqf_opt(VQF_OPT_GEMM_F32_WAVE, 1) == 0) return 0;
   if (ta || M > 1024 || (K % TK) || K < 256 || !aligned16(A) || !aligned16(B) || (lda % 4) || (ldb % 4)) return 0;
   if (tb && (N % 4)) return 0;
   if ((long long)((M + 127) / 128) * ((N + 127) / 128) >= 256) return 0;
+  const int tiles = ((M + WTM - 1) / WTM) * ((N + WTN - 1) / WTN);
+  const int nwg1 = (tiles + 3) / 4, nwg4 = tiles;
+  const bool ok4 = (K % (4 * TK) == 0) && K / 4 >= 256;
+  if (nwg1 <= 256 && nwg1 >= 192) return 1;
+  if (ok4 && nwg4 <= 256 && nwg4 >= 192) return 4;
+  return 0;
+}
+
+int vqf_gemm_f32_wave_try(int ta, int tb, int M, int N, int K, const float* A, int lda, const float* B, int ldb, float* C,
+                          int ldc, const float* bias, int flags, hipStream_t s, int* rc) {
+  const int wk = vqf_gemm_f32_wave_applies(ta, tb, M, N, K, A, lda, B, ldb);
+  if (!wk) return 0;
   WaveArgs g;
   g.A = A; g.B = B; g.C = C; g.bias = bias;
   g.M = M; g.N = N; g.K = K; g.lda = lda; g.ldb = ldb; g.ldc = ldc; g.flags = flags;
@@ -514,11 +525,6 @@
   g.tiles_n = (N + WTN - 1) / WTN;
   const int tiles = g.tiles_m * g.tiles_n;
   const int nwg1 = (tiles + 3) / 4, nwg4 = tiles;
-  const bool ok4 = (K % (4 * TK) == 0) && K / 4 >= 256;
-  int wk = 0;
-  if (nwg1 <= 256 && nwg1 >= 192) wk = 1;
-  else if (ok4 && nwg4 <= 256 && nwg4 >= 192) wk = 4;
-  if (!wk) return 0;
   g.kpart = (wk == 1) ? K : K / 4;
   vqf_prof_dims(M, N, K);
   vqf_stat_bump(VQF_STAT_GEMM_F32_WAVE);
diff --git a/vqa-attention-networks_amd/csrc/gemm_group_plan.h b/vqa-attention-networks_amd/csrc/gemm_group_plan.h
--- /dev/null
+++ b/vqa-attention-networks_amd/csrc/gemm_group_plan.h
@@ -0,0 +1,131 @@
+#pragma once
+#include <stddef.h>
+#include <stdint.h>
+#include "../../include/vqa_fusion.h"
+
+constexpr int VQF_T128_TILE = 128;
+constexpr int VQF_GROUP_MAX = 4;
+constexpr int VQF_GROUP_WS_ALIGN = 256;
+
+static inline int vqf_tile128_split(int M, int N, int K, int bk, bool has_ws, size_t ws_bytes, int* kchunk) {
+  const long long tiles = (long long)((M + VQF_T128_TILE - 1) / VQF_T128_TILE) * ((N + VQF_T128_TILE - 1) / VQF_T128_TILE);
+  const int ktiles = (K + bk - 1) / bk;
+  int splits = 1;
+  const int slots = 512;
+  if (has_ws && tiles < 1024 && ktiles >= 32 && !(tiles >= 512 && K <= 1024) && !(tiles >= 192 && tiles <= 256 && K <= 512)) {
+    double best = 1e30;
+    for (int sp = 1; sp <= 16; ++sp) {
+      if (ktiles / sp < 16) break;
+      if ((size_t)sp * M * N * sizeof(float) > ws_bytes) break;
+      const double blocks = (double)tiles * sp;
+      const double rounds = (double)((long long)((blocks + slots - 1) / slots));
+      const double cost = rounds / sp * (1.0 + 0.01 * sp);
+      if (cost < best - 1e-12) { best = cost; splits = sp; }
+    }
+  }
+  const int kt_per = (ktiles + splits - 1) / splits;
+  *kchunk = kt_per * bk;
+  return (K + *kchunk - 1) / *kchunk;
+}
+
+static inline bool vqf_gemm_desc_ok(const VqfGemmDesc& d) {
+  return d.A && d.B && d.C && d.M > 0 && d.N > 0 && d.K > 0 && d.lda > 0 && d.ldb > 0 && d.ldc >= d.N;
+}
+
+struct VqfGroupMember {
+  int desc;
+  int tiles_m, tiles_n;
+  int splits, kchunk;
+  int block_end;
+  size_t slab_off;
+  size_t slab_bytes;
+  int reduce_blocks;
+  int reduce_end;
+};
+
+struct VqfGroupPlan {
+  int n_grouped;
+  VqfGroupMember m[VQF_GROUP_MAX];
+  int n_solo;
+  int solo[VQF_GROUP_MAX];
+  int total_blocks;
+  int n_split, reduce_total;
+  size_t ws_used;
+};
+
+typedef int (*VqfOtherFamilyFn)(const VqfGemmDesc* d, const void* ws, size_t ws_bytes);
+
+static inline int vqf_gemm_group_plan(int count, const VqfGemmDesc* descs, const void* ws, size_t ws_bytes, int bk, bool grouping,
+                                      VqfOtherFamilyFn other_family, VqfGroupPlan* plan) {
+  if (!plan) return VQF_E_BADARG;
+  *plan = VqfGroupPlan{};
+  if (count < 1 || count > VQF_GROUP_MAX || !descs) return VQF_E_BADARG;
+  for (int i = 0; i < count; ++i)
+    if (!vqf_gemm_desc_ok(descs[i])) return VQF_E_BADARG;
+  bool take[VQF_GROUP_MAX] = {};
+  VqfGroupMember cand[VQF_GROUP_MAX] = {};
+  const uintptr_t base = (uintptr_t)ws;
+  size_t cur = 0;
+  int n = 0;
+  for (int i = 0; i < count && grouping; ++i) {
+    const VqfGemmDesc& d = descs[i];
+    if (other_family && other_family(&d, ws, ws_bytes)) continue;
+    VqfGroupMember c = {};
+    c.desc = i;
+    c.tiles_m = (d.M + VQF_T128_TILE - 1) / VQF_T128_TILE;
+    c.tiles_n = (d.N + VQF_T128_TILE - 1) / VQF_T128_TILE;
+    c.splits = vqf_tile128_split(d.M, d.N, d.K, bk, ws != nullptr, ws_bytes, &c.kchunk);
+    const long long blocks = (long long)c.tiles_m * c.tiles_n * c.splits;
+    if (blocks > (1LL << 24)) continue;
+    if (c.splits > 1) {
+      const size_t pad = (size_t)((VQF_GROUP_WS_ALIGN - ((base + cur) % VQF_GROUP_WS_ALIGN)) % VQF_GROUP_WS_ALIGN);
+      const size_t bytes = (size_t)c.splits * d.M * d.N * sizeof(float);
+      if (cur + pad > ws_bytes || bytes > ws_bytes - (cur + pad)) continue;
+      c.slab_off = cur + pad;
+      c.slab_bytes = bytes;
+      cur = c.slab_off + bytes;
+    }
+    cand[n++] = c;
+    take[i] = true;
+  }
+  if (n < 2) {
+    for (int i = 0; i < count; ++i) plan->solo[plan->n_solo++] = i;
+    return VQF_OK;
+  }
+  for (int i = 0; i < count; ++i)
+    if (!take[i]) plan->solo[plan->n_solo++] = i;
+  for (int i = 1; i < n; ++i) {
+    const VqfGroupMember c = cand[i];
+    const int depth = c.kchunk < descs[c.desc].K ? c.kchunk : descs[c.desc].K;
+    int j = i;
+    while (j > 0) {
+      const VqfGroupMember& p = cand[j - 1];
+      const int pd = p.kchunk < descs[p.desc].K ? p.kchunk : descs[p.desc].K;
+      if (pd >= depth) break;
+      cand[j] = cand[j - 1];
+      --j;
+    }
+    cand[j] = c;
+  }
+  int end = 0, rend = 0;
+  for (int i = 0; i < n; ++i) {
+    VqfGroupMember& c = cand[i];
+    end += c.tiles_m * c.tiles_n * c.splits;
+    c.block_end = end;
+    if (c.splits > 1) {
+      const long long total = (long long)descs[c.desc].M * descs[c.desc].N;
+      long long rb = (total + 255) / 256;
+      if (rb > 4096) rb = 4096;
+      c.reduce_blocks = (int)rb;
+      rend += c.reduce_blocks;
+      ++plan->n_split;
+    }
+    c.reduce_end = rend;
+    plan->m[i] = c;
+  }
+  plan->n_grouped = n;
+  plan->total_blocks = end;
+  plan->reduce_total = rend;
+  plan->ws_used = cur;
+  return VQF_OK;
+}
diff --git a/vqa-attention-networks_amd/csrc/prof.hip b/vqa-attention-networks_amd/csrc/prof.hip
--- a/vqa-attention-networks_amd/csrc/prof.hip
+++ b/vqa-attention-networks_amd/csrc/prof.hip
@@ -11,7 +11,8 @@
 const char* const kOptEnv[VQF_OPT_COUNT] = {
     "VQF_GEMM_F32_PERSIST", "VQF_GEMM_BF16_PERSIST", "VQF_GEMM_F32_LOOP", "VQF_GEMM_BF16_LOOP", "VQF_GEMM_F32_BIG",
     "VQF_GEMM_BF16_BIG", "VQF_GEMM_F32_WAVE", "VQF_FUSE_COAL", "VQF_FUSE_LS", "VQF_FUSE_LS_BWD", "VQF_GEMM_CU_LIMIT",
-    "VQF_GEMM_F32_EDGE", "VQF_GEMM_F32_ROUNDS", "VQF_GEMM_SPLITK_FUSED", "VQF_GEMM_F32_STREAMK", "VQF_GEMM_SPLITK_ORDER", "VQF_GEMM_F32_SAMPLE", "VQF_GEMM_F32_N80"};
+    "VQF_GEMM_F32_EDGE", "VQF_GEMM_F32_ROUNDS", "VQF_GEMM_SPLITK_FUSED", "VQF_GEMM_F32_STREAMK", "VQF_GEMM_SPLITK_ORDER", "VQF_GEMM_F32_SAMPLE", "VQF_GEMM_F32_N80",
+    "VQF_GEMM_F32_GROUP"};
 const char* const kOptEnvOld[VQF_OPT_COUNT] = {
     nullptr, nullptr, "VQF_GEMM_F32_PP", "VQF_GEMM_BF16_PP", nullptr, nullptr, nullptr, nullptr, nullptr, nullptr, nullptr,
     nullptr, nullptr, nullptr, nullptr, nullptr, nullptr};
@@ -47,7 +48,7 @@
     "lstm_cell_fwd", "lstm_cell_bwd", "embed_tanh_fwd", "embed_tanh_bwd", "hbm_copy", "hbm_read_sweep", "multi_add", "multi_copy", "hie_hv_fwd", "hie_head_bwd", "hie_rank_add", "hie_rank_left", "hie_slab_sum", "hie_affinity",
     "phrase_ngram_fwd", "phrase_ngram_bwd", "hie_affinity_levels", "guided_logits_fwd", "guided_logits_bwd",
     "ce_loss_pred", "answer_match_rows", "topk_rows", "glimpse_dfeat_grouped", "row_block_gather", "row_block_group_sum",
-    "mfb_fuse_bwd_image", "zero_cols_len"};
+    "mfb_fuse_bwd_image", "zero_cols_len", "gemm_f32_group"};
 
 hipEvent_t get_event() {
   std::lock_guard<std::mutex> lk(g_mu);
@@ -60,7 +61,7 @@
 
 bool vqf_prof_begin(int id, hipStream_t s) {
   if (g_min_mnk > 0) {
-    const bool gemm = (id >= KID_GEMM_A0B0 && id <= KID_GEMM_A1B1) || id == KID_GEMM_BF16;
+    const bool gemm = (id >= KID_GEMM_A0B0 && id <= KID_GEMM_A1B1) || id == KID_GEMM_BF16 || id == KID_GEMM_GROUP;
     if (!gemm || (long long)t_dims[0] * t_dims[1] * t_dims[2] < g_min_mnk) return false;
   }
   t_start = get_event();
diff --git a/vqa-attention-networks_amd/host/functions.py b/vqa-attention-networks_amd/host/functions.py
--- a/vqa-attention-networks_amd/host/functions.py
+++ b/vqa-attention-networks_amd/host/functions.py
@@ -55,6 +55,11 @@
 
     def __init__(self):
         self.inv, self.L, self.lin, self.xb = None, 0, None, None
+
+
+def _underfilled_pair(M, N, K):
+    t = lambda r, c: ((r + 127) // 128) * ((c + 127) // 128)
+    return t(M, K) + t(N, K) <= 256
 
 
 class LinearFn(torch.autograd.Function):
@@ -94,6 +99,9 @@
             if ctx.needs_input_grad[1]:
                 dw = ops.gemm_bf16(dyb, x, ta=True, tb=True).view_as(w)
             return dx, dw, db, None, None
+        if ctx.needs_input_grad[0] and ctx.needs_input_grad[1] and _underfilled_pair(dy.shape[0], dy.shape[1], x.shape[1]):
+            dx, dw = ops.gemm_group([dict(a=dy, b=w2, tb=True), dict(a=dy, b=x, ta=True, tb=True)])
+            return dx, dw.view_as(w), db, None, None
         if ctx.needs_input_grad[0]:
             dx = ops.gemm(dy, w2, tb=True)
         if ctx.needs_input_grad[1]:
@@ -120,6 +128,13 @@
         w2 = _w2d(w)
         dy = _c(dy)
         K1 = x1.shape[1]
+        if all(ctx.needs_input_grad[:3]):
+            dw = torch.empty_like(w2)
+            dx1, dx2, _, _ = ops.gemm_group([dict(a=dy, b=w2[:, :K1], tb=True), dict(a=dy, b=w2[:, K1:], tb=True),
+                                             dict(a=dy, b=x1, ta=True, tb=True, out=dw[:, :K1]),
+                                             dict(a=dy, b=x2, ta=True, tb=True, out=dw[:, K1:])])
+            db = ops.colsum(dy) if (ctx.has_bias and ctx.needs_input_grad[3]) else None
+            return dx1, dx2, dw.view_as(w), db
         dx1 = ops.gemm(dy, w2[:, :K1], tb=True) if ctx.needs_input_grad[0] else None
         dx2 = ops.gemm(dy, w2[:, K1:], tb=True) if ctx.needs_input_grad[1] else None
         dw = None
@@ -563,10 +578,15 @@
             return dqa, dva, dwq, dbq, dwv, dbv, None, None, None, dcasc, None, None
         else:
             wq2, wv2 = _w2d(wq), _w2d(wv)
-            dqa = ops.gemm(dqq, wq2, tb=True) if ctx.needs_input_grad[0] else None
-            dva = ops.gemm(dvv, wv2, tb=True) if ctx.needs_input_grad[1] else None
-            dwq = ops.gemm(dqq, qa, ta=True, tb=True).view_as(wq)
-            dwv = ops.gemm(dvv, va, ta=True, tb=True).view_as(wv)
+            items = [dict(a=dqq, b=qa, ta=True, tb=True), dict(a=dvv, b=va, ta=True, tb=True)]
+            if ctx.needs_input_grad[0]:
+                items.append(dict(a=dqq, b=wq2, tb=True))
+            if ctx.needs_input_grad[1]:
+                items.append(dict(a=dvv, b=wv2, tb=True))
+            outs = ops.gemm_group(items)
+            dwq, dwv = outs[0].view_as(wq), outs[1].view_as(wv)
+            dqa = outs[2] if ctx.needs_input_grad[0] else None
+            dva = outs[-1] if ctx.needs_input_grad[1] else None
         dbq = ops.colsum(dqq)
         dbv = ops.colsum(dvv)
         return dqa, dva, dwq, dbq, dwv, dbv, None, None, None, dcasc, None, None
@@ -1008,8 +1028,17 @@
             dx, dw_ih = _lstm_in_proj_bwd(dGb, xb, wb, I, ctx.needs_input_grad[0])
             dx = dx.view(T, B, I) if dx is not None else None
         else:
-            dx = ops.gemm(dG2, _c(w_ih), tb=True).view(T, B, I) if ctx.needs_input_grad[0] else None
-            dw_ih = ops.gemm(dG2, x.view(T * B, I), ta=True, tb=True)
+            items = [dict(a=dG2, b=x.view(T * B, I), ta=True, tb=True)]
+            if ctx.needs_input_grad[0]:
+                items.append(dict(a=dG2, b=_c(w_ih), tb=True))
+            if T > 1:
+                items.append(dict(a=dG[1:].reshape((T - 1) * B, 4 * H), b=hs[:-1].reshape((T - 1) * B, H), ta=True, tb=True))
+            outs = ops.gemm_group(items)
+            dw_ih = outs[0]
+            dx = outs[1].view(T, B, I) if ctx.needs_input_grad[0] else None
+            dw_hh = outs[-1] if T > 1 else torch.zeros_like(w_hh)
+            db = ops.colsum(dG2) if ctx.has_bias else None
+            return dx, dw_ih, dw_hh, db, _copy_of(db), None
         if T > 1 and ctx.bf16_proj and B % 8 == 0:
             dw_hh = ops.gemm_bf16(dGb[B:], ops.cast_bf16(hs[:-1].reshape((T - 1) * B, H)), ta=True, tb=True)
         elif T > 1:
diff --git a/vqa-attention-networks_amd/host/lib.py b/vqa-attention-networks_amd/host/lib.py
--- a/vqa-attention-networks_amd/host/lib.py
+++ b/vqa-attention-networks_amd/host/lib.py
@@ -21,6 +21,14 @@
 c_sz = ctypes.c_size_t
 c_u64 = ctypes.c_uint64
 c_p = ctypes.c_void_p
+
+
+
+class VqfGemmDesc(ctypes.Structure):
+    _fields_ = [("ta", c_i), ("tb", c_i), ("M", c_i), ("N", c_i), ("K", c_i),
+                ("A", c_f), ("lda", c_i), ("B", c_f), ("ldb", c_i), ("C", c_f), ("ldc", c_i),
+                ("bias", c_f), ("flags", c_i)]
+
 
 SIGNATURES = {
     "vqf_abi_version": (c_i, []),
@@ -31,6 +39,8 @@
     "vqf_stat_get": (c_i, [c_i, ctypes.POINTER(ctypes.c_longlong)]),
     "vqf_gemm_f32_ws_bytes": (c_sz, [c_i, c_i, c_i, c_i, c_i]),
     "vqf_gemm_f32": (c_i, [c_i, c_i, c_i, c_i, c_i, c_f, c_i, c_f, c_i, c_f, c_i, c_f, c_i, c_p, c_sz, c_p]),
+    "vqf_gemm_f32_group_ws_bytes": (c_sz, [c_i, ctypes.POINTER(VqfGemmDesc)]),
+    "vqf_gemm_f32_group": (c_i, [c_i, ctypes.POINTER(VqfGemmDesc), c_p, c_sz, c_p]),
     "vqf_gemm_f32_big_rows": (c_i, [c_i, c_i, c_i, c_i, c_i]),
     "vqf_gemm_f32_sample_supported": (c_i, [c_i, c_i, c_i, c_i]),
     "vqf_gemm_f32_sample": (c_i, [c_i, c_i, c_i, c_i, c_i, c_f, c_i, c_f, c_i, c_f, c_i, c_f, c_i, c_p]),
diff --git a/vqa-attention-networks_amd/host/ops.py b/vqa-attention-networks_amd/host/ops.py
--- a/vqa-attention-networks_amd/host/ops.py
+++ b/vqa-attention-networks_amd/host/ops.py
@@ -60,7 +60,7 @@
 OPTIONS = {"gemm_f32_persist": 0, "gemm_bf16_persist": 1, "gemm_f32_loop": 2, "gemm_bf16_loop": 3, "gemm_f32_big": 4,
            "gemm_bf16_big": 5, "gemm_f32_wave": 6, "fuse_coal": 7, "fuse_ls": 8, "fuse_ls_bwd": 9, "gemm_cu_limit": 10,
            "gemm_f32_edge": 11, "gemm_f32_rounds": 12, "gemm_splitk_fused": 13, "gemm_f32_streamk": 14,
-           "gemm_splitk_order": 15, "gemm_f32_sample": 16, "gemm_f32_n80": 17}
+           "gemm_splitk_order": 15, "gemm_f32_sample": 16, "gemm_f32_n80": 17, "gemm_f32_group": 18}
 
 
 def set_option(name, value):
@@ -77,7 +77,7 @@
 
 
 STATS = {"gemm_f32_tile128": 0, "gemm_f32_big": 1, "gemm_f32_wave": 2, "gemm_bf16_tile128": 3, "gemm_bf16_big": 4,
-         "gemm_f32_sample": 5, "gemm_f32_n80": 6}
+         "gemm_f32_sample": 5, "gemm_f32_n80": 6, "gemm_f32_group": 7}
 
 
 def stat(name):
@@ -102,8 +102,7 @@
         return False
 
 
-def gemm(a, b, ta=False, tb=False, bias=None, relu=False, out=None, accumulate=False,
-         M=None, N=None, K=None, splitk=True):
+def _gemm_args(a, b, ta=False, tb=False, bias=None, relu=False, out=None, accumulate=False, M=None, N=None, K=None):
     _chk(bias)
     for t in (a, b, out):
         if t is None:
@@ -124,14 +123,34 @@
             raise _l.VqfError("gemm: accumulate needs out")
         out = torch.empty((M, N), dtype=torch.float32, device=a.device)
     flags = (GEMM_RELU if relu else 0) | (GEMM_ACCUM if accumulate else 0)
+    return int(ta), int(tb), M, N, K, a, b, out, bias, flags
+
+
+def gemm(a, b, ta=False, tb=False, bias=None, relu=False, out=None, accumulate=False,
+         M=None, N=None, K=None, splitk=True):
+    ta, tb, M, N, K, a, b, out, bias, flags = _gemm_args(a, b, ta, tb, bias, relu, out, accumulate, M, N, K)
     ws = None
     if splitk:
-        ws = workspace(a.device, max(SPLITK_WS_BYTES, int(_lib().vqf_gemm_f32_ws_bytes(int(ta), int(tb), M, N, K))))
-    rc = _lib().vqf_gemm_f32(int(ta), int(tb), M, N, K, _ptr(a), a.stride(0), _ptr(b), b.stride(0),
+        ws = workspace(a.device, max(SPLITK_WS_BYTES, int(_lib().vqf_gemm_f32_ws_bytes(ta, tb, M, N, K))))
+    rc = _lib().vqf_gemm_f32(ta, tb, M, N, K, _ptr(a), a.stride(0), _ptr(b), b.stride(0),
                              _ptr(out), out.stride(0), _ptr(bias), flags,
                              _ptr(ws), ws.numel() if ws is not None else 0, _stream())
     _l.check(rc, "vqf_gemm_f32")
     return out
+
+
+def gemm_group(items):
+    args = [_gemm_args(**it) for it in items]
+    descs = (_l.VqfGemmDesc * max(len(args), 1))()
+    for d, (ta, tb, M, N, K, a, b, out, bias, flags) in zip(descs, args):
+        d.ta, d.tb, d.M, d.N, d.K = ta, tb, M, N, K
+        d.A, d.lda, d.B, d.ldb, d.C, d.ldc = a.data_ptr(), a.stride(0), b.data_ptr(), b.stride(0), out.data_ptr(), out.stride(0)
+        d.bias, d.flags = (bias.data_ptr() if bias is not None else None), flags
+    if not args:
+        raise _l.VqfError("gemm_group: no items")
+    ws = workspace(args[0][5].device, max(SPLITK_WS_BYTES, int(_lib().vqf_gemm_f32_group_ws_bytes(len(args), descs))))
+    _l.check(_lib().vqf_gemm_f32_group(len(args), descs, _ptr(ws), ws.numel(), _stream()), "vqf_gemm_f32_group")
+    return [x[7] for x in args]
 
 
 def gemm_rows(a, b, L, tb=False, bias=None, relu=False, out=None):
```

Result: no change. 12820 (-0.3%).
